# LMNS3d/SOFTX_2020_200

Hardware: AMD Instinct MI355X
Metric: nonlinear iters/sec (3D cavity Q2 128^3 BDF2) (higher is better)
Workload: dtype f64; 1 GPU; 3D lid-driven cavity Q2-Q2 128^3 transient BDF2 (BASELINE configs[2]); n_dofs=67898372, n_cells=2097152, parallelism=single

## Files before the change

softx_2020_200_amd/csrc/gls_api.cpp:

```cpp
#include <hip/hip_runtime.h>

#include <algorithm>
#include <array>
#include <chrono>
#include <cmath>
#include <cstdlib>
#include <cstdarg>
#include <cstdio>
#include <cstring>
#include <map>
#include <array>
#include <memory>
#include <string>
#include <vector>
#include <set>

#include "gls_ctx.hpp"

using namespace gls_impl;

namespace {

thread_local std::string g_err;

// ... 748 lines not shown
    v = c->hang.vbuf.p;
  }
  P.v = v;
  P.y = y;
  P.hmask = c->hang.on ? c->hang.hmask.p : nullptr;
  const bool brick = c->use_brick && mode != gls::MODE_DIAG;
  const bool col = brick && c->use_colors;
  if (col) set_colors(c, P, y);
  else P.slab = brick ? brick_slab(c) : nullptr;
  if (!brick) {
    GLS_TRY(ensure_element_maps(c));
    P.ev = c->ev.p;
    if (cq_on) {
      P.cq = c->cq.p;
      P.cq_mode = mode == gls::MODE_DIAG ? 1 : 2;
    }
  }
  const bool oct = c->oct.on && (mode == gls::MODE_JV || mode == gls::MODE_DIAG) && !brick;
  if (oct) {
    const size_t nq = gls::brick_qdata_size(c->k, 8 * c->oct.nb);
    if (c->qdata.n != nq) {
      GLS_TRY(c->qdata.alloc(nq));
      c->qd_valid = false;
      c->cq_valid = false;
    }
    if (mode == gls::MODE_JV && !c->qd_valid) GLS_TRY(oct_lin(c));
    if (mode == gls::MODE_JV && c->oct.f32_next && !c->qd32_valid) {
      if (c->qdata32.n != c->qdata.n) GLS_TRY(c->qdata32.alloc(c->qdata.n));
      HIP_TRY(gls::vec_to_f32(c->qdata.p, c->qdata32.p, (int64_t)c->qdata.n, c->stream));
      c->qd32_valid = true;
    }
    P.cell_list = c->oct.rest.p;
    P.cell_list_n = c->oct.n_rest;
  }
  if (!col && !P.slab && !P.ev) HIP_TRY(hipMemsetAsync(y, 0, sizeof(double) * c->n_dofs, c->stream));
  {
    TimedLaunch t(c, mode == gls::MODE_JVQ ? (int)gls::MODE_JV : (lin_diag ? (int)gls::MODE_DIAG : mode));
    if (brick && split_jv && mode == gls::MODE_JVQ) {
      auto &D = c->dist;
      double *vv = const_cast<double *>(v);
      const int64_t voff = 3 * (int64_t)c->n_vnodes;
      if (D.on && !D.comm) {
        GLS_TRY(dist_import(c, vv));
      } else if (D.on) {
        HIP_TRY(hipEventRecord(D.ev_ready, c->stream));
        HIP_TRY(hipStreamWaitEvent(D.xstream, D.ev_ready, 0));
        HIP_TRY(gls::vec_pack_nodes(vv, D.send_nodes.p, D.n_send, voff, D.send_buf, D.xstream));
        if (rccl_exchange_on(c, 0, D.xstream) != 0) return set_err(GLS_ECOMM, "ghost import exchange failed");
        HIP_TRY(gls::vec_unpack_nodes(vv, D.recv_nodes.p, D.n_recv, voff, D.recv_buf, 0, D.xstream));
        HIP_TRY(hipEventRecord(D.ev_done, D.xstream));
      }
      gls::OpParams Q = P;
      Q.subset = c->split.p + c->split_bnd;
      Q.subset_n = c->split_int;
      if (Q.subset_n > 0) HIP_TRY(gls::launch_brick_kernel(c->k, mode, Q, c->tables, c->stream));
      if (D.on && D.comm) HIP_TRY(hipStreamWaitEvent(c->stream, D.ev_done, 0));
      Q.subset = c->split.p;
      Q.subset_n = c->split_bnd;
      if (Q.subset_n > 0) HIP_TRY(gls::launch_brick_kernel(c->k, mode, Q, c->tables, c->stream));
    } else if (brick) {
      HIP_TRY(gls::launch_brick_kernel(c->k, mode, P, c->tables, c->stream));
    } else {
      HIP_TRY(gls::launch_cell_kernel(c->dim, c->k, c->kp, c->nq1d, mode, P, c->tables, c->stream));
      if (oct) {
        gls::OpParams Q = P;
        Q.cell_list = nullptr;
        Q.cell_list_n = 0;
        Q.y = nullptr;
        Q.qd = c->qdata.p;
        Q.subset = c->oct.list.p;
        Q.subset_n = c->oct.nb;
        Q.brick_cell0 = c->oct.cell0.p;
        const bool f32 = mode == gls::MODE_JV && c->oct.f32_next;
        if (f32) Q.qdf = c->qdata32.p;
        HIP_TRY(gls::launch_pencil_ev(mode == gls::MODE_JV ? gls::MODE_JVQ : gls::MODE_LIN, Q, c->tables, c->stream, f32));
        if (mode == gls::MODE_DIAG) {
          c->qd_valid = true;
          c->qd32_valid = false;
        }
      }
    }
  }
  if (P.ev)
    HIP_TRY(gls::gather_element_vectors(y, c->ev.p, c->ev_voff.p, c->ev_vslot.p, c->n_vnodes, c->ev_poff.p,
                                        c->ev_pslot.p, c->n_pnodes, c->dim, c->stream));
  if (brick && !col && P.slab) {
    TimedLaunch t(c, 5);
    HIP_TRY(slab_sum(c, y));
  }
  if (c->hang.on && (mode == gls::MODE_RESIDUAL || mode == gls::MODE_JV))
    HIP_TRY(gls::vec_csr_condense(y, c->hang.tm.p, c->hang.toff.p, c->hang.tdof.p, c->hang.tw.p,
                                  (int64_t)c->hang.tm.n, c->stream));
  if (!c->probe_local) GLS_TRY(dist_export_add(c, y));
  if (P.cq_mode == 1) c->cq_valid = true;
  if (lin_diag) {
    c->qd_valid = true;
    c->qd32_valid = P.qdf != nullptr;
    c->qd32_partial = P.qdf != nullptr && P.oseen;
  }
  return GLS_OK;
}

}
namespace gls_impl {
int ensure_diag(gls_ctx *c) {
  if (c->diag_valid) return GLS_OK;
  GLS_TRY(run_cell(c, gls::MODE_DIAG, nullptr, c->diag.p));
  if (c->dist.on) {
    const int64_t d = c->dim, nl = c->n_vnodes, no = c->dist.n_owned, npl = c->n_dofs - d * nl, nop = c->dist.n_owned_p;
    HIP_TRY(gls::vec_fill(c->diag.p + d * no, d * (nl - no), 1.0, c->stream));
    HIP_TRY(gls::vec_fill(c->diag.p + d * nl + nop, npl - nop, 1.0, c->stream));
  }
  c->diag_valid = true;
  return GLS_OK;
}
}
namespace {

int device_dot(gls_ctx *c, const double *a, const double *b, double *host_out) {
  return dist_multidot(c, a, 0, 1, b, host_out);
}

const double *reduce_dots_async(gls_ctx *c, const double *out, int nd, double *hp, int *err) {
  const double *res = out;
  *err = GLS_OK;
  if (c->dist.on) {
    if (hipMemcpyAsync(c->dist.red_buf, out, sizeof(double) * nd, hipMemcpyDeviceToDevice, c->stream) != hipSuccess) {
      *err = set_err(GLS_EHIP, "reduce_dots_async: D2D copy");
      return nullptr;
    }
    if (c->dist.allreduce(c->dist.user, c->dist.red_buf, nd) != 0) {
      *err = set_err(GLS_ECOMM, "allreduce failed");
      return nullptr;
    }
    res = c->dist.red_buf;
  }
  if (hipMemcpyAsync(hp, res, sizeof(double) * nd, hipMemcpyDeviceToHost, c->stream) != hipSuccess) {
    *err = set_err(GLS_EHIP, "reduce_dots_async: D2H copy");
    return nullptr;
  }
  return res;
}
int multidot_async(gls_ctx *c, const double *A, int64_t lda, int nk, const double *w, double *out, double *hp,
                   const double **dev_res) {
  const int64_t n1 = c->dist.on ? (int64_t)c->dim * c->dist.n_owned : c->n_dofs;
  const int64_t off2 = c->dist.on ? (int64_t)c->dim * c->n_vnodes : 0;
  const int64_t n2 = c->dist.on ? c->dist.n_owned_p : 0;
  HIP_TRY(gls::vec_multidot2(A, lda, nk, w, n1, off2, n2, out, c->work.p, c->stream));
  int err;
  *dev_res = reduce_dots_async(c, out, nk, hp, &err);
  return err;
}
int multiaxpy_dots_async(gls_ctx *c, double *w, const double *V, int64_t lda, int nk, const double *h, bool dots,
                         double *out, double *hp, const double **dev_res, double scale = 1.0) {
  const int64_t n1 = c->dist.on ? (int64_t)c->dim * c->dist.n_owned : c->n_dofs;
  const int64_t off2 = c->dist.on ? (int64_t)c->dim * c->n_vnodes : 0;
  const int64_t n2 = c->dist.on ? c->dist.n_owned_p : 0;
  HIP_TRY(gls::vec_multiaxpy_dots(w, V, lda, nk, h, 1.0, c->n_dofs, n1, off2, n2, dots, scale, out, c->work.p,
                                  c->stream));
  int err;
  *dev_res = reduce_dots_async(c, out, dots ? nk + 1 : 1, hp, &err);
  return err;
}

}

extern "C" {

int gls_create(const gls_mesh_desc *d, gls_ctx **out) {
  if (!d || !out) return set_err(GLS_EINVAL, "null argument");
  *out = nullptr;
  const int nq1d = d->nq1d > 0 ? d->nq1d : d->k + 1;
  if (d->dim != 2 && d->dim != 3) return set_err(GLS_EINVAL, "dim must be 2 or 3");
  if (!gls::cell_kernel_supported(d->dim, d->k, d->kp, nq1d))
    return set_err(GLS_EINVAL, "unsupported element Q%d-Q%d (dim %d, QGauss %d)", d->k, d->kp, d->dim, nq1d);
  const bool mapped = d->map_degree > 0;
  if (d->n_cells < 0 || d->n_vnodes <= 0 || d->n_pnodes <= 0 || !d->cell_vnodes || (!mapped && !d->cell_h))
    return set_err(GLS_EINVAL, "incomplete mesh description");
  if (mapped && (d->map_degree > 2 || !d->cell_support))
    return set_err(GLS_EINVAL, "mapped cells: map_degree 1 or 2 with cell_support");
  if (d->kp != d->k && !d->cell_pnodes) return set_err(GLS_EINVAL, "cell_pnodes required when kp != k");
  if (d->srf && !d->cell_x0 && !mapped) return set_err(GLS_EINVAL, "srf requires cell_x0");
  std::unique_ptr<gls_ctx> c(new gls_ctx);
  c->dim = d->dim;
  c->k = d->k;
  c->kp = d->kp;
  c->nq1d = nq1d;
  c->n_cells = d->n_cells;
  c->n_vnodes = d->n_vnodes;
  c->n_pnodes = d->n_pnodes;
  c->nq = gls::ipow(nq1d, d->dim);
  c->n_dofs = (int64_t)d->dim * d->n_vnodes + d->n_pnodes;
  c->viscosity = d->viscosity;
  c->srf = d->srf;
  for (int i = 0; i < 3; ++i) c->omega[i] = d->omega[i];
  c->tables = make_tables(d->k, d->kp, nq1d);
  const int nv = gls::ipow(d->k + 1, d->dim), np = gls::ipow(d->kp + 1, d->dim);
  for (int64_t i = 0; i < (int64_t)d->n_cells * nv; ++i)
    if (d->cell_vnodes[i] < 0 || d->cell_vnodes[i] >= d->n_vnodes) return set_err(GLS_EINVAL, "cell_vnodes out of range");
  if (d->cell_pnodes)
    for (int64_t i = 0; i < (int64_t)d->n_cells * np; ++i)
      if (d->cell_pnodes[i] < 0 || d->cell_pnodes[i] >= d->n_pnodes) return set_err(GLS_EINVAL, "cell_pnodes out of range");
  if (!d->cell_pnodes && d->n_pnodes != d->n_vnodes) return set_err(GLS_EINVAL, "n_pnodes != n_vnodes without cell_pnodes");

  GLS_TRY(c->cell_vnodes.upload(d->cell_vnodes, (size_t)d->n_cells * nv));
  c->use_brick = !mapped && detect_bricks(d, nq1d);
  if (c->use_brick) GLS_TRY(build_slab_map(c.get(), d));
  if (const char *e = std::getenv("GLS_JV_RECOMPUTE")) c->use_qdata = std::atoi(e) == 0;
  if (d->cell_pnodes) GLS_TRY(c->cell_pnodes.upload(d->cell_pnodes, (size_t)d->n_cells * np));
  std::vector<double> geo((size_t)d->n_cells * 4);
  const int nsup = mapped ? gls::ipow(d->map_degree + 1, d->dim) : 0;
  for (int cix = 0; cix < d->n_cells; ++cix) {
    double meas = 1.;
    if (mapped) {
      meas = corner_measure(d->dim, d->map_degree, d->cell_support + (size_t)cix * nsup * d->dim);
      if (!(meas > 0)) return set_err(GLS_EINVAL, "cell %d: non-positive measure (inverted cell)", cix);
      geo[cix * 4 + 0] = geo[cix * 4 + 1] = geo[cix * 4 + 2] = 1.0;
    } else {
      for (int e = 0; e < d->dim; ++e) {
        geo[cix * 4 + e] = d->cell_h[(size_t)cix * d->dim + e];
        meas *= geo[cix * 4 + e];
      }
      if (d->dim == 2) geo[cix * 4 + 2] = 1.0;
    }
    geo[cix * 4 + 3] = d->dim == 2 ? std::sqrt(4. * meas / M_PI) / d->k : std::pow(6 * meas / M_PI, 1. / 3.) / d->k;
  }
  GLS_TRY(c->geo.upload(geo.data(), geo.size()));
  if (mapped) {
    c->map_degree = d->map_degree;
    c->host_support.assign(d->cell_support, d->cell_support + (size_t)d->n_cells * nsup * d->dim);
    std::vector<double> gq((size_t)d->n_cells * c->nq * gls::kGeo);
    for (int cix = 0; cix < d->n_cells; ++cix) {
      mapped_geometry(d->dim, d->map_degree, nq1d, d->cell_support + (size_t)cix * nsup * d->dim,
                      gq.data() + (size_t)cix * c->nq * gls::kGeo);
      for (int q = 0; q < c->nq; ++q)
        if (!(gq[((size_t)cix * c->nq + q) * gls::kGeo + gls::kGeoJxW] > 0))
          return set_err(GLS_EINVAL, "cell %d: non-positive Jacobian at quadrature point %d", cix, q);
    }
    GLS_TRY(c->gq.upload(gq.data(), gq.size()));
  } else {
    c->host_h.assign(d->cell_h, d->cell_h + (size_t)d->n_cells * d->dim);
    if (d->cell_x0) c->host_x0.assign(d->cell_x0, d->cell_x0 + (size_t)d->n_cells * d->dim);
  }
  if (d->cell_x0) {
    std::vector<double> x0((size_t)d->n_cells * 3, 0.);
    for (int cix = 0; cix < d->n_cells; ++cix)
      for (int e = 0; e < d->dim; ++e) x0[cix * 3 + e] = d->cell_x0[(size_t)cix * d->dim + e];
    GLS_TRY(c->x0.upload(x0.data(), x0.size()));
  }
  if (d->force_q) GLS_TRY(c->force_q.upload(d->force_q, (size_t)d->n_cells * c->nq * d->dim));
  std::vector<int64_t> con;
  if (d->vnode_mask) {
    GLS_TRY(c->vmask.upload(d->vnode_mask, (size_t)d->n_vnodes));
    for (int64_t n = 0; n < d->n_vnodes; ++n)
      for (int e = 0; e < d->dim; ++e)
        if ((d->vnode_mask[n] >> e) & 1) con.push_back(n * d->dim + e);
  }
  GLS_TRY(c->con_dofs.upload(con.data(), con.size()));
  GLS_TRY(c->diag.alloc(c->n_dofs));
  GLS_TRY(c->work.alloc(gls::multidot_work_size()));
  GLS_TRY(c->scal.alloc(64));
  if (hipStreamCreateWithFlags(&c->stream, hipStreamNonBlocking) != hipSuccess)
    return set_err(GLS_EHIP, "stream create failed");
  c->own_stream = true;
  HIP_TRY(hipDeviceSynchronize());
  *out = c.release();
  return GLS_OK;
}

int gls_destroy(gls_ctx *c) {
  if (!c) return GLS_OK;
  (void)hipStreamSynchronize(c->stream);
  delete c;
  return GLS_OK;
}

int gls_set_stream(gls_ctx *c, void *s) {
  GLS_TRY(check_ctx(c));
  if (c->own_stream && c->stream) {
    (void)hipStreamSynchronize(c->stream);
    (void)hipStreamDestroy(c->stream);
  }
  c->own_stream = false;
  c->stream = (hipStream_t)s;
  if (c->mg.on) {
    for (size_t l = 1; l < c->mg.lev.size(); ++l) GLS_TRY(gls_set_stream(c->mg.lev[l], s));
    if (c->mg.replica) GLS_TRY(gls_set_stream(c->mg.replica, s));
    if (c->mg.rep2) GLS_TRY(gls_set_stream(c->mg.rep2, s));
  }
  return GLS_OK;
}

int gls_uses_brick_kernels(const gls_ctx *c) { return c && c->use_brick ? 1 : 0; }

int gls_quadrature_points(const gls_ctx *c, double *xq) {
  if (!c || !xq) return set_err(GLS_EINVAL, "null argument");
  const int dim = c->dim, nq = c->nq;
  if (c->map_degree > 0) {
    const int nsup = gls::ipow(c->map_degree + 1, dim);
    std::vector<double> g((size_t)nq * gls::kGeo);
    for (int cix = 0; cix < c->n_cells; ++cix) {
      mapped_geometry(dim, c->map_degree, c->nq1d, c->host_support.data() + (size_t)cix * nsup * dim, g.data());
      for (int q = 0; q < nq; ++q)
        for (int e = 0; e < dim; ++e) xq[((size_t)cix * nq + q) * dim + e] = g[(size_t)q * gls::kGeo + gls::kGeoX + e];
    }
    return GLS_OK;
  }
  if (c->host_x0.empty()) return set_err(GLS_EINVAL, "gls_quadrature_points: the mesh was created without cell_x0");
  for (int cix = 0; cix < c->n_cells; ++cix)
    for (int q = 0; q < nq; ++q) {
      const int qi[3] = {q % c->nq1d, (q / c->nq1d) % c->nq1d, q / (c->nq1d * c->nq1d)};
      for (int e = 0; e < dim; ++e)
        xq[((size_t)cix * nq + q) * dim + e] =
            c->host_x0[(size_t)cix * dim + e] + c->host_h[(size_t)cix * dim + e] * c->tables.xi[qi[e]];
    }
  return GLS_OK;
}

int gls_n_dofs(const gls_ctx *c, int64_t *n) {
  if (!c || !n) return set_err(GLS_EINVAL, "null argument");
  *n = c->n_dofs;
  return GLS_OK;
}

int gls_set_force(gls_ctx *c, const double *f) {
  GLS_TRY(check_ctx(c));
  HIP_TRY(hipStreamSynchronize(c->stream));
  if (!f) {
    c->force_q.release();
  } else {
    GLS_TRY(c->force_q.upload(f, (size_t)c->n_cells * c->nq * c->dim));
  }
  c->diag_valid = false;
  c->ilu.valid = false;
  c->qd_valid = false;
  c->cq_valid = false;
  return GLS_OK;
}

int gls_set_viscosity(gls_ctx *c, double nu) {
  GLS_TRY(check_ctx(c));
  c->viscosity = nu;
  c->diag_valid = false;
  c->ilu.valid = false;
  c->qd_valid = false;
  c->cq_valid = false;
  return GLS_OK;
}

int gls_set_time(gls_ctx *c, int scheme, const double ts[4]) {
  GLS_TRY(check_ctx(c));
  if (scheme < GLS_STEADY || scheme > GLS_SDIRK3_3) return set_err(GLS_EINVAL, "scheme %d", scheme);
  if (scheme != GLS_STEADY && (!ts || ts[0] == 0.)) return set_err(GLS_EINVAL, "time steps required");
  c->scheme = scheme;
  if (ts)
    for (int i = 0; i < 4; ++i) c->time_steps[i] = ts[i];
  if (!c->jf.on) c->mg.dirty = true;
  for (double &a : c->alpha) a = 0.;
  c->alpha_jac = 0.;
  c->sdt2 = 0.;
  c->n_hist = 0;
  if (scheme != GLS_STEADY) {
    const double sdt = 1. / ts[0];
    c->sdt2 = sdt * sdt;
  }
  if (scheme == GLS_BDF1 || scheme == GLS_BDF2 || scheme == GLS_BDF3) {
    const int order = scheme - GLS_BDF1 + 1;
    double a[6];
    GLS_TRY(gls_bdf_coefficients(order, ts, 4, a));
    for (int i = 0; i <= order; ++i) c->alpha[i] = a[i];
    c->alpha_jac = a[0];
    c->n_hist = order;
  } else if (is_sdirk(scheme)) {
    const bool three = scheme == GLS_SDIRK3 || scheme == GLS_SDIRK3_1 || scheme == GLS_SDIRK3_2 || scheme == GLS_SDIRK3_3;
    const int order = three ? 3 : 2;
    double t[12];
    GLS_TRY(gls_sdirk_coefficients(order, ts[0], t));
    int stage = 0;
    if (scheme == GLS_SDIRK2_1 || scheme == GLS_SDIRK3_1) stage = 1;
    if (scheme == GLS_SDIRK2_2 || scheme == GLS_SDIRK3_2) stage = 2;
    if (scheme == GLS_SDIRK3_3) stage = 3;
    c->alpha_jac = t[0];
    if (stage > 0) {
      for (int i = 0; i <= stage; ++i) c->alpha[i] = t[(stage - 1) * (order + 1) + i];
      c->n_hist = stage;
    }
  }
  if (!c->jf.on) {
    c->diag_valid = false;
    c->ilu.valid = false;
    c->qd_valid = false;
    c->cq_valid = false;
  }
  return GLS_OK;
}

int gls_set_state(gls_ctx *c, const double *u, const double *u1, const double *u2, const double *u3) {
  GLS_TRY(check_ctx(c));
  if (!u) return set_err(GLS_EINVAL, "u is null");
  c->u = u;
  c->u1 = u1;
  c->u2 = u2;
  c->u3 = u3;
  if (!c->jf.on) {
    c->diag_valid = false;
    c->ilu.valid = false;
    c->qd_valid = false;
    c->cq_valid = false;
    c->mg.dirty = true;
  }
  return dist_import(c, const_cast<double *>(u));
}

int gls_freeze_jacobian(gls_ctx *c, int freeze) {
  GLS_TRY(check_ctx(c));
  auto &j = c->jf;
  if (!freeze) {
    if (j.on) {
      j.on = false;
      c->diag_valid = false;
      c->ilu.valid = false;
      c->qd_valid = false;
      c->cq_valid = false;
      c->mg.dirty = true;
    }
    return GLS_OK;
  }
  if (!c->u) return set_err(GLS_EINVAL, "gls_freeze_jacobian: gls_set_state was not called");
  if (j.on) return GLS_OK;
  const size_t n = (size_t)c->n_dofs;
  if (j.u.n != n) GLS_TRY(j.u.alloc(n));
  HIP_TRY(hipMemcpyAsync(j.u.p, c->u, sizeof(double) * n, hipMemcpyDeviceToDevice, c->stream));
  const double *hs[3] = {c->u1, c->u2, c->u3};
  for (int h = 0; h < 3; ++h) {
    j.has[h] = hs[h] != nullptr && h < c->n_hist;
    if (!j.has[h]) continue;
    if (j.h[h].n != n) GLS_TRY(j.h[h].alloc(n));
    HIP_TRY(hipMemcpyAsync(j.h[h].p, hs[h], sizeof(double) * n, hipMemcpyDeviceToDevice, c->stream));
  }
  for (int i = 0; i < 4; ++i) {
    j.alpha[i] = c->alpha[i];
    j.ts[i] = c->time_steps[i];
  }
  j.alpha_jac = c->alpha_jac;
  j.sdt2 = c->sdt2;
  j.n_hist = c->n_hist;
  j.scheme = c->scheme;
  j.on = true;
  return GLS_OK;
}

int gls_dist_import(gls_ctx *c, double *x) {
  GLS_TRY(check_ctx(c));
  return dist_import(c, x);
}

int gls_dist_attach(gls_ctx *c, int64_t n_owned_nodes, int n_nbrs, const int64_t *send_offsets,
                    const int32_t *send_nodes, const int64_t *recv_offsets, const int32_t *recv_nodes, double *send_buf,
                    double *recv_buf, double *red_buf, gls_exchange_fn xchg, gls_allreduce_fn allreduce, void *user) {
  GLS_TRY(check_ctx(c));
  if (c->dim != 3 || c->k != c->kp || c->cell_pnodes.p) return set_err(GLS_EINVAL, "distributed path: 3D Qk-Qk only");
  if (n_owned_nodes < 0 || n_owned_nodes > c->n_vnodes || n_nbrs < 0 || !xchg || !allreduce || !red_buf)
    return set_err(GLS_EINVAL, "gls_dist_attach: bad arguments");
  const int64_t ns = n_nbrs ? send_offsets[n_nbrs] : 0, nr = n_nbrs ? recv_offsets[n_nbrs] : 0;
  for (int64_t i = 0; i < ns; ++i)
    if (send_nodes[i] < 0 || send_nodes[i] >= n_owned_nodes) return set_err(GLS_EINVAL, "send node not owned");
  for (int64_t i = 0; i < nr; ++i)
    if (recv_nodes[i] < n_owned_nodes || recv_nodes[i] >= c->n_vnodes) return set_err(GLS_EINVAL, "recv node not a ghost");
  if ((ns && !send_buf) || (nr && !recv_buf)) return set_err(GLS_EINVAL, "exchange buffers missing");
  GLS_TRY(upload_export_order(c->dist, send_nodes, ns));
  GLS_TRY(c->dist.send_nodes.upload(send_nodes, (size_t)ns));
  GLS_TRY(c->dist.recv_nodes.upload(recv_nodes, (size_t)nr));
  c->dist.n_owned = n_owned_nodes;
  c->dist.n_owned_p = n_owned_nodes;
  c->dist.dofs = false;
  c->dist.width = 4;
  c->dist.n_send = ns;
  c->dist.n_recv = nr;
  c->dist.send_buf = send_buf;
  c->dist.recv_buf = recv_buf;
  c->dist.red_buf = red_buf;
  c->dist.xchg = xchg;
  c->dist.allreduce = allreduce;
  c->dist.user = user;
  c->dist.on = true;
  c->diag_valid = false;
  c->ilu.valid = false;
  c->qd_valid = false;
  c->cq_valid = false;
  if (c->use_brick && gls::brick_subset_supported(c->k)) {
    std::vector<char> flag((size_t)c->n_vnodes, 0);
    for (int64_t i = 0; i < ns; ++i) flag[(size_t)send_nodes[i]] = 1;
    for (int64_t i = 0; i < nr; ++i) flag[(size_t)recv_nodes[i]] = 1;
    GLS_TRY(build_brick_split(c, flag));
  }
  return GLS_OK;
}

int gls_dist_attach_dofs(gls_ctx *c, int64_t n_owned_vnodes, int64_t n_owned_pnodes, int n_nbrs,
                         const int64_t *send_offsets, const int32_t *send_dofs, const int64_t *recv_offsets,
                         const int32_t *recv_dofs, double *send_buf, double *recv_buf, double *red_buf,
                         gls_exchange_fn xchg, gls_allreduce_fn allreduce, void *user) {
  GLS_TRY(check_ctx(c));
  const int64_t nvd = (int64_t)c->dim * c->n_vnodes, npn = c->n_dofs - nvd;
  if (n_owned_vnodes < 0 || n_owned_vnodes > c->n_vnodes || n_owned_pnodes < 0 || n_owned_pnodes > npn || n_nbrs < 0 ||
      !xchg || !allreduce || !red_buf)
    return set_err(GLS_EINVAL, "gls_dist_attach_dofs: bad arguments");
  if (c->mg.on) return set_err(GLS_EINVAL, "gls_dist_attach_dofs: no multigrid");
  const int64_t ns = n_nbrs ? send_offsets[n_nbrs] : 0, nr = n_nbrs ? recv_offsets[n_nbrs] : 0;
  auto owned = [&](int64_t d) { return d < nvd ? d / c->dim < n_owned_vnodes : d - nvd < n_owned_pnodes; };
  for (int64_t i = 0; i < ns; ++i)
    if (send_dofs[i] < 0 || send_dofs[i] >= c->n_dofs || !owned(send_dofs[i])) return set_err(GLS_EINVAL, "send DoF not owned");
  for (int64_t i = 0; i < nr; ++i)
    if (recv_dofs[i] < 0 || recv_dofs[i] >= c->n_dofs || owned(recv_dofs[i])) return set_err(GLS_EINVAL, "recv DoF not a ghost");
  if ((ns && !send_buf) || (nr && !recv_buf)) return set_err(GLS_EINVAL, "exchange buffers missing");
  auto &D = c->dist;
  GLS_TRY(upload_export_order(D, send_dofs, ns));
  GLS_TRY(D.send_nodes.upload(send_dofs, (size_t)ns));
  GLS_TRY(D.recv_nodes.upload(recv_dofs, (size_t)nr));
  D.h_send.assign(send_dofs, send_dofs + ns);
  D.h_recv.assign(recv_dofs, recv_dofs + nr);
  D.h_soff.assign(1, 0);
  D.h_roff.assign(1, 0);
  if (n_nbrs > 0) {
    D.h_soff.assign(send_offsets, send_offsets + n_nbrs + 1);
    D.h_roff.assign(recv_offsets, recv_offsets + n_nbrs + 1);
  }
  D.dofs = true;
  D.width = 1;
  D.n_owned = n_owned_vnodes;
  D.n_owned_p = n_owned_pnodes;
  D.n_send = ns;
  D.n_recv = nr;
  D.send_buf = send_buf;
  D.recv_buf = recv_buf;
  D.red_buf = red_buf;
  D.xchg = xchg;
  D.allreduce = allreduce;
  D.user = user;
  D.on = true;
  c->diag_valid = false;
  c->ilu.valid = false;
  c->qd_valid = false;
  c->cq_valid = false;
  return GLS_OK;
}

int gls_residual(gls_ctx *c, double *rhs) {
  GLS_TRY(check_ctx(c));
  if (!rhs) return set_err(GLS_EINVAL, "rhs is null");
  GLS_TRY(run_cell(c, gls::MODE_RESIDUAL, nullptr, rhs));
  HIP_TRY(gls::vec_set_indexed(rhs, c->con_dofs.p, nullptr, (int64_t)c->con_dofs.n, c->stream));
  return GLS_OK;
}

int gls_residual_and_diagonal(gls_ctx *c, double *rhs, double *d) {
  GLS_TRY(check_ctx(c));
  if (!rhs) return set_err(GLS_EINVAL, "rhs is null");
  if (!c->u) return set_err(GLS_EINVAL, "gls_set_state was not called");
  if (c->n_hist > 0 && !c->u1) return set_err(GLS_EINVAL, "scheme needs solution_m1");
  if (c->n_hist > 1 && !c->u2) return set_err(GLS_EINVAL, "scheme needs solution_m2");
  if (c->n_hist > 2 && !c->u3) return set_err(GLS_EINVAL, "scheme needs solution_m3");
  const bool fuse = !c->diag_valid && c->use_brick && c->use_qdata && c->use_slab && !c->use_colors && !c->hang.on &&
                    !c->dist.on && !c->jf.on && c->k == 2 && c->cube_nb1 > 0 && gls::pencil_enabled() &&
                    std::getenv("GLS_NO_RESLIN") == nullptr;
  if (fuse) {
    const size_t nq = gls::brick_qdata_size(c->k, c->n_cells);
    if (c->qdata.n != nq) GLS_TRY(c->qdata.alloc(nq));
    double *slab = brick_slab(c);
    if (!slab) return set_err(GLS_ENOMEM, "slab allocation failed");
    if (c->slab2.n != c->slab.n) GLS_TRY(c->slab2.alloc(c->slab.n));
    gls::OpParams P = make_params(c, true);
    P.qd = c->qdata.p;
    GLS_TRY(lin_f32_target(c, P));
    P.y = c->diag.p;
    P.slab = slab;
    P.res_y = rhs;
    P.res_slab = c->slab2.p;
    {
      TimedLaunch t(c, gls::MODE_DIAG);
      HIP_TRY(gls::launch_pencil_reslin(P, c->tables, c->stream));
    }
    {
      TimedLaunch t(c, 5);
      HIP_TRY(slab_sum_ex(c, c->slab2.p, nullptr, rhs, nullptr, nullptr, nullptr, 0.0, nullptr));
    }
    {
      TimedLaunch t(c, 5);
      HIP_TRY(slab_sum(c, c->diag.p));
    }
    HIP_TRY(gls::vec_set_indexed(rhs, c->con_dofs.p, nullptr, (int64_t)c->con_dofs.n, c->stream));
    c->qd_valid = true;
    c->qd32_valid = P.qdf != nullptr;
  c->qd32_partial = P.qdf != nullptr && P.oseen;
    c->diag_valid = true;
  } else {
    GLS_TRY(gls_residual(c, rhs));
    GLS_TRY(ensure_diag(c));
  }
  if (d && d != c->diag.p) HIP_TRY(gls::vec_copy(d, c->diag.p, c->n_dofs, c->stream));
  return GLS_OK;
}

int gls_jacobian_diagonal(gls_ctx *c, double *d) {
  GLS_TRY(check_ctx(c));
  GLS_TRY(ensure_diag(c));
  if (d && d != c->diag.p) HIP_TRY(gls::vec_copy(d, c->diag.p, c->n_dofs, c->stream));
  return GLS_OK;
}

int gls_jacobian_apply(gls_ctx *c, const double *v, double *y) {
  GLS_TRY(check_ctx(c));
  if (!v || !y || v == y) return set_err(GLS_EINVAL, "v/y null or aliased");
  if (c->con_dofs.n || c->dist.on) GLS_TRY(ensure_diag(c));
  GLS_TRY(run_cell(c, gls::MODE_JV, v, y));
  HIP_TRY(gls::vec_gather_scale_set(y, c->diag.p, v, c->con_dofs.p, (int64_t)c->con_dofs.n, c->stream));
  return GLS_OK;
}

}
namespace gls_impl {
int ensure_qdata32(gls_ctx *g, bool full) {
  GLS_TRY(ensure_qdata(g));
  if (!g->qd32_valid || (full && g->qd32_partial)) {
    if (g->qdata32.n != g->qdata.n) GLS_TRY(g->qdata32.alloc(g->qdata.n));
    HIP_TRY(gls::vec_to_f32(g->qdata.p, g->qdata32.p, (int64_t)g->qdata.n, g->stream));
    g->qd32_valid = true;
    g->qd32_partial = false;
  }
  return GLS_OK;
}
bool slab_f32() { return std::getenv("GLS_SLAB_F64") == nullptr; }
bool first_sweep_fusable(gls_ctx *g) {
  const char *e = std::getenv("GLS_MG_FIRST_FUSE");
  return e && std::atoi(e) != 0 && g->smooth_f32 && g->use_brick && g->use_qdata && !g->use_colors && !g->dist.on &&
         !g->hang.on && g->k == 2 && g->cube_nb1 > 0 && g->use_slab && gls::pencil_enabled() &&
         std::getenv("GLS_MG_NO_FUSE") == nullptr;
}
int jacobian_apply_f32(gls_ctx *g, const double *v, double *y, const double *rb, double first_omega, bool oseen) {
  if (!g->u) return set_err(GLS_EINVAL, "gls_set_state was not called");
  GLS_TRY(ensure_diag(g));
  GLS_TRY(ensure_qdata32(g, !oseen));
  GLS_TRY(dist_import(g, const_cast<double *>(v)));
  gls::OpParams P = make_params(g, true);
  P.qdf = g->qdata32.p;
  P.oseen = oseen ? 1 : 0;
  P.v = v;
  P.y = y;
  const bool col = g->use_colors;
  P.slab = col ? nullptr : brick_slab(g);
  const bool fuse_rb = rb && (P.slab || col) && !g->dist.on && gls::brick_fused_jacobi_supported(g->k) &&
                       std::getenv("GLS_MG_NO_FUSE") == nullptr;
  P.rb = fuse_rb ? rb : nullptr;
  P.slabf = P.slab && slab_f32() && gls::brick_fused_jacobi_supported(g->k) ? reinterpret_cast<float *>(P.slab)
                                                                             : nullptr;
  if (first_omega > 0.0) {
    if (!fuse_rb || !first_sweep_fusable(g)) return set_err(GLS_EINVAL, "fused first sweep not applicable");
    P.jx0 = const_cast<double *>(v);
    P.jd = g->diag.p;
    P.jomega = first_omega;
  }
  if (col) set_colors(g, P, y);
  if (!col && !P.slab) HIP_TRY(hipMemsetAsync(y, 0, sizeof(double) * g->n_dofs, g->stream));
  {
    TimedLaunch t(g, 4);
    HIP_TRY(gls::launch_brick_jv_f32(g->k, P, g->tables, g->stream));
  }
  if (P.slab) {
    TimedLaunch t(g, 5);
    HIP_TRY(slab_sum_ex(g, P.slab, P.slabf, y, nullptr, nullptr, P.jx0 ? g->diag.p : nullptr, P.jomega, P.rb, P.jx0));
  }
  GLS_TRY(dist_export_add(g, y));
  HIP_TRY(gls::vec_gather_scale_set(y, g->diag.p, v, g->con_dofs.p, (int64_t)g->con_dofs.n, g->stream, P.rb));
  if (rb && !fuse_rb) HIP_TRY(gls::vec_axpby(y, 1.0, rb, -1.0, g->n_dofs, g->stream));
  return GLS_OK;
}
int smoother_apply(gls_ctx *g, const double *v, double *y, const double *rb) {
  if (g->smooth_f32 && g->use_brick && g->use_qdata) return jacobian_apply_f32(g, v, y, rb, 0.0, g->smooth_oseen);
  g->oct.f32_next = g->smooth_f32 && g->oct.on;
  const int rc = gls_jacobian_apply(g, v, y);
  g->oct.f32_next = false;
  GLS_TRY(rc);
  if (rb) HIP_TRY(gls::vec_axpby(y, 1.0, rb, -1.0, g->n_dofs, g->stream));
  return GLS_OK;
}
static int ilu_sweep(gls_ctx *g, double *x, const double *b, double *y, double *z) {
  GLS_TRY(ensure_ilu(g));
  GLS_TRY(gls_jacobian_apply(g, x, y));
  HIP_TRY(gls::vec_axpby(y, 1.0, b, -1.0, g->n_dofs, g->stream));
  GLS_TRY(apply_ilu(g, y, z));
  HIP_TRY(gls::vec_axpy(x, 1.0, z, g->n_dofs, g->stream));
  return GLS_OK;
}
int smoother_sweep(gls_ctx *g, double *x, const double *b, double *y, double omega, double *z, const double *pxc) {
  const bool nofuse = std::getenv("GLS_MG_NO_FUSE") != nullptr;
  const bool brick = g->use_brick && g->use_qdata && (g->use_colors || brick_slab(g)) && !g->dist.on &&
                     !g->hang.on && gls::brick_fused_jacobi_supported(g->k);
  if (pxc && ((z && g->ilu.on && !g->ilu.probe_only) || nofuse || !brick || !g->smooth_f32 || g->use_colors || g->cube_nb1 <= 0))
    return set_err(GLS_EINVAL, "fused prolongation not applicable");
  if (z && g->ilu.on && !g->ilu.probe_only) return ilu_sweep(g, x, b, y, z);
  if (nofuse || !brick) {
    GLS_TRY(smoother_apply(g, x, y));
    HIP_TRY(gls::mg_jacobi_update(x, b, y, g->diag.p, omega, g->n_dofs, 0, g->stream));
    return GLS_OK;
  }
  if (!g->u) return set_err(GLS_EINVAL, "gls_set_state was not called");
  GLS_TRY(ensure_diag(g));
  const bool f32 = g->smooth_f32;
  GLS_TRY(f32 ? ensure_qdata32(g, !g->smooth_oseen) : ensure_qdata(g));
  gls::OpParams P = make_params(g, true);
  P.v = x;
// ... 73 lines not shown
}

}
static int detect_oct_bricks(gls_ctx *c) {
  auto &O = c->oct;
  O = gls_ctx::Oct();
  const char *e = std::getenv("GLS_OCT_BRICKS");
  if ((e && std::atoi(e) == 0) || c->dim != 3 || c->k != 2 || c->kp != 2 || c->map_degree > 0 || c->dist.on ||
      c->cell_pnodes.p || c->host_h.empty() || !gls::pencil_enabled() || c->n_cells < 8)
    return GLS_OK;
  const int64_t nc = c->n_cells;
  std::vector<int32_t> cv((size_t)nc * 27);
  HIP_TRY(hipMemcpy(cv.data(), c->cell_vnodes.p, cv.size() * sizeof(int32_t), hipMemcpyDeviceToHost));
  std::vector<int32_t> cell0;
  std::vector<char> in((size_t)nc, 0);
  int32_t lat[125];
  for (int64_t i = 0; i + 8 <= nc;) {
    bool ok = true;
    for (int ci = 1; ci < 8 && ok; ++ci)
      for (int d = 0; d < 3; ++d) ok = ok && c->host_h[(size_t)(i + ci) * 3 + d] == c->host_h[(size_t)i * 3 + d];
    for (int t = 0; t < 125 && ok; ++t) lat[t] = -1;
    for (int ci = 0; ci < 8 && ok; ++ci) {
      const int cx = ci & 1, cy = (ci >> 1) & 1, cz = ci >> 2;
      for (int a = 0; a < 27 && ok; ++a) {
        const int X = 2 * cx + a % 3, Y = 2 * cy + (a / 3) % 3, Z = 2 * cz + a / 9;
        int32_t &slot = lat[X + 5 * (Y + 5 * Z)];
        const int32_t nd = cv[(size_t)(i + ci) * 27 + a];
        if (slot < 0) slot = nd;
        else ok = slot == nd;
      }
    }
    if (ok) {
      std::vector<int32_t> u(lat, lat + 125);
      std::sort(u.begin(), u.end());
      ok = std::adjacent_find(u.begin(), u.end()) == u.end();
    }
    if (ok) {
      cell0.push_back((int32_t)i);
      for (int ci = 0; ci < 8; ++ci) in[(size_t)(i + ci)] = 1;
      i += 8;
    } else {
      ++i;
    }
  }
  if (cell0.empty()) return GLS_OK;
  std::vector<int32_t> rest;
  for (int64_t q = 0; q < nc; ++q)
    if (!in[(size_t)q]) rest.push_back((int32_t)q);
  std::vector<int32_t> list(cell0.size());
  for (size_t b = 0; b < list.size(); ++b) list[b] = (int32_t)b;
  GLS_TRY(O.cell0.upload(cell0.data(), cell0.size()));
  GLS_TRY(O.list.upload(list.data(), list.size()));
  O.n_rest = (int)rest.size();
  if (rest.empty()) rest.push_back(0);
  GLS_TRY(O.rest.upload(rest.data(), rest.size()));
  O.nb = (int)cell0.size();
  O.on = true;
  return GLS_OK;
}
extern "C" {
int gls_forest_bricks(const gls_ctx *c) { return c && c->oct.on ? c->oct.nb : 0; }

int gls_set_hanging(gls_ctx *c, int64_t n, const int64_t *dofs, const int64_t *off, const int64_t *masters,
                    const double *w) {
  GLS_TRY(check_ctx(c));
  if (n < 0 || (n > 0 && (!dofs || !off || !masters || !w))) return set_err(GLS_EINVAL, "gls_set_hanging: arrays");
  if (c->mg.on) return set_err(GLS_EINVAL, "hanging constraints: no multigrid");
  if (c->dist.on && !c->dist.dofs) return set_err(GLS_EINVAL, "hanging constraints across ranks: gls_dist_attach_dofs");
  HIP_TRY(hipStreamSynchronize(c->stream));
  const int dim = c->dim;
  const int64_t N = c->n_dofs, nvd = (int64_t)dim * c->n_vnodes;
  std::vector<uint8_t> vm((size_t)c->n_vnodes, 0);
  if (c->vmask.p) HIP_TRY(hipMemcpy(vm.data(), c->vmask.p, (size_t)c->n_vnodes, hipMemcpyDeviceToHost));
  auto dirichlet = [&](int64_t d) { return d < nvd && ((vm[(size_t)(d / dim)] >> (d % dim)) & 1); };
  std::vector<char> is_h((size_t)N, 0);
  if (n > 0 && off[0] != 0) return set_err(GLS_EINVAL, "gls_set_hanging: offsets[0] != 0");
  for (int64_t i = 0; i < n; ++i) {
    const int64_t d = dofs[i];
    if (d < 0 || d >= N || off[i + 1] < off[i]) return set_err(GLS_EINVAL, "gls_set_hanging: line %lld", (long long)i);
    if (dirichlet(d)) return set_err(GLS_EINVAL, "hanging DoF %lld carries a Dirichlet mask bit", (long long)d);
    if (is_h[(size_t)d]) return set_err(GLS_EINVAL, "hanging DoF %lld listed twice", (long long)d);
    is_h[(size_t)d] = 1;
  }
  const int64_t nm = n ? off[n] : 0;
  for (int64_t j = 0; j < nm; ++j)
    if (masters[j] < 0 || masters[j] >= N || is_h[(size_t)masters[j]])
      return set_err(GLS_EINVAL, "gls_set_hanging: master %lld out of range or hanging itself", (long long)masters[j]);
  std::vector<int64_t> ooff{0}, omas, cnt((size_t)N + 1, 0);
  std::vector<double> ow;
  for (int64_t i = 0; i < n; ++i) {
    for (int64_t j = off[i]; j < off[i + 1]; ++j)
      if (!dirichlet(masters[j])) {
        omas.push_back(masters[j]);
        ow.push_back(w[j]);
        ++cnt[(size_t)masters[j] + 1];
      }
    ooff.push_back((int64_t)omas.size());
  }
  std::vector<int64_t> tm, toff{0};
  std::vector<int64_t> start((size_t)N + 1, 0);
  for (int64_t m = 0; m < N; ++m) {
    start[(size_t)m + 1] = start[(size_t)m] + cnt[(size_t)m + 1];
    if (cnt[(size_t)m + 1]) {
      tm.push_back(m);
      toff.push_back(start[(size_t)m + 1]);
    }
  }
  std::vector<int64_t> tdof(omas.size()), fill(start.begin(), start.end() - 1);
  std::vector<double> tw(omas.size());
  for (int64_t i = 0; i < n; ++i)
    for (int64_t j = ooff[(size_t)i]; j < ooff[(size_t)i + 1]; ++j) {
      const int64_t slot = fill[(size_t)omas[(size_t)j]]++;
      tdof[(size_t)slot] = dofs[i];
      tw[(size_t)slot] = ow[(size_t)j];
    }
  c->hang.h_dof.assign(dofs, dofs + n);
  c->hang.h_off.assign(off, off + n + 1);
  c->hang.h_master.assign(masters, masters + nm);
  if (n == 0) c->hang.h_off.assign(1, 0);
  std::vector<uint8_t> hm((size_t)c->n_vnodes, 0), dm((size_t)N, 0);
  std::vector<int64_t> con;
  for (int64_t d = 0; d < N; ++d) {
    if (is_h[(size_t)d] && d < nvd) hm[(size_t)(d / dim)] |= (uint8_t)(1u << (d % dim));
    dm[(size_t)d] = is_h[(size_t)d] ? 1 : 0;
    if (is_h[(size_t)d] || dirichlet(d)) con.push_back(d);
  }
  auto &h = c->hang;
  GLS_TRY(h.dof.upload(dofs, (size_t)n));
  GLS_TRY(h.off.upload(off, (size_t)(n ? n + 1 : 0)));
  GLS_TRY(h.master.upload(masters, (size_t)nm));
  GLS_TRY(h.w.upload(w, (size_t)nm));
  GLS_TRY(h.ooff.upload(ooff.data(), n ? ooff.size() : 0));
  GLS_TRY(h.omaster.upload(omas.data(), omas.size()));
  GLS_TRY(h.ow.upload(ow.data(), ow.size()));
  GLS_TRY(h.tm.upload(tm.data(), tm.size()));
  GLS_TRY(h.toff.upload(toff.data(), tm.empty() ? 0 : toff.size()));
  GLS_TRY(h.tdof.upload(tdof.data(), tdof.size()));
  GLS_TRY(h.tw.upload(tw.data(), tw.size()));
  GLS_TRY(h.hmask.upload(hm.data(), hm.size()));
  GLS_TRY(h.dmask.upload(dm.data(), dm.size()));
  GLS_TRY(c->con_dofs.upload(con.data(), con.size()));
  h.on = n > 0;
  c->use_brick = false;
  c->use_slab = false;
  c->use_colors = false;
  c->diag_valid = false;
  c->ilu.valid = false;
  c->qd_valid = false;
  c->cq_valid = false;
  return detect_oct_bricks(c);
}

namespace {
int apply_prec(gls_ctx *c, const double *v, double *z) {
  if (c->mg.on && c->mg.rep_csr) return mg_vcycle_rep2(c, v, z);
  if (c->mg.on) return mg_vcycle(c, 0, v, z);
  if (c->ilu.on && !c->ilu.probe_only) return apply_ilu(c, v, z);
  HIP_TRY(gls::vec_div(z, v, c->diag.p, c->n_dofs, c->stream));
  return GLS_OK;
}
}

int gls_apply_preconditioner(gls_ctx *c, const double *v, double *z) {
  GLS_TRY(check_ctx(c));
  if (!v || !z || v == z) return set_err(GLS_EINVAL, "v/z null or aliased");
  GLS_TRY(ensure_diag(c));
  if (c->mg.on) GLS_TRY(mg_prepare(c));
  GLS_TRY(ensure_ilu(c));
  return apply_prec(c, v, z);
}


static int solve_bicgstab(gls_ctx *c, const double *b, double *x, gls_linear_params *prm) {
  const int64_t n = c->n_dofs;
  hipStream_t s = c->stream;
  double *w[7];
  if (c->krylov.p && c->krylov.n >= (size_t)7 * n) {
    for (int i = 0; i < 7; ++i) w[i] = c->krylov.p + (int64_t)i * n;
  } else {
    if (c->bicg.n != (size_t)7 * n) GLS_TRY(c->bicg.alloc((size_t)7 * n));
    for (int i = 0; i < 7; ++i) w[i] = c->bicg.p + (int64_t)i * n;
  }
  double *r = w[0], *rh = w[1], *p = w[2], *v = w[3], *ph = w[4], *sh = w[5], *t = w[6];
  double bn2;
  GLS_TRY(device_dot(c, b, b, &bn2));
  const double tol = std::max(prm->relative_residual * std::sqrt(bn2), prm->minimum_residual);
  HIP_TRY(gls::vec_fill(x, n, 0.0, s));
  HIP_TRY(gls::vec_copy(r, b, n, s));
  HIP_TRY(gls::vec_copy(rh, b, n, s));
  HIP_TRY(gls::vec_fill(p, n, 0.0, s));
  HIP_TRY(gls::vec_fill(v, n, 0.0, s));
  double res = std::sqrt(bn2), rho = 1.0, alpha = 1.0, omega = 1.0;
  int it = 0;
  bool converged = res <= tol;
  while (!converged && it < prm->max_iterations) {
    double rho1;
    GLS_TRY(device_dot(c, rh, r, &rho1));
    if (rho1 == 0.0 || omega == 0.0) break;
    const double beta = (rho1 / rho) * (alpha / omega);
    rho = rho1;
    HIP_TRY(gls::vec_axpy(p, -omega, v, n, s));
    HIP_TRY(gls::vec_axpby(p, 1.0, r, beta, n, s));
    GLS_TRY(apply_prec(c, p, ph));
    GLS_TRY(gls_jacobian_apply(c, ph, v));
    double rhv;
    GLS_TRY(device_dot(c, rh, v, &rhv));
    if (rhv == 0.0) break;
    alpha = rho / rhv;
    HIP_TRY(gls::vec_axpy(r, -alpha, v, n, s));
    HIP_TRY(gls::vec_axpy(x, alpha, ph, n, s));
    ++it;
    double sn2;
    GLS_TRY(device_dot(c, r, r, &sn2));
    res = std::sqrt(sn2);
    if (res <= tol) {
      converged = true;
      break;
    }
    GLS_TRY(apply_prec(c, r, sh));
    GLS_TRY(gls_jacobian_apply(c, sh, t));
    double tt, ts;
    GLS_TRY(device_dot(c, t, t, &tt));
    GLS_TRY(device_dot(c, t, r, &ts));
    if (tt == 0.0) break;
    omega = ts / tt;
    HIP_TRY(gls::vec_axpy(x, omega, sh, n, s));
    HIP_TRY(gls::vec_axpy(r, -omega, t, n, s));
    double rn2;
    GLS_TRY(device_dot(c, r, r, &rn2));
    res = std::sqrt(rn2);
    converged = res <= tol;
    if (getenv("GLS_GMRES_VERBOSE") && (it % 10 == 0 || it == 1))
      printf("  bicgstab it %d  res %.6e  (tol %.3e)\n", it, res, tol);
  }
  if (converged && prm->true_residual) {
    GLS_TRY(gls_jacobian_apply(c, x, t));
    HIP_TRY(gls::vec_axpby(t, 1.0, b, -1.0, n, s));
    double rn2;
    GLS_TRY(device_dot(c, t, t, &rn2));
    res = std::sqrt(rn2);
  }
  prm->iterations = it;
  prm->final_residual = res;
  if (!converged) return set_err(GLS_ENOCONV, "BiCGStab: %d iterations, residual %.3e > %.3e", it, res, tol);
  return GLS_OK;
}

int gls_solve_linear(gls_ctx *c, const double *b, double *x, gls_linear_params *prm) {
  GLS_TRY(check_ctx(c));
  if (!b || !x || !prm) return set_err(GLS_EINVAL, "null argument");
  const int m = prm->restart > 0 ? std::min(prm->restart, 200) : 30;
  const int64_t n = c->n_dofs;
  if (c->krylov_m != m || !c->krylov.p) {
    GLS_TRY(c->krylov.alloc((size_t)(m + 1) * n));
    GLS_TRY(c->coef.alloc((size_t)m + 8));
    if (c->scal.n < (size_t)m + 8) GLS_TRY(c->scal.alloc((size_t)m + 8));
    if (c->scal2.n < (size_t)m + 8) GLS_TRY(c->scal2.alloc((size_t)m + 8));
    if (c->hpin_n < 3 * ((size_t)m + 8)) {
      if (c->hpin) HIP_TRY(hipHostFree(c->hpin));
      c->hpin = nullptr;
      c->hpin_n = 0;
      HIP_TRY(hipHostMalloc(reinterpret_cast<void **>(&c->hpin), sizeof(double) * 3 * ((size_t)m + 8)));
      c->hpin_n = 3 * ((size_t)m + 8);
    }
    c->krylov_m = m;
  }
  if (!c->tmp1.p) {
    GLS_TRY(c->tmp1.alloc(n));
    GLS_TRY(c->tmp2.alloc(n));
  }
  GLS_TRY(ensure_diag(c));
  if (c->mg.on) GLS_TRY(mg_prepare(c));
  GLS_TRY(ensure_ilu(c));
  if (prm->method == GLS_LIN_BICGSTAB) return solve_bicgstab(c, b, x, prm);
  if (prm->method != GLS_LIN_GMRES) return set_err(GLS_EINVAL, "linear solver method %d unknown", prm->method);
  const bool keepz = c->mg.on;
  if (keepz && c->zbasis.n != (size_t)m * n) GLS_TRY(c->zbasis.alloc((size_t)m * n));
  double *V = c->krylov.p, *z = c->tmp1.p, *r = c->tmp2.p;
  hipStream_t s = c->stream;
  double bnorm2;
  GLS_TRY(device_dot(c, b, b, &bnorm2));
  const double tol = std::max(prm->relative_residual * std::sqrt(bnorm2), prm->minimum_residual);
  bool x_zero = keepz;
  if (!keepz) HIP_TRY(gls::vec_fill(x, n, 0.0, s));
  const double *rcur = b;
  double beta = std::sqrt(bnorm2);
  int it = 0;
  std::vector<double> H((size_t)(m + 1) * m), cs(m), sn(m), g(m + 1), hc2(m + 2), y(m);
  const bool gram = prm->orthogonalization != GLS_ORTHO_CGS2;
  int ortho_repairs = 0;
  const double repair_tol = std::getenv("GLS_GMRES_REPAIR_TOL") ? std::atof(std::getenv("GLS_GMRES_REPAIR_TOL")) : 1e-8;
  const bool repair_measured = std::getenv("GLS_GMRES_REPAIR_MEASURED") != nullptr;
  std::vector<double> Gm((size_t)(m + 1) * (m + 1), 0.0);
  bool converged = beta <= tol;
  const bool lverbose = std::getenv("GLS_ILU_VERBOSE") != nullptr;
  while (!converged && it < prm->max_iterations) {
    if (lverbose) std::printf("gmres: it %d residual %.6e (tol %.3e)\n", it, beta, tol);
    HIP_TRY(gls::vec_axpby(V, 1.0 / beta, rcur, 0.0, n, s));
    std::fill(Gm.begin(), Gm.end(), 0.);
    std::fill(g.begin(), g.end(), 0.);
    g[0] = beta;
    int j = 0;
    double res = beta;
    for (; j < m && it < prm->max_iterations; ++j) {
      double *vj = V + (int64_t)j * n, *w = V + (int64_t)(j + 1) * n;
      double *zj = keepz ? c->zbasis.p + (int64_t)j * n : z;
      GLS_TRY(apply_prec(c, vj, zj));
      GLS_TRY(gls_jacobian_apply(c, zj, w));
      double *hp1 = c->hpin, *hp2 = c->hpin + (m + 8), *hp3 = c->hpin + 2 * (m + 8);
      const double *hdev = nullptr, *h2dev = nullptr, *h3dev = nullptr;
      GLS_TRY(multidot_async(c, V, n, j + 2, w, c->scal.p, hp1, &hdev));
      double wn2, wnorm, wnorm0;
      bool normalized = false;
      bool done = false;
      if (gram) {
        HIP_TRY(hipStreamSynchronize(s));
        const double wn0sq = std::max(hp1[j + 1], 0.0);
        wnorm0 = std::sqrt(wn0sq);
        auto G = [&](int a, int b) { return Gm[(size_t)std::min(a, b) * (m + 1) + std::max(a, b)]; };
        double *hc = hp3;
        for (int i = 0; i <= j; ++i) {
          double t = hp1[i];
          for (int k = 0; k <= j; ++k)
            if (k != i) t -= G(i, k) * hp1[k];
          hc[i] = t;
        }
        double q = wn0sq;
        for (int i = 0; i <= j; ++i) q += hc[i] * hc[i] - 2.0 * hc[i] * hp1[i];
        for (int i = 0; i <= j; ++i)
          for (int k = i + 1; k <= j; ++k) q += 2.0 * hc[i] * hc[k] * G(i, k);
        if (q > 1e-20 * wn0sq && q > 0.) {
          const double est = std::sqrt(q);
          HIP_TRY(hipMemcpyAsync(c->coef.p, hc, sizeof(double) * (j + 1), hipMemcpyHostToDevice, s));
          if (j + 1 <= 8) {
            GLS_TRY(multiaxpy_dots_async(c, w, V, n, j + 1, c->coef.p, true, c->scal2.p, hp2, &h2dev, 1.0 / est));
          } else {
            HIP_TRY(gls::vec_multiaxpy(w, V, n, j + 1, c->coef.p, 1.0, n, s));
            HIP_TRY(gls::vec_scale(w, 1.0 / est, n, s));
            GLS_TRY(multidot_async(c, V, n, j + 2, w, c->scal2.p, hp2, &h2dev));
          }
          HIP_TRY(hipStreamSynchronize(s));
          for (int i = 0; i <= j; ++i) H[(size_t)i * m + j] = hc[i];
          H[(size_t)(j + 1) * m + j] = est;
          double gmax = 0., gg = 0.;
          for (int i = 0; i <= j; ++i) {
            gmax = std::max(gmax, std::fabs(hp2[i]));
            gg += hp2[i] * hp2[i];
          }
          const double nrm2 = hp2[j + 1];
          const double est2sq = nrm2 - gg;
          if (gmax > repair_tol || std::fabs(nrm2 - 1.0) > repair_tol) {
            const bool use_est = est2sq > 1e-4 && !repair_measured;
            const double est2 = use_est ? std::sqrt(est2sq) : 1.0;
            for (int i = 0; i <= j; ++i) H[(size_t)i * m + j] += est * hp2[i];
            if (j + 1 <= 8) {
              GLS_TRY(multiaxpy_dots_async(c, w, V, n, j + 1, h2dev, true, c->scal.p, hp1, &hdev, 1.0 / est2));
            } else {
              HIP_TRY(gls::vec_multiaxpy(w, V, n, j + 1, h2dev, 1.0, n, s));
              if (use_est) HIP_TRY(gls::vec_scale(w, 1.0 / est2, n, s));
              GLS_TRY(multidot_async(c, V, n, j + 2, w, c->scal.p, hp1, &hdev));
            }
            HIP_TRY(hipStreamSynchronize(s));
            const double nn = std::max(hp1[j + 1], 0.0);
            double sc = 1.0;
            if (nn <= 1e-28 * (use_est ? 1.0 : std::max(nrm2, 1e-300))) {
              sc = 0.0;
            } else if (!use_est || std::fabs(nn - 1.0) > 1e-8) {
              sc = std::sqrt(nn);
              HIP_TRY(gls::vec_scale(w, 1.0 / sc, n, s));
            }
            H[(size_t)(j + 1) * m + j] = est * est2 * sc;
            for (int i = 0; i <= j; ++i) Gm[(size_t)i * (m + 1) + j + 1] = sc > 0. ? hp1[i] / sc : 0.;
            ++ortho_repairs;
          } else {
            for (int i = 0; i <= j; ++i) Gm[(size_t)i * (m + 1) + j + 1] = hp2[i];
          }
          wnorm = H[(size_t)(j + 1) * m + j];
          normalized = done = true;
        }
      }
      if (done) {
      } else if (j + 1 <= 8) {
        GLS_TRY(multiaxpy_dots_async(c, w, V, n, j + 1, hdev, true, c->scal2.p, hp2, &h2dev));
        HIP_TRY(hipStreamSynchronize(s));
        wnorm0 = std::sqrt(std::max(hp1[j + 1], 0.0));
        for (int i = 0; i <= j; ++i) H[(size_t)i * m + j] = hp1[i];
        std::copy(hp2, hp2 + j + 2, hc2.begin());
        wnorm = std::sqrt(std::max(hc2[j + 1], 0.0));
        if (wnorm < 0.7071 * wnorm0) {
          for (int i = 0; i <= j; ++i) H[(size_t)i * m + j] += hc2[i];
          double h2 = 0.;
          for (int i = 0; i <= j; ++i) h2 += hc2[i] * hc2[i];
          const double est2 = wnorm * wnorm - h2;
          if (est2 > 0.25 * wnorm * wnorm && est2 > 0.) {
            const double est = std::sqrt(est2);
            GLS_TRY(multiaxpy_dots_async(c, w, V, n, j + 1, h2dev, false, c->scal.p, hp3, &h3dev, 1.0 / est));
            HIP_TRY(hipStreamSynchronize(s));
            wn2 = hp3[0];
            H[(size_t)(j + 1) * m + j] = est;
            normalized = true;
            wnorm = est * std::sqrt(std::max(wn2, 0.0));
          } else {
            GLS_TRY(multiaxpy_dots_async(c, w, V, n, j + 1, h2dev, false, c->scal.p, hp3, &h3dev));
            HIP_TRY(hipStreamSynchronize(s));
            wn2 = hp3[0];
            wnorm = std::sqrt(std::max(wn2, 0.0));
          }
        }
      } else {
        HIP_TRY(gls::vec_multiaxpy(w, V, n, j + 1, hdev, 1.0, n, s));
        GLS_TRY(multidot_async(c, w, 0, 1, w, c->scal2.p, hp2, &h2dev));
        HIP_TRY(hipStreamSynchronize(s));
        wnorm0 = std::sqrt(std::max(hp1[j + 1], 0.0));
        for (int i = 0; i <= j; ++i) H[(size_t)i * m + j] = hp1[i];
        wn2 = hp2[0];
        wnorm = std::sqrt(std::max(wn2, 0.0));
        if (wnorm < 0.7071 * wnorm0) {
          GLS_TRY(multidot_async(c, V, n, j + 1, w, c->scal.p, hp1, &hdev));
          HIP_TRY(gls::vec_multiaxpy(w, V, n, j + 1, hdev, 1.0, n, s));
          GLS_TRY(multidot_async(c, w, 0, 1, w, c->scal2.p, hp2, &h2dev));
          HIP_TRY(hipStreamSynchronize(s));
          for (int i = 0; i <= j; ++i) H[(size_t)i * m + j] += hp1[i];
          wn2 = hp2[0];
          wnorm = std::sqrt(std::max(wn2, 0.0));
        }
      }
      if (!normalized) {
        H[(size_t)(j + 1) * m + j] = wnorm;
        if (wnorm > 0) HIP_TRY(gls::vec_scale(w, 1.0 / wnorm, n, s));
      }
      for (int i = 0; i < j; ++i) {
        const double a = H[(size_t)i * m + j], bb = H[(size_t)(i + 1) * m + j];
        H[(size_t)i * m + j] = cs[i] * a + sn[i] * bb;
        H[(size_t)(i + 1) * m + j] = -sn[i] * a + cs[i] * bb;
      }
      const double a = H[(size_t)j * m + j], bb = H[(size_t)(j + 1) * m + j];
      const double rr = std::hypot(a, bb);
      cs[j] = rr > 0 ? a / rr : 1.0;
      sn[j] = rr > 0 ? bb / rr : 0.0;
      H[(size_t)j * m + j] = rr;
      H[(size_t)(j + 1) * m + j] = 0.;
      g[j + 1] = -sn[j] * g[j];
      g[j] = cs[j] * g[j];
      res = std::fabs(g[j + 1]);
      ++it;
      if (getenv("GLS_GMRES_VERBOSE") && (it % 10 == 0 || it == 1))
        printf("  gmres it %d  res %.6e  (tol %.3e)\n", it, res, tol);
      if (res <= tol || wnorm == 0.) { ++j; break; }
    }
    const int kdim = j;
    for (int i = kdim - 1; i >= 0; --i) {
      double s_ = g[i];
      for (int l = i + 1; l < kdim; ++l) s_ -= H[(size_t)i * m + l] * y[l];
      y[i] = H[(size_t)i * m + i] != 0. ? s_ / H[(size_t)i * m + i] : 0.;
    }
    HIP_TRY(hipMemcpyAsync(c->coef.p, y.data(), sizeof(double) * kdim, hipMemcpyHostToDevice, s));
    if (keepz) {
      HIP_TRY(gls::vec_multiaxpy(x, c->zbasis.p, n, kdim, c->coef.p, -1.0, n, s, x_zero));
      x_zero = false;
    } else {
      HIP_TRY(gls::vec_fill(r, n, 0.0, s));
      HIP_TRY(gls::vec_multiaxpy(r, V, n, kdim, c->coef.p, -1.0, n, s));
      GLS_TRY(apply_prec(c, r, z));
      HIP_TRY(gls::vec_axpy(x, 1.0, z, n, s));
    }
    if (res <= tol) {
      beta = res;
      converged = true;
      if (prm->true_residual) {
        GLS_TRY(gls_jacobian_apply(c, x, r));
        HIP_TRY(gls::vec_axpby(r, 1.0, b, -1.0, n, s));
        double rn2;
        GLS_TRY(device_dot(c, r, r, &rn2));
        beta = std::sqrt(rn2);
      }
      break;
    }
    GLS_TRY(gls_jacobian_apply(c, x, r));
    HIP_TRY(gls::vec_axpby(r, 1.0, b, -1.0, n, s));
    rcur = r;
    double rn2;
    GLS_TRY(device_dot(c, r, r, &rn2));
    beta = std::sqrt(rn2);
    converged = beta <= tol;
    if (beta == 0.) break;
  }
  if (x_zero) HIP_TRY(gls::vec_fill(x, n, 0.0, s));
  prm->iterations = it;
  prm->final_residual = beta;
  if (ortho_repairs && std::getenv("GLS_GMRES_VERBOSE")) printf("  gmres: %d orthogonality repair passes\n", ortho_repairs);
  if (!converged) return set_err(GLS_ENOCONV, "GMRES: %d iterations, residual %.3e > %.3e", it, beta, tol);
  return GLS_OK;
}

}

namespace {

struct NewtonStats {
  int outer = 0, linear = 0, residuals = 0;
  double final_res = 0.;
};

template <class Phys>
int skip_newton_template(Phys &ph, double tolerance, int max_iterations, int verbosity, int skip_iterations,
                         bool is_initial_step, bool force_matrix_renewal, int &consecutive, NewtonStats &st) {
  double current_res = 1.0, last_res = 1.0;
  int outer = 0;
  bool assembly_needed = consecutive == 0 || is_initial_step || force_matrix_renewal;
  while (current_res > tolerance && outer < max_iterations) {
    GLS_TRY(ph.evaluation_point_from_present());
    if (assembly_needed) {
      GLS_TRY(ph.assemble_matrix_and_rhs());
      ++st.residuals;
    } else if (outer == 0) {
      GLS_TRY(ph.assemble_rhs());
      ++st.residuals;
    }
    if (outer == 0) {
      GLS_TRY(ph.rhs_norm(current_res));
      last_res = current_res;
    }
    if (verbosity) printf("Newton iteration: %d  - Residual:  %g\n", outer, current_res);
    int lin_it = 0;
    GLS_TRY(ph.solve_linear_system(lin_it));
    st.linear += lin_it;
    for (double alpha = 1.0; alpha > 1e-3; alpha *= 0.5) {
      GLS_TRY(ph.line_point(alpha));
      GLS_TRY(ph.assemble_rhs());
      ++st.residuals;
      GLS_TRY(ph.rhs_norm(current_res));
      if (verbosity) printf("\t\talpha = %6g res = %g\n", alpha, current_res);
      if (current_res < 0.9 * last_res || last_res < tolerance) break;
    }
    GLS_TRY(ph.present_from_evaluation_point());
    last_res = current_res;
    ++outer;
    assembly_needed = false;
  }
  if (!force_matrix_renewal) consecutive = (consecutive + 1) % std::max(skip_iterations, 1);
  st.outer = outer;
  st.final_res = current_res;
  return GLS_OK;
}

template <class Phys>
int newton_template(Phys &ph, double tolerance, int max_iterations, int verbosity, NewtonStats &st) {
  double current_res = 1.0, last_res = 1.0;
  int outer = 0;
  while (current_res > tolerance && outer < max_iterations) {
    GLS_TRY(ph.evaluation_point_from_present());
    GLS_TRY(ph.assemble_matrix_and_rhs());
    ++st.residuals;
    if (outer == 0) {
      GLS_TRY(ph.rhs_norm(current_res));
      last_res = current_res;
    }
    if (verbosity) printf("Newton iteration: %d  - Residual:  %g\n", outer, current_res);
    int lin_it = 0;
    GLS_TRY(ph.solve_linear_system(lin_it));
    st.linear += lin_it;
    for (double alpha = 1.0; alpha > 1e-3; alpha *= 0.5) {
      GLS_TRY(ph.line_point(alpha));
      GLS_TRY(ph.assemble_rhs());
      ++st.residuals;
      GLS_TRY(ph.rhs_norm(current_res));
      if (verbosity) printf("\t\talpha = %6g res = %g\n", alpha, current_res);
      if (current_res < 0.9 * last_res || last_res < tolerance) break;
    }
    GLS_TRY(ph.present_from_evaluation_point());
    last_res = current_res;
    ++outer;
  }
  st.outer = outer;
  st.final_res = current_res;
  return GLS_OK;
}

struct SectionScope {
  gls_ctx *c;
  int s;
  std::chrono::steady_clock::time_point t0;
  SectionScope(gls_ctx *c_, int s_) : c(c_), s(s_) {
    if (c->sec_on) {
      (void)hipStreamSynchronize(c->stream);
      t0 = std::chrono::steady_clock::now();
    }
  }
  ~SectionScope() {
    if (!c->sec_on) return;
    (void)hipStreamSynchronize(c->stream);
    c->sec_t[s] += std::chrono::duration<double>(std::chrono::steady_clock::now() - t0).count();
    ++c->sec_n[s];
  }
};

struct DevicePhysics {
  gls_ctx *c;
  double *present, *eval, *update, *rhs;
  const double *u1, *u2, *u3;
  gls_linear_params lin;
  int verbosity;
  bool skip = false;
  int linear_failures = 0;
  int evaluation_point_from_present() {
    if (!skip) return gls_set_state(c, present, u1, u2, u3);
    HIP_TRY(gls::vec_copy(eval, present, c->n_dofs, c->stream));
    return gls_set_state(c, eval, u1, u2, u3);
  }
  int assemble_matrix_and_rhs() {
    SectionScope t(c, GLS_SEC_ASSEMBLE_SYSTEM);
    if (skip) {
      GLS_TRY(gls_freeze_jacobian(c, 0));
      GLS_TRY(gls_set_state(c, eval, u1, u2, u3));
    }
    GLS_TRY(gls_residual_and_diagonal(c, rhs, nullptr));
    return skip ? gls_freeze_jacobian(c, 1) : GLS_OK;
  }
  int assemble_rhs() {
    SectionScope t(c, GLS_SEC_ASSEMBLE_RHS);
    return gls_residual(c, rhs);
  }
  int rhs_norm(double &r) {
    double r2;
    GLS_TRY(device_dot(c, rhs, rhs, &r2));
    r = std::sqrt(r2);
    return GLS_OK;
  }
  int solve_linear_system(int &its) {
    gls_linear_params lp = lin;
    if (c->mg.on) {
      SectionScope t(c, GLS_SEC_SETUP_GMG);
      GLS_TRY(ensure_diag(c));
      GLS_TRY(mg_prepare(c));
    } else if (c->ilu.on && !c->ilu.probe_only) {
      SectionScope t(c, GLS_SEC_SETUP_ILU);
      GLS_TRY(ensure_diag(c));
      GLS_TRY(ensure_ilu(c));
    }
    SectionScope t(c, GLS_SEC_SOLVE_LINEAR);
    const int rc = gls_solve_linear(c, rhs, update, &lp);
    if (rc < 0 && rc != GLS_ENOCONV) return rc;
    if (rc == GLS_ENOCONV) {
      ++linear_failures;
      if (verbosity) printf("  -Iterative solver did not converge: %d steps, residual %g\n", lp.iterations, lp.final_residual);
    }
    its = lp.iterations;
    if (verbosity) printf("  -Iterative solver took : %d steps \n", lp.iterations);
    HIP_TRY(gls::vec_set_indexed(update, c->con_dofs.p, nullptr, (int64_t)c->con_dofs.n, c->stream));
    return GLS_OK;
  }
  int line_point(double alpha) {
    HIP_TRY(gls::vec_waxpy(eval, present, alpha, update, c->n_dofs, c->stream));
    GLS_TRY(gls_apply_dirichlet(c, eval));
    return gls_set_state(c, eval, u1, u2, u3);
  }
  int present_from_evaluation_point() {
    HIP_TRY(gls::vec_copy(present, eval, c->n_dofs, c->stream));
    return GLS_OK;
  }
};

struct KatPhysics {
  double present[2] = {1., 0.}, eval[2] = {0, 0}, update[2] = {0, 0}, rhs[2] = {0, 0};
  double J[2][2] = {{0, 0}, {0, 0}};
  int evaluation_point_from_present() { eval[0] = present[0]; eval[1] = present[1]; return GLS_OK; }
  int assemble_matrix_and_rhs() {
    J[0][0] = 2 * eval[0]; J[0][1] = 1; J[1][0] = 0; J[1][1] = 2;
    return assemble_rhs();
  }
  int assemble_rhs() {
    rhs[0] = -(eval[0] * eval[0] + eval[1]);
    rhs[1] = -(2 * eval[1] + 3);
    return GLS_OK;
  }
  int rhs_norm(double &r) { r = std::sqrt(rhs[0] * rhs[0] + rhs[1] * rhs[1]); return GLS_OK; }
  int solve_linear_system(int &its) {
    const double det = J[0][0] * J[1][1] - J[0][1] * J[1][0];
    if (det == 0.) return set_err(GLS_EINVAL, "singular KAT Jacobian");
    update[0] = (rhs[0] * J[1][1] - J[0][1] * rhs[1]) / det;
    update[1] = (J[0][0] * rhs[1] - J[1][0] * rhs[0]) / det;
    its = 1;
    return GLS_OK;
  }
  int line_point(double a) { eval[0] = present[0] + a * update[0]; eval[1] = present[1] + a * update[1]; return GLS_OK; }
  int present_from_evaluation_point() { present[0] = eval[0]; present[1] = eval[1]; return GLS_OK; }
};

}

extern "C" {

int gls_newton_solve(gls_ctx *c, double *present, const double *u1, const double *u2, const double *u3,
                     gls_newton_params *prm) {
  GLS_TRY(check_ctx(c));
  if (!present || !prm) return set_err(GLS_EINVAL, "null argument");
  const int64_t n = c->n_dofs;
  if (!c->tmp3.p) {
    GLS_TRY(c->tmp3.alloc(n));
    GLS_TRY(c->tmp4.alloc(n));
    GLS_TRY(c->tmp5.alloc(n));
  }
  DevicePhysics ph{c, present, c->tmp3.p, c->tmp4.p, c->tmp5.p, u1, u2, u3, prm->lin, prm->verbosity};
  NewtonStats st;
  if (prm->solver == GLS_SKIP_NEWTON) {
    ph.skip = true;
    GLS_TRY(skip_newton_template(ph, prm->tolerance, prm->max_iterations, prm->verbosity, prm->skip_iterations,
                                 prm->is_initial_step != 0, prm->force_matrix_renewal != 0, c->skip_consecutive, st));
  } else {
    GLS_TRY(gls_freeze_jacobian(c, 0));
    GLS_TRY(newton_template(ph, prm->tolerance, prm->max_iterations, prm->verbosity, st));
  }
  HIP_TRY(hipStreamSynchronize(c->stream));
  prm->newton_iterations = st.outer;
  prm->linear_iterations = st.linear;
  prm->residual_evaluations = st.residuals;
  prm->final_residual = st.final_res;
  prm->linear_failures = ph.linear_failures;
  return GLS_OK;
}

int gls_section_timing(gls_ctx *c, int enable) {
  GLS_TRY(check_ctx(c));
  c->sec_on = enable != 0;
  for (int i = 0; i < GLS_N_SECTIONS; ++i) {
    c->sec_t[i] = 0.;
    c->sec_n[i] = 0;
  }
  return GLS_OK;
}
int gls_section_get(const gls_ctx *c, int section, double *seconds, int *calls) {
  if (!c) return set_err(GLS_EINVAL, "null context");
  if (section < 0 || section >= GLS_N_SECTIONS) return set_err(GLS_EINVAL, "section %d", section);
  if (seconds) *seconds = c->sec_t[section];
  if (calls) *calls = c->sec_n[section];
  return GLS_OK;
}

int gls_newton_selftest(double xo[2]) {
  if (!xo) return set_err(GLS_EINVAL, "null");
  KatPhysics ph;
  NewtonStats st;
  GLS_TRY(newton_template(ph, 1e-8, 10, 0, st));
  xo[0] = ph.present[0];
  xo[1] = ph.present[1];
  return GLS_OK;
}

int gls_skip_newton_selftest(int skip_iterations, double xo[2]) {
  if (!xo || skip_iterations < 1) return set_err(GLS_EINVAL, "gls_skip_newton_selftest arguments");
  KatPhysics ph;
  NewtonStats st;
  int consecutive = 0;
  GLS_TRY(skip_newton_template(ph, 1e-8, 10, 0, skip_iterations, true, true, consecutive, st));
  xo[0] = ph.present[0];
  xo[1] = ph.present[1];
  return GLS_OK;
}

int gls_mesh_hyper_cube_sizes(int dim, int n, int k, int kp, int pmask, int64_t *nc, int64_t *nv, int64_t *np) {
  if ((dim != 2 && dim != 3) || n <= 0 || k <= 0 || kp <= 0) return set_err(GLS_EINVAL, "mesh args");
  int64_t c = 1, v = 1, p = 1;
  for (int d = 0; d < dim; ++d) {
    const bool per = (pmask >> d) & 1;
    c *= n;
    v *= (int64_t)k * n + (per ? 0 : 1);
    p *= (int64_t)kp * n + (per ? 0 : 1);
  }
  if (nc) *nc = c;
  if (nv) *nv = v;
  if (np) *np = p;
  return GLS_OK;
}

int gls_mesh_hyper_cube(int dim, int n, int k, int kp, double lo, double hi, int pmask, int32_t *cv, int32_t *cp,
                        double *x0, double *h) {
  int64_t nc, nv, np;
  GLS_TRY(gls_mesh_hyper_cube_sizes(dim, n, k, kp, pmask, &nc, &nv, &np));
  if (nv > INT32_MAX || np > INT32_MAX) return set_err(GLS_EINVAL, "mesh too large for int32 node ids");
  int L = 0;
  while ((1 << L) < n) ++L;
  const double hc = (hi - lo) / n;
  int vsh[3], psh[3];
  for (int d = 0; d < 3; ++d) {
    const bool per = (pmask >> d) & 1;
    vsh[d] = k * n + (per ? 0 : 1);
    psh[d] = kp * n + (per ? 0 : 1);
  }
  const int nvl = gls::ipow(k + 1, dim), npl = gls::ipow(kp + 1, dim);
  int64_t cell = 0;
  const int64_t total = (int64_t)1 << (dim * L);
  for (int64_t mcode = 0; mcode < total; ++mcode) {
    int ijk[3] = {0, 0, 0};
    for (int b = 0; b < L; ++b)
      for (int d = 0; d < dim; ++d) ijk[d] |= (int)((mcode >> (b * dim + d)) & 1) << b;
    bool inside = true;
    for (int d = 0; d < dim; ++d) inside = inside && ijk[d] < n;
    if (!inside) continue;
    for (int a = 0; a < nvl; ++a) {
      int loc[3] = {a % (k + 1), (a / (k + 1)) % (k + 1), a / ((k + 1) * (k + 1))};
      int64_t id = 0, stride = 1;
      for (int d = 0; d < dim; ++d) {
        id += (int64_t)((ijk[d] * k + loc[d]) % vsh[d]) * stride;
        stride *= vsh[d];
      }
      cv[cell * nvl + a] = (int32_t)id;
    }
    if (cp) {
      for (int a = 0; a < npl; ++a) {
        int loc[3] = {a % (kp + 1), (a / (kp + 1)) % (kp + 1), a / ((kp + 1) * (kp + 1))};
        int64_t id = 0, stride = 1;
        for (int d = 0; d < dim; ++d) {
          id += (int64_t)((ijk[d] * kp + loc[d]) % psh[d]) * stride;
          stride *= psh[d];
        }
        cp[cell * npl + a] = (int32_t)id;
      }
    }
    for (int d = 0; d < dim; ++d) {
      if (x0) x0[cell * dim + d] = lo + ijk[d] * hc;
      if (h) h[cell * dim + d] = hc;
    }
    ++cell;
  }
  return cell == nc ? GLS_OK : set_err(GLS_EINVAL, "morton enumeration mismatch");
}

int gls_timing_enable(gls_ctx *c, int en) {
  GLS_TRY(check_ctx(c));
  c->timing = en != 0;
  return GLS_OK;
}
int gls_timing_reset(gls_ctx *c) {
  GLS_TRY(check_ctx(c));
  HIP_TRY(hipStreamSynchronize(c->stream));
  for (auto &e : c->events) { (void)hipEventDestroy(e.a); (void)hipEventDestroy(e.b); }
  c->events.clear();
  for (int i = 0; i < 6; ++i) { c->t_ms[i] = 0; c->t_n[i] = 0; }
  return GLS_OK;
}
int gls_timing_get(gls_ctx *c, int which, double *ms, int64_t *cnt) {
  GLS_TRY(check_ctx(c));
  if (which < 0 || which > 5) return set_err(GLS_EINVAL, "which");
  HIP_TRY(hipStreamSynchronize(c->stream));
  for (auto &e : c->events) {
    float t = 0;
    HIP_TRY(hipEventElapsedTime(&t, e.a, e.b));
    c->t_ms[e.which] += t;
    c->t_n[e.which] += 1;
    (void)hipEventDestroy(e.a);
    (void)hipEventDestroy(e.b);
  }
  c->events.clear();
  if (ms) *ms = c->t_ms[which];
  if (cnt) *cnt = c->t_n[which];
  return GLS_OK;
}

}
```

softx_2020_200_amd/csrc/gls_brick_kernels.hip:

```cpp
#include "gls_brick_common.hpp"
#include "gls_common.hpp"
#include "gls_launch.hpp"

#include <algorithm>
#include <cstdlib>
#include <type_traits>

#ifndef GLS_ABL
#define GLS_ABL 0
#endif
#ifndef GLS_ROWS_REG
#define GLS_ROWS_REG 1
#endif
#ifndef GLS_BRICK_WAVES_PER_EU
#define GLS_BRICK_WAVES_PER_EU 4
#endif
#ifndef GLS_BRICK_WPE_F32
#define GLS_BRICK_WPE_F32 6
#endif

#ifndef GLS_QD_LITE
#define GLS_QD_LITE 0
#endif

// ... 1077 lines not shown
__device__ __forceinline__ uint32_t morton3(uint32_t x, uint32_t y, uint32_t z) {
  uint32_t m = 0;
  for (int b = 0; b < 10; ++b)
    m |= (((x >> b) & 1u) << (3 * b)) | (((y >> b) & 1u) << (3 * b + 1)) | (((z >> b) & 1u) << (3 * b + 2));
  return m;
}
template <typename S, bool J, int K, bool XS = false>
__global__ void __launch_bounds__(256) k_slab_sum_cube(const S *__restrict__ slab, int nb1, int64_t voff,
                                                       double *__restrict__ y, const uint8_t *__restrict__ vmask,
                                                       const double *__restrict__ jb, const double *__restrict__ jd,
                                                       double jomega, const double *__restrict__ rb,
                                                       double *__restrict__ x0, const double *__restrict__ xs) {
  static_assert(!XS || J, "start values: fused Jacobi sweep");
  constexpr int BN = 2 * K + 1, P2 = 2 * K, NBND = BN * BN * BN - (BN - 2) * (BN - 2) * (BN - 2);
  const int NX = P2 * nb1 + 1;
  int bx = blockIdx.x, Z = blockIdx.y;
  if (GLS_SLAB_XCD) {
    const int lin = xcd_swizzle((int)(blockIdx.x + gridDim.x * blockIdx.y), (int)(gridDim.x * gridDim.y));
    bx = lin % (int)gridDim.x;
    Z = lin / (int)gridDim.x;
  }
  const bool zs = Z % P2 == 0;
  const int64_t t = (int64_t)bx * blockDim.x + threadIdx.x;
  int X, Y;
  const int ns = nb1 + 1;
  if (zs) {
    if (t >= (int64_t)NX * NX) return;
    X = (int)(t % NX);
    Y = (int)(t / NX);
  } else {
    const int64_t full = (int64_t)ns * NX, sparse = (int64_t)(NX - ns) * ns;
    if (t >= full + sparse) return;
    if (t < full) {
      X = (int)(t % NX);
      Y = (int)(t / NX) * P2;
    } else {
      const int64_t u = t - full;
      const int r = (int)(u / ns);
      X = (int)(u % ns) * P2;
      Y = (r / (P2 - 1)) * P2 + 1 + r % (P2 - 1);
    }
  }
  int bc[3][2], lc[3][2], nc[3];
  const int co[3] = {X, Y, Z};
#pragma unroll
  for (int d = 0; d < 3; ++d) {
    const int x = co[d];
    if (x % P2 == 0 && x > 0 && x < NX - 1) {
      nc[d] = 2;
      bc[d][0] = x / P2 - 1;
      lc[d][0] = P2;
      bc[d][1] = x / P2;
      lc[d][1] = 0;
    } else {
      nc[d] = 1;
      bc[d][0] = min(x / P2, nb1 - 1);
      lc[d][0] = x - P2 * bc[d][0];
      bc[d][1] = bc[d][0];
      lc[d][1] = lc[d][0];
    }
  }
  int64_t sl[8];
  int cnt = 0;
#pragma unroll
  for (int k = 0; k < 2; ++k)
#pragma unroll
    for (int j = 0; j < 2; ++j)
#pragma unroll
      for (int i = 0; i < 2; ++i) {
        const bool on = i < nc[0] && j < nc[1] && k < nc[2];
        const int64_t s = (int64_t)morton3(bc[0][i], bc[1][j], bc[2][k]) * NBND + bnd_index<BN>(lc[0][i], lc[1][j], lc[2][k]);
        sl[i + 2 * j + 4 * k] = on ? s : INT64_MAX;
        cnt += on;
      }
  auto cs = [&](int a, int b) {
    const int64_t lo = min(sl[a], sl[b]), hi = max(sl[a], sl[b]);
    sl[a] = lo;
    sl[b] = hi;
  };
  cs(0, 1); cs(2, 3); cs(4, 5); cs(6, 7);
  cs(0, 2); cs(1, 3); cs(4, 6); cs(5, 7);
  cs(1, 2); cs(5, 6); cs(0, 4); cs(3, 7);
  cs(1, 5); cs(2, 6);
  cs(1, 4); cs(3, 6);
  cs(2, 4); cs(3, 5);
  cs(3, 4);
  double e[8][4];
#pragma unroll
  for (int q = 0; q < 8; ++q)
    if (q < cnt) SlabQuad<S>::load(slab + sl[q] * 4, e[q][0], e[q][1], e[q][2], e[q][3]);
  double s[4] = {0., 0., 0., 0.};
#pragma unroll
  for (int q = 0; q < 8; ++q)
    if (q < cnt) {
      s[0] += e[q][0];
      s[1] += e[q][1];
      s[2] += e[q][2];
      s[3] += e[q][3];
    }
  const int64_t node = X + (int64_t)NX * (Y + (int64_t)NX * Z);
  const int64_t gi[4] = {node * 3, node * 3 + 1, node * 3 + 2, voff + node};
  if constexpr (J) {
    const unsigned m = vmask ? vmask[node] : 0u;
#pragma unroll
    for (int f = 0; f < 4; ++f) {
      const double x = XS ? xs[gi[f]] : y[gi[f]], dd = jd[gi[f]];
      y[gi[f]] = x + jomega * (jb[gi[f]] - ((f < 3 && ((m >> f) & 1u)) ? dd * x : s[f])) / dd;
    }
  } else if (rb) {
#pragma unroll
    for (int f = 0; f < 4; ++f) y[gi[f]] = rb[gi[f]] - s[f];
    if (x0) {
#pragma unroll
      for (int f = 0; f < 4; ++f) x0[gi[f]] = 0.0 + jomega * rb[gi[f]] / jd[gi[f]];
    }
  } else {
#pragma unroll
    for (int f = 0; f < 4; ++f) y[gi[f]] = s[f];
  }
}
hipError_t brick_slab_sum_cube(int k, int nb1, const double *slab, const float *slabf, int64_t n_vnodes, double *y,
                               const uint8_t *vmask, const double *jb, const double *jd, double jomega, hipStream_t s,
                               const double *rb, double *x0, const double *xs) {
  if (nb1 <= 0 || (k != 1 && k != 2)) return hipErrorInvalidValue;
  if (x0 && (!rb || !jd || jb)) return hipErrorInvalidValue;
  if (xs && (k != 2 || !jb || !jd || xs == y)) return hipErrorInvalidValue;
  const int NX = 2 * k * nb1 + 1;
  const dim3 g((unsigned)(((int64_t)NX * NX + 255) / 256), (unsigned)NX), b(256);
  const int64_t voff = 3 * n_vnodes;
  if (xs) {
    if (slabf) hipLaunchKernelGGL((k_slab_sum_cube<float, true, 2, true>), g, b, 0, s, slabf, nb1, voff, y, vmask, jb, jd, jomega, rb, x0, xs);
    else hipLaunchKernelGGL((k_slab_sum_cube<double, true, 2, true>), g, b, 0, s, slab, nb1, voff, y, vmask, jb, jd, jomega, rb, x0, xs);
    return hipGetLastError();
  }
  const double *const no_xs = nullptr;
#define GLS_SLAB_CUBE(KK)                                                                                                  \
  if (slabf) {                                                                                                              \
    if (jb) hipLaunchKernelGGL((k_slab_sum_cube<float, true, KK>), g, b, 0, s, slabf, nb1, voff, y, vmask, jb, jd, jomega, rb, x0, no_xs);  \
    else hipLaunchKernelGGL((k_slab_sum_cube<float, false, KK>), g, b, 0, s, slabf, nb1, voff, y, vmask, jb, jd, jomega, rb, x0, no_xs);   \
  } else {                                                                                                                  \
    if (jb) hipLaunchKernelGGL((k_slab_sum_cube<double, true, KK>), g, b, 0, s, slab, nb1, voff, y, vmask, jb, jd, jomega, rb, x0, no_xs); \
    else hipLaunchKernelGGL((k_slab_sum_cube<double, false, KK>), g, b, 0, s, slab, nb1, voff, y, vmask, jb, jd, jomega, rb, x0, no_xs);  \
  }
  if (k == 1) {
    GLS_SLAB_CUBE(1)
  } else {
    GLS_SLAB_CUBE(2)
  }
#undef GLS_SLAB_CUBE
  return hipGetLastError();
}

__global__ void __launch_bounds__(256) k_restrict_sum_cube(const double *__restrict__ ev, int nb1, int64_t voff,
                                                           double *__restrict__ bc, const uint8_t *__restrict__ vmask) {
  const int NX = 2 * nb1 + 1;
  int bx = blockIdx.x, Z = blockIdx.y;
  if (GLS_SLAB_XCD) {
    const int lin = xcd_swizzle((int)(blockIdx.x + gridDim.x * blockIdx.y), (int)(gridDim.x * gridDim.y));
    bx = lin % (int)gridDim.x;
    Z = lin / (int)gridDim.x;
  }
  const int64_t t = (int64_t)bx * blockDim.x + threadIdx.x;
  if (t >= (int64_t)NX * NX) return;
  const int X = (int)(t % NX), Y = (int)(t / NX);
  int bcd[3][2], lc[3][2], nc[3];
  const int co[3] = {X, Y, Z};
#pragma unroll
  for (int d = 0; d < 3; ++d) {
    const int x = co[d];
    if (x % 2 == 0 && x > 0 && x < NX - 1) {
      nc[d] = 2;
      bcd[d][0] = x / 2 - 1;
      lc[d][0] = 2;
      bcd[d][1] = x / 2;
      lc[d][1] = 0;
    } else {
      nc[d] = 1;
      bcd[d][0] = min(x / 2, nb1 - 1);
      lc[d][0] = x - 2 * bcd[d][0];
      bcd[d][1] = bcd[d][0];
      lc[d][1] = lc[d][0];
    }
  }
  int64_t sl[8];
  int cnt = 0;
#pragma unroll
  for (int k = 0; k < 2; ++k)
#pragma unroll
    for (int j = 0; j < 2; ++j)
#pragma unroll
      for (int i = 0; i < 2; ++i) {
        const bool on = i < nc[0] && j < nc[1] && k < nc[2];
        const int64_t s = (int64_t)morton3(bcd[0][i], bcd[1][j], bcd[2][k]) * 27 + lc[0][i] + 3 * (lc[1][j] + 3 * lc[2][k]);
        sl[i + 2 * j + 4 * k] = on ? s : INT64_MAX;
        cnt += on;
      }
  auto cs = [&](int a, int b) {
    const int64_t lo = min(sl[a], sl[b]), hi = max(sl[a], sl[b]);
    sl[a] = lo;
    sl[b] = hi;
  };
  cs(0, 1); cs(2, 3); cs(4, 5); cs(6, 7);
  cs(0, 2); cs(1, 3); cs(4, 6); cs(5, 7);
  cs(1, 2); cs(5, 6); cs(0, 4); cs(3, 7);
  cs(1, 5); cs(2, 6);
  cs(1, 4); cs(3, 6);
  cs(2, 4); cs(3, 5);
  cs(3, 4);
  double e[8][4];
#pragma unroll
  for (int q = 0; q < 8; ++q)
    if (q < cnt) SlabQuad<double>::load(ev + sl[q] * 4, e[q][0], e[q][1], e[q][2], e[q][3]);
  double s[4] = {0., 0., 0., 0.};
#pragma unroll
  for (int q = 0; q < 8; ++q)
    if (q < cnt) {
      s[0] += e[q][0];
      s[1] += e[q][1];
      s[2] += e[q][2];
      s[3] += e[q][3];
    }
  const int64_t node = X + (int64_t)NX * (Y + (int64_t)NX * Z);
  const unsigned m = vmask ? vmask[node] : 0u;
  bc[node * 3] = (m & 1u) ? 0.0 : s[0];
  bc[node * 3 + 1] = (m & 2u) ? 0.0 : s[1];
  bc[node * 3 + 2] = (m & 4u) ? 0.0 : s[2];
  bc[voff + node] = s[3];
}
hipError_t brick_restrict_sum_cube(int nb1, const double *ev, int64_t n_vnodes, double *bc, const uint8_t *vmask,
                                   hipStream_t s) {
  const int64_t NX = 2 * (int64_t)nb1 + 1;
  if (nb1 <= 0 || nb1 > 1023 || !ev || !bc || NX * NX * NX != n_vnodes) return hipErrorInvalidValue;
  const dim3 g((unsigned)((NX * NX + 255) / 256), (unsigned)NX), b(256);
  hipLaunchKernelGGL(k_restrict_sum_cube, g, b, 0, s, ev, nb1, 3 * n_vnodes, bc, vmask);
  return hipGetLastError();
}

bool brick_fused_jacobi_supported(int k) { return brick_impl(k) == 0 && (k == 1 || k == 2); }
#ifdef GLS_BRICK_COLORS_BUILD
bool brick_colors_supported(int k) { return brick_impl(k) == 0 && (k == 1 || k == 2); }
#else
bool brick_colors_supported(int) { return false; }
#endif
bool brick_subset_supported(int k) { return brick_impl(k) == 0 && (k == 1 || k == 2); }

size_t brick_qdata_size(int k, int n_cells) {
  if (brick_impl(k) == 1) return brick_wave_qdata_size(k, n_cells);
  return k == 1 ? brick_qdata_doubles<1>(n_cells) : (k == 2 ? brick_qdata_doubles<2>(n_cells) : 0);
}

hipError_t launch_brick_kernel(int k, int mode, const OpParams &P, const Tables1D &T, hipStream_t s) {
  if (mode == MODE_DIAG) return hipErrorNotSupported;
  if (brick_impl(k) == 1) return launch_brick_wave(k, mode, P, T, s);
  if (k == 1) return launch_brick_t<1>(mode, P, T, s);
  if (k == 2) return launch_brick_t<2>(mode, P, T, s);
  return hipErrorNotSupported;
}

}
```

softx_2020_200_amd/csrc/gls_ctx.hpp:

```cpp
#pragma once
#include <hip/hip_runtime.h>

#include <array>
#include <cstdint>
#include <memory>
#include <string>
#include <vector>

#include <rocblas/rocblas.h>
#include <rocsparse/rocsparse.h>
#include <rccl/rccl.h>

#include "../../include/gls_native.h"
#include "gls_common.hpp"
#include "gls_devbuf.hpp"
#include "gls_error.hpp"
#include "gls_launch.hpp"
#include "gls_mg_coarse.hpp"

#define RS_TRY(x)                                                                        \
  do {                                                                                   \
    const rocsparse_status rs_ = (x);                                                    \
    if (rs_ != rocsparse_status_success) return ::gls_impl::set_err(GLS_EHIP, "%s: rocsparse status %d", #x, (int)rs_); \
  } while (0)

using gls_impl::DevBuf;

struct gls_ctx {
  int dim = 0, k = 0, kp = 0, nq1d = 0, n_cells = 0, n_vnodes = 0, n_pnodes = 0, nq = 0;
  int64_t n_dofs = 0;
  hipStream_t stream = nullptr;
  bool own_stream = false;
  gls::Tables1D tables;
  DevBuf<int32_t> cell_vnodes, cell_pnodes;
  DevBuf<int32_t> face_nbr;
  DevBuf<double> geo, x0, force_q;
  DevBuf<double> gq;
  DevBuf<double> fd_meas, fd_tab, fd_partial, fd_out;
  std::vector<double> host_x0, host_h, host_support;
  int map_degree = 0;
  DevBuf<uint8_t> vmask;
  DevBuf<int64_t> con_dofs;
  DevBuf<int64_t> dir_dofs;
  DevBuf<double> dir_vals;
  double viscosity = 1.0;
  int srf = 0;
  double omega[3] = {0, 0, 0};
  int scheme = GLS_STEADY;
  double alpha[4] = {0, 0, 0, 0}, alpha_jac = 0., sdt2 = 0.;
  int n_hist = 0;
  const double *u = nullptr, *u1 = nullptr, *u2 = nullptr, *u3 = nullptr;
  DevBuf<double> diag;
  bool diag_valid = false;
  DevBuf<double> qdata;
  bool qd_valid = false;
  DevBuf<double> cq;
  bool cq_valid = false;
  DevBuf<float> qdata32;
  bool qd32_valid = false;
  bool qd32_partial = false;
  DevBuf<double> ev;
  DevBuf<double> bev;
  DevBuf<uint8_t> bact;
  DevBuf<int64_t> ev_voff, ev_vslot, ev_poff, ev_pslot;
  bool smooth_f32 = false;
  bool smooth_oseen = false;
  bool use_qdata = true;
  DevBuf<double> work, scal, coef;
  DevBuf<double> scal2;
  double *hpin = nullptr;
  size_t hpin_n = 0;
  DevBuf<double> krylov;
  DevBuf<double> zbasis;
  DevBuf<double> bicg;
  int krylov_m = 0;
  DevBuf<double> tmp1, tmp2, tmp3, tmp4, tmp5;
  bool use_brick = false;
  bool use_slab = false;
  DevBuf<double> slab;
  DevBuf<double> slab2;
  DevBuf<int32_t> sum_nodes, sum_off, sum_slots;
  int cube_nb1 = 0;
  bool use_colors = false;
  int n_colors = 0;
  int color_off[17] = {0};
  DevBuf<int32_t> color_bricks;
  DevBuf<uint16_t> ncolor;
  DevBuf<double> acc;
  struct Dist {
    bool on = false;
    bool dofs = false;
    int width = 4;
    int64_t n_owned = 0, n_owned_p = 0, n_send = 0, n_recv = 0;
    DevBuf<int32_t> add_u, add_off, add_slot;
    DevBuf<int32_t> send_nodes, recv_nodes;
    double *send_buf = nullptr, *recv_buf = nullptr, *red_buf = nullptr;
    gls_exchange_fn xchg = nullptr;
    gls_allreduce_fn allreduce = nullptr;
    void *user = nullptr;
    ncclComm_t comm = nullptr;
    std::vector<int> nbrs;
    std::vector<int64_t> soff, roff;
    std::vector<int32_t> h_send, h_recv;
    std::vector<int64_t> h_soff, h_roff;
    DevBuf<double> own_send, own_recv, own_red;
    hipStream_t xstream = nullptr;
    hipEvent_t ev_ready = nullptr, ev_done = nullptr;
  } dist;
  DevBuf<int32_t> split;
  int split_bnd = 0, split_int = 0;
  struct ILU {
    bool on = false, valid = false;
    bool probe_only = false;
    double athresh = 0., rthresh = 1.;
    double boost_tol = 0., boost_val = 0.;
    int n_probes = 0, fill = 0;
    int64_t block_dofs = 0;
    int ordering = GLS_ILU_ORDER_CM, n_blocks = 1, n_order_colors = 0;
    bool mc_solve = false;
    bool mc_factor = false;
    bool mc_compact = false;
    DevBuf<double> rdiag;
    std::vector<uint8_t> mc_wl, mc_wu;
    DevBuf<int64_t> mc_desc;
    DevBuf<int64_t> mc_moff;
    DevBuf<uint16_t> mc_map;
    std::vector<int32_t> mc_cg;
    DevBuf<int32_t> mc_grow;
    DevBuf<int64_t> mc_lsp, mc_usp;
    DevBuf<int64_t> ghost_diag;
    bool complete = false;
    int n_rounds = 0;
    std::vector<int64_t> rr;
    DevBuf<int64_t> ru;
    DevBuf<int32_t> ruoff, rslot;
    std::vector<int64_t> pdoff, peoff;
    DevBuf<int32_t> pdofs, prow;
    DevBuf<int64_t> pent;
    DevBuf<int32_t> pdpid, pepid;
    DevBuf<double> bV, bC, bY;
    DevBuf<uint8_t> wact;
    DevBuf<int32_t> wlist;
    std::vector<int64_t> woff;
    int wB = 0;
    int64_t wnblk = 0;
    DevBuf<int64_t> rowp, didx;
    DevBuf<int32_t> col, rowp32;
    DevBuf<int32_t> perm;
    DevBuf<double> val, vbuf, ybuf, tbuf;
    DevBuf<char> work;
    rocsparse_handle h = nullptr;
    rocsparse_mat_descr dA = nullptr, dL = nullptr, dU = nullptr;
    rocsparse_mat_info info = nullptr;
    int64_t nnz = 0, nnz_a = 0;
    void release() {
      if (info) rocsparse_destroy_mat_info(info);
      if (dA) rocsparse_destroy_mat_descr(dA);
      if (dL) rocsparse_destroy_mat_descr(dL);
      if (dU) rocsparse_destroy_mat_descr(dU);
      if (h) rocsparse_destroy_handle(h);
      info = nullptr;
      dA = dL = dU = nullptr;
      h = nullptr;
    }
    ~ILU() { release(); }
  } ilu;
  struct Hang {
    bool on = false;
    DevBuf<int64_t> dof, off, master, ooff, omaster;
    DevBuf<double> w, ow;
    DevBuf<int64_t> tm, toff, tdof;
    DevBuf<double> tw;
    DevBuf<uint8_t> hmask;
    DevBuf<uint8_t> dmask;
    DevBuf<double> vbuf;
    std::vector<int64_t> h_dof, h_off, h_master;
  } hang;
  struct Oct {
    bool on = false;
    int nb = 0;
    DevBuf<int32_t> cell0, list;
    DevBuf<int32_t> rest;
    int n_rest = 0;
    bool f32_next = false;
  } oct;
  struct Lattice {
    bool set = false;
    int n1d = 0, box0[3] = {0, 0, 0}, bdim[3] = {0, 0, 0};
    DevBuf<int32_t> map;
  } lat;
  struct MG {
    bool on = false;
    bool boxed = false;
    std::vector<gls_ctx *> lev;
    std::vector<std::array<int, 3>> dims;
    int k = 2, pre = 2, post = 2, csweeps = 30;
    std::vector<int> lpre, lpost;
    double omega = 0.6, comega = 0.6;
    std::vector<std::unique_ptr<DevBuf<double>>> bufs;
    struct Taps {
      DevBuf<int32_t> pi[3], ri[3], pc[3], rc[3];
      DevBuf<double> pw[3], rw[3];
      bool two_pass = false;
      bool q2_brick = false;
    };
    std::vector<std::unique_ptr<Taps>> taps;
    bool csr = false;
    bool ilu_smooth = false;
    struct Csr {
      DevBuf<int64_t> poff, roff;
      DevBuf<int32_t> pcol, rcol, inj;
      DevBuf<double> pw, rw;
      int64_t nf = 0, nc = 0;
      int plane = 1, rlane = 1;
    };
    std::vector<std::unique_ptr<Csr>> xfer;
    std::vector<gls_ctx *> ilu_levels;
    DevBuf<double> xwork;
    bool direct = false;
    gls_ctx *probe_ilu = nullptr;
    gls_impl::CoarseSolve coarse;
    struct Graph {
      hipGraphExec_t h = nullptr;
      Graph() = default;
      Graph(const Graph &) = delete;
      Graph &operator=(const Graph &) = delete;
      Graph(Graph &&o) noexcept : h(o.h) { o.h = nullptr; }
      Graph &operator=(Graph &&o) noexcept {
        if (this != &o) {
          reset();
          h = o.h;
          o.h = nullptr;
        }
        return *this;
      }
      void reset() {
        if (h) (void)hipGraphExecDestroy(h);
        h = nullptr;
      }
      ~Graph() { reset(); }
    } cgraph;
    std::vector<unsigned char> cgraph_key;
    bool cgraph_failed = false;
    bool dirty = true;
    gls_ctx *replica = nullptr;
    bool rep_csr = false;
    gls_ctx *rep2 = nullptr;
    DevBuf<int64_t> r2p_off, r2r_off;
    DevBuf<int32_t> r2p_col, r2r_col;
    DevBuf<double> r2p_w, r2r_w;
    int r2p_lane = 1, r2r_lane = 1;
    DevBuf<int32_t> r2inj_c, r2inj_f;
    DevBuf<int32_t> rep_own_loc, rep_own_glob;
    DevBuf<int32_t> rep_map;
    DevBuf<double> rep_b, rep_x, rep_tmp, rep_u[4];
  } mg;
  double time_steps[4] = {1, 1, 1, 1};
  struct JacFreeze {
    bool on = false;
    DevBuf<double> u, h[3];
    bool has[3] = {false, false, false};
    double alpha[4] = {0, 0, 0, 0}, alpha_jac = 0., sdt2 = 0., ts[4] = {1, 1, 1, 1};
    int n_hist = 0, scheme = GLS_STEADY;
  } jf;
  int skip_consecutive = 0;
  bool probe_local = false;
  bool sec_on = false;
  double sec_t[GLS_N_SECTIONS] = {};
  int sec_n[GLS_N_SECTIONS] = {};
  bool timing = false;
  struct Ev { int which; hipEvent_t a, b; };
  std::vector<Ev> events;
  double t_ms[6] = {0, 0, 0, 0, 0, 0};
  int64_t t_n[6] = {0, 0, 0, 0, 0, 0};

  ~gls_ctx() {
    if (hpin) (void)hipHostFree(hpin);
    for (auto &e : events) { (void)hipEventDestroy(e.a); (void)hipEventDestroy(e.b); }
    if (dist.ev_ready) (void)hipEventDestroy(dist.ev_ready);
    if (dist.ev_done) (void)hipEventDestroy(dist.ev_done);
    if (dist.xstream) (void)hipStreamDestroy(dist.xstream);
    if (own_stream && stream) (void)hipStreamDestroy(stream);
  }
};

namespace gls_impl {

inline int check_ctx(gls_ctx *c) {
  if (!c) return set_err(GLS_EINVAL, "null context");
  return GLS_OK;
}

gls::OpParams make_params(gls_ctx *c, bool jac = false);

struct TimedLaunch {
  gls_ctx *c;
  int which;
  hipEvent_t a = nullptr, b = nullptr;
  TimedLaunch(gls_ctx *c_, int w) : c(c_), which(w) {
    if (c->timing) {
      (void)hipEventCreate(&a);
      (void)hipEventCreate(&b);
      (void)hipEventRecord(a, c->stream);
    }
  }
  ~TimedLaunch() {
    if (c->timing) {
      (void)hipEventRecord(b, c->stream);
      c->events.push_back({which, a, b});
    }
  }
};

void gauss_points(int n, double *x, double *w);
void lobatto_points(int k, double *x);
void lagrange_1d(int k, const double *xn, int i, double s, double &v, double &d, double &dd);
double corner_measure(int dim, int md, const double *S);
int ensure_element_maps(gls_ctx *c);
int ensure_diag(gls_ctx *c);
inline bool cell_cache_on(const gls_ctx *c) {
  return !c->use_brick && c->n_cells > 0;
}
inline size_t cell_cache_size(const gls_ctx *c) {
  const int dim = c->dim;
  return (size_t)c->n_cells * (size_t)gls::ipow(c->nq1d, dim) * (size_t)(dim + dim * dim + 1 + dim);
}

double *brick_slab(gls_ctx *c);
int dist_import(gls_ctx *c, double *x);
int dist_export_add(gls_ctx *c, double *y);
int dist_allreduce_vector(gls_ctx *c, double *v, int64_t n);
int ensure_qdata(gls_ctx *c);
int ensure_qdata32(gls_ctx *g, bool full = true);
bool slab_f32();
bool first_sweep_fusable(gls_ctx *g);
int jacobian_apply_f32(gls_ctx *g, const double *v, double *y, const double *rb = nullptr, double first_omega = 0.0,
                       bool oseen = false);
int smoother_apply(gls_ctx *g, const double *v, double *y, const double *rb = nullptr);
int smoother_sweep(gls_ctx *g, double *x, const double *b, double *y, double omega, double *z = nullptr,
                   const double *pxc = nullptr);

int mg_prepare(gls_ctx *c);
int mg_vcycle(gls_ctx *c, int l, const double *b, double *x);
int mg_vcycle_rep2(gls_ctx *c, const double *b, double *x);

int ilu_probe(gls_ctx *c);
int ensure_ilu(gls_ctx *c);
int apply_ilu(gls_ctx *c, const double *v, double *z);

int rccl_exchange_on(gls_ctx *c, int phase, hipStream_t stream);

}
```

softx_2020_200_amd/csrc/gls_launch.hpp:

```cpp
#pragma once
#include "gls_common.hpp"

namespace gls {

hipError_t gather_element_vectors(double *y, const double *ev, const int64_t *voff, const int64_t *vslot, int64_t nv,
                                  const int64_t *poff, const int64_t *pslot, int64_t np, int dim, hipStream_t s);
hipError_t launch_cell_kernel(int dim, int k, int kp, int nq1d, int mode, const OpParams &P, const Tables1D &T,
                              hipStream_t s);
bool cell_kernel_supported(int dim, int k, int kp, int nq1d);
hipError_t launch_cell_sf_jv(int dim, int k, int kp, int nq1d, const OpParams &P, const Tables1D &T, hipStream_t s);
bool cell_sf_enabled();
int cell_kernel_cells_per_block(int dim, int k, int nq1d, bool probe = false);
hipError_t launch_brick_kernel(int k, int mode, const OpParams &P, const Tables1D &T, hipStream_t s);
size_t brick_qdata_size(int k, int n_cells);
hipError_t launch_brick_jv_f32(int k, const OpParams &P, const Tables1D &T, hipStream_t s);
hipError_t vec_to_f32(const double *a, float *b, int64_t n, hipStream_t s);
hipError_t vec_from_f32(const float *a, double *b, int64_t n, hipStream_t s);
hipError_t launch_pencil_jv(const OpParams &P, const Tables1D &T, hipStream_t s, bool f32);
hipError_t launch_pencil_jv_restrict(const OpParams &P, const Tables1D &T, hipStream_t s);
hipError_t launch_pencil_jv_prolong(const OpParams &P, const Tables1D &T, hipStream_t s);
hipError_t launch_pencil_residual(const OpParams &P, const Tables1D &T, hipStream_t s);
hipError_t launch_pencil_lin(const OpParams &P, const Tables1D &T, hipStream_t s);
hipError_t launch_pencil_reslin(const OpParams &P, const Tables1D &T, hipStream_t s);
hipError_t launch_pencil_ev(int mode, const OpParams &P, const Tables1D &T, hipStream_t s, bool f32 = false);
bool pencil_enabled();
hipError_t launch_brick_wave(int k, int mode, const OpParams &P, const Tables1D &T, hipStream_t s);
hipError_t launch_brick_wave_jv_f32(int k, const OpParams &P, const Tables1D &T, hipStream_t s);
hipError_t launch_brick_wave_probe(int k, const OpParams &P, const Tables1D &T, int64_t j0, int nprobe, hipStream_t s);
size_t brick_wave_qdata_size(int k, int n_cells);

int brick_boundary_nodes(int k);
hipError_t brick_slab_sum(const double *slab, const int32_t *nodes, const int32_t *off, const int32_t *slots,
                          int64_t n_sum, int64_t n_vnodes, double *y, hipStream_t s);
hipError_t brick_slab_sum_ex(const double *slab, const float *slabf, const int32_t *nodes, const int32_t *off,
                             const int32_t *slots, int64_t n_sum, int64_t n_vnodes, double *y, const uint8_t *vmask,
                             const double *jb, const double *jd, double jomega, hipStream_t s,
                             const double *rb = nullptr);
hipError_t brick_slab_sum_cube(int k, int nb1, const double *slab, const float *slabf, int64_t n_vnodes, double *y,
                               const uint8_t *vmask, const double *jb, const double *jd, double jomega, hipStream_t s,
                               const double *rb = nullptr, double *x0 = nullptr,
                               const double *xs = nullptr);
hipError_t brick_restrict_sum_cube(int nb1, const double *ev, int64_t n_vnodes, double *bc, const uint8_t *vmask,
                                   hipStream_t s);
bool brick_fused_jacobi_supported(int k);
bool brick_colors_supported(int k);
bool brick_subset_supported(int k);
hipError_t launch_brick_probe(int k, const OpParams &P, const Tables1D &T, int64_t j0, int nprobe, hipStream_t s);

hipError_t vec_fill(double *x, int64_t n, double a, hipStream_t s);
hipError_t vec_copy(double *y, const double *x, int64_t n, hipStream_t s);
hipError_t vec_axpy(double *y, double a, const double *x, int64_t n, hipStream_t s);
hipError_t vec_axpby(double *y, double a, const double *x, double b, int64_t n, hipStream_t s);
hipError_t vec_scale(double *x, double a, int64_t n, hipStream_t s);
hipError_t vec_div(double *y, const double *x, const double *d, int64_t n, hipStream_t s);
hipError_t vec_multidot(const double *A, int64_t lda, int nk, const double *w, int64_t n, double *out,
                        double *work, hipStream_t s);
hipError_t vec_multidot2(const double *A, int64_t lda, int nk, const double *w, int64_t n1, int64_t off2, int64_t n2,
                         double *out, double *work, hipStream_t s);
hipError_t vec_pack_nodes(const double *x, const int32_t *nodes, int64_t m, int64_t voff, double *buf, hipStream_t s);
hipError_t vec_unpack_nodes(double *x, const int32_t *nodes, int64_t m, int64_t voff, const double *buf, int add,
                            hipStream_t s);
hipError_t vec_multiaxpy(double *w, const double *A, int64_t lda, int nk, const double *h, double sign, int64_t n,
                         hipStream_t s, bool zero_init = false);
hipError_t vec_waxpy(double *w, const double *y, double a, const double *x, int64_t n, hipStream_t s);
hipError_t vec_multiaxpy_dots(double *w, const double *A, int64_t lda, int nk, const double *h, double sign, int64_t n,
                              int64_t n1, int64_t off2, int64_t n2, bool dots, double scale, double *out,
                              double *work, hipStream_t s);
hipError_t vec_csr_gather_set(double *x, const double *src, const int64_t *dof, const int64_t *off,
                              const int64_t *master, const double *w, int64_t n, hipStream_t s);
hipError_t vec_copy_gather_set(double *x, const double *v, const uint8_t *dmask, int64_t n, const int64_t *dof,
                               const int64_t *off, const int64_t *master, const double *w, int64_t nl, hipStream_t s);
hipError_t vec_csr_condense(double *y, const int64_t *tm, const int64_t *toff, const int64_t *tdof, const double *tw,
                            int64_t n, hipStream_t s);
hipError_t vec_csr_spmv(double *y, const double *x, const int64_t *off, const int32_t *col, const double *w, int64_t n,
                        bool add, hipStream_t s, int lanes = 1);
hipError_t vec_gather_scale_set(double *y, const double *d, const double *v, const int64_t *idx, int64_t m,
                                hipStream_t s, const double *rb = nullptr);
hipError_t vec_set_const_indexed(double *x, const int32_t *idx, int64_t m, double a, hipStream_t s);
hipError_t csr_probe_extract(double *val, const int64_t *ent, const int32_t *row, int64_t m, const double *y,
                             hipStream_t s, bool add = false);
hipError_t csr_to_dense(double *A, const int64_t *rowp, const int32_t *col, const double *val, const int32_t *perm,
                        const int32_t *inv, int64_t n, hipStream_t s);
hipError_t vec_permute(double *out, const double *in, const int32_t *idx, int64_t n, int dir, hipStream_t s);
hipError_t probe_set_batched(double *V, int64_t n, const int32_t *dofs, const int32_t *pid, int p0, int64_t m,
                             hipStream_t s);
hipError_t probe_extract_batched(double *val, const int64_t *ent, const int32_t *row, const int32_t *pid, int p0,
                                 int64_t m, const double *Y, int64_t n, hipStream_t s);
hipError_t vec_csr_gather_set_b(double *x, const int64_t *dof, const int64_t *off, const int64_t *master,
                                const double *w, int64_t n, int nb, int64_t bs, hipStream_t s);
hipError_t vec_csr_condense_b(double *y, const int64_t *tm, const int64_t *toff, const int64_t *tdof, const double *tw,
                              int64_t n, int nb, int64_t bs, hipStream_t s);
hipError_t vec_gather_scale_set_b(double *y, const double *d, const double *v, const int64_t *idx, int64_t m, int nb,
                                  int64_t bs, hipStream_t s);
hipError_t gather_element_vectors_b(double *y, const double *ev, const int64_t *voff, const int64_t *vslot, int64_t nv,
                                    const int64_t *poff, const int64_t *pslot, int64_t np, int dim, int nb, int64_t ys,
                                    int64_t evs, const uint8_t *act, int64_t el, int cb, int nblk, hipStream_t s);
constexpr int kMaxGroupRows = 4;
constexpr int kIluMaxRow = 640;
constexpr int kIluCompactRow = 448;
hipError_t ilu_mc_factor(const int32_t *grow, const int32_t *color_groups, int n_colors, const int64_t *rowp,
                         const int32_t *col, double *val, const int64_t *lsp, const int64_t *didx, double boost_tol,
                         double boost_val, const int64_t *moff, const uint16_t *map, bool compact, double *rdiag,
                         hipStream_t s);
hipError_t ilu_mc_factor_map(int64_t n, const int64_t *rowp, const int32_t *col, const int64_t *lsp,
                             const int64_t *didx, const int64_t *moff, uint16_t *map, hipStream_t s);
constexpr int kGroupDesc = 24;
hipError_t ilu_mc_solve(const int64_t *gdesc, const int32_t *color_groups, int n_colors, const int32_t *col,
                        const double *val, const double *b, double *y, double *x, const uint8_t *waves_lower,
                        const uint8_t *waves_upper, hipStream_t s);
hipError_t vec_pack_dofs(const double *x, const int32_t *dofs, int64_t m, double *buf, hipStream_t s);
hipError_t vec_unpack_dofs(double *x, const int32_t *dofs, int64_t m, const double *buf, hipStream_t s);
hipError_t vec_add_dofs_ordered(double *x, const int32_t *u, const int32_t *off, const int32_t *slot, int64_t n,
                                const double *buf, hipStream_t s);
hipError_t vec_add_nodes_ordered(double *x, const int32_t *u, const int32_t *off, const int32_t *slot, int64_t n,
                                 int64_t voff, const double *buf, hipStream_t s);
hipError_t csr_diag_perturb(double *val, const int64_t *didx, int64_t n, double athresh, double rthresh, hipStream_t s);
hipError_t vec_set_const_indexed64(double *x, const int64_t *idx, int64_t m, double a, hipStream_t s);
hipError_t vec_add_pos_ordered(double *x, const int64_t *u, const int32_t *off, const int32_t *slot, int64_t n,
                               const double *buf, hipStream_t s);
hipError_t vec_set_indexed(double *y, const int64_t *idx, const double *vals, int64_t m, hipStream_t s);
int multidot_work_size();

struct KellyTables {
  int nq;
  double w[kMaxQ1D];
  double V[kMaxQ1D][kMaxNodes1D];
  double De[2][kMaxNodes1D];
  double xq[kMaxQ1D];
  double xn[kMaxNodes1D];
};
hipError_t launch_kelly_faces(int dim, int m, const int32_t *cell_nodes, const double *geo, const double *sol,
                              int64_t n_faces, const int32_t *fa, const int32_t *fb, const int32_t *fdir,
                              const double *rect_a, const double *rect_b, int ncomp, int64_t base, int stride,
                              const KellyTables &T, double *fint, hipStream_t s);
hipError_t launch_kelly_mapped(int dim, int m, const int32_t *cell_nodes, const double *sol, int64_t n_pieces, int nqf,
                               const int32_t *ca, const int32_t *cb, const double *xi, const double *g,
                               const double *jxw, int ncomp, int64_t base, int stride, const KellyTables &T,
                               double *fint, hipStream_t s);
hipError_t launch_kelly(int dim, int m, const int32_t *cell_nodes, const int32_t *nbr, const double *geo,
                        const double *sol, int n_cells, int ncomp, int64_t base, int stride, const KellyTables &T,
                        double *eta, hipStream_t s);

int64_t boundary_loads_blocks(int64_t n_pts);
bool boundary_loads_supported(int dim, int k, int kp);
hipError_t launch_boundary_loads(int dim, int k, int kp, const int32_t *cell_vnodes, const int32_t *cell_pnodes,
                                 const double *sol, int64_t pbase, int64_t n_pts, int nqf, const int32_t *fcell,
                                 const int32_t *fslot, const double *xi, const double *jinv, const double *normal,
                                 const double *jxw, const double *xq, double nu, const double *cor, int n_slots,
                                 double *partial, double *out, hipStream_t s);

int64_t flow_diagnostics_blocks(int64_t n_cells);
bool flow_diagnostics_supported(int dim, int k, int kp);
hipError_t launch_flow_diagnostics(int dim, int k, const int32_t *cell_vnodes, const double *geo, const double *gq,
                                   const double *meas, const double *tab, const double *sol, int64_t n_cells, double dt,
                                   double *partial, double *out, hipStream_t s);

bool output_fields_supported(int dim, int k, int kp, int map_degree, int subdivision);
hipError_t launch_output_fields(int dim, int k, int kp, int map_degree, int subdivision, const int32_t *cell_vnodes,
                                const int32_t *cell_pnodes, const double *sol, int64_t pbase, const double *x0h,
                                const double *support, const double *tab, int64_t n_cells, int srf, const double *omega,
                                double *pts, double *vel, double *pre, double *vort, double *qcr, double *eul,
                                hipStream_t s);

namespace expr {
struct DeviceProgram;
}
bool l2_error_supported(int dim, int k, int kp, int map_degree, int max_stack);
int64_t l2_error_blocks(int dim, int k, int kp, int map_degree, int max_stack, int64_t n_cells);
hipError_t launch_l2_error(int dim, int k, int kp, int map_degree, const int32_t *cell_vnodes, const int32_t *cell_pnodes,
                           const double *sol, int64_t pbase, const double *x0h, const double *support, const double *tab,
                           int64_t n_cells, const expr::DeviceProgram &exact, double time, double volume, double *partial,
                           double *out, hipStream_t s);

hipError_t mg_inject(const double *fine, double *coarse, const int nf[3], const int nc[3], hipStream_t s);
hipError_t mg_transfer3d(const double *in, double *out, const int nin[3], const int nout[3],
                         const int32_t *const taps[3], const double *const w[3], const int32_t *const cnt[3],
                         hipStream_t s);
hipError_t mg_transfer_2pass(const double *in, double *out, const int nin[3], const int nout[3], int restrict_,
                             const int32_t *const taps[3], const double *const w[3], const int32_t *const cnt[3],
                             double *work, hipStream_t s, int add = 0);
int mg_transfer_tile_fits(int restrict_, int axis, int n_out, const int32_t *taps, const int32_t *cnt);
hipError_t mg_box_gather(const double *loc, double *box, const int32_t *map, int64_t nbox, int64_t nvl,
                         int64_t n_owned, hipStream_t s);
hipError_t mg_box_scatter(const double *box, double *loc, const int32_t *map, int64_t nbox, int64_t nvl,
                          hipStream_t s);
hipError_t mg_dense_invert(const double *Y, double *aug, int n, int *status, hipStream_t s);
hipError_t mg_unit_step(double *e, int64_t j, hipStream_t s);
hipError_t mg_probe_fix(double *Y, int64_t n, int64_t j0, int nprobe, const int64_t *con, int64_t ncon, const double *d,
                        hipStream_t s);
hipError_t mg_dense_apply(const double *aug, int n, const double *b, double *x, hipStream_t s);
hipError_t mg_pin_dof(double *A, int64_t n, int64_t pin, hipStream_t s);
hipError_t mg_zero_row(double *A, int64_t n, int64_t row, hipStream_t s);
hipError_t dense_lu_solve_f32(const float *LU, int n, float *x, hipStream_t s, int bl = -1, int bu = -1);
hipError_t mg_jacobi_update(double *x, const double *b, const double *y, const double *d, double omega, int64_t n,
                            int zero_start, hipStream_t s);

}
```

softx_2020_200_amd/csrc/gls_mg.cpp:

```cpp
#include <algorithm>
#include <array>
#include <cmath>
#include <cstdio>
#include <cstdlib>
#include <cstring>
#include <memory>
#include <vector>

#include "gls_ctx.hpp"

using namespace gls_impl;

namespace {
enum { MB_U = 0, MB_U1, MB_U2, MB_U3, MB_B, MB_X, MB_Y, MB_BOX, MB_N };
double *mgbuf(gls_ctx *c, int l, int which) { return c->mg.bufs[(size_t)l * MB_N + which]->p; }
int64_t mg_nbox(const gls_ctx *c, int l) {
  const auto &d = c->mg.dims[(size_t)l];
  return (int64_t)d[0] * d[1] * d[2];
}
const double *mg_to_box(gls_ctx *c, int l, const double *loc, bool owned_only) {
  if (!c->mg.boxed) return loc;
  gls_ctx *g = c->mg.lev[(size_t)l];
  double *box = mgbuf(c, l, MB_BOX);
  if (gls::mg_box_gather(loc, box, g->lat.map.p, mg_nbox(c, l), g->n_vnodes, owned_only ? g->dist.n_owned : -1,
// ... 125 lines not shown
  const int batch = 4096;
  for (int64_t j0 = 0; j0 < n; j0 += batch) {
    const int nb = (int)std::min<int64_t>(batch, n - j0);
    P.y = A + j0 * n;
    HIP_TRY(gls::launch_brick_probe(g->k, P, g->tables, j0, nb, c->stream));
    HIP_TRY(gls::mg_probe_fix(A + j0 * n, n, j0, nb, g->con_dofs.p, (int64_t)g->con_dofs.n, g->diag.p, c->stream));
  }
  return GLS_OK;
}
int mg_probe_band(gls_ctx *c, gls_ctx *g) {
  auto &cs = c->mg.coarse;
  const auto &I = g->ilu;
  const int64_t n = g->n_dofs;
  std::vector<int64_t> rp((size_t)n + 1);
  std::vector<int32_t> cl((size_t)I.nnz), pm((size_t)n), id((size_t)n);
  HIP_TRY(hipMemcpy(rp.data(), I.rowp.p, sizeof(int64_t) * rp.size(), hipMemcpyDeviceToHost));
  HIP_TRY(hipMemcpy(cl.data(), I.col.p, sizeof(int32_t) * cl.size(), hipMemcpyDeviceToHost));
  HIP_TRY(hipMemcpy(pm.data(), I.perm.p, sizeof(int32_t) * pm.size(), hipMemcpyDeviceToHost));
  int64_t bl = 0, bu = 0;
  for (int64_t r = 0; r < n; ++r)
    for (int64_t e = rp[(size_t)r]; e < rp[(size_t)r + 1]; ++e) {
      bl = std::max<int64_t>(bl, r - cl[(size_t)e]);
      bu = std::max<int64_t>(bu, cl[(size_t)e] - r);
    }
  for (int64_t i = 0; i < n; ++i) id[(size_t)i] = (int32_t)i;
  GLS_TRY(cs.ident.upload(id.data(), id.size()));
  cs.band = {bl, bu, pm[(size_t)((int64_t)g->dim * g->n_vnodes)]};
  if (std::getenv("GLS_MG_VERBOSE"))
    std::printf("mg: coarse matrix n=%lld in Cuthill-McKee order: bandwidths %lld / %lld\n", (long long)n, (long long)bl,
                (long long)bu);
  return GLS_OK;
}
int mg_probe_ilu_csr(gls_ctx *c, gls_ctx *g, double *A, bool *banded) {
  auto &cs = c->mg.coarse;
  const int64_t n = g->n_dofs;
  GLS_TRY(ensure_diag(g));
  GLS_TRY(ilu_probe(g));
  HIP_TRY(hipMemsetAsync(A, 0, sizeof(double) * (size_t)(n * n), c->stream));
  const auto &I = g->ilu;
  *banded = n > kDirectSmall;
  if (*banded && cs.band.bl < 0) GLS_TRY(mg_probe_band(c, g));
  HIP_TRY(gls::csr_to_dense(A, I.rowp.p, I.col.p, I.val.p, *banded ? cs.ident.p : I.perm.p, cs.pinv.p, n, c->stream));
  return GLS_OK;
}
int mg_probe_columns(gls_ctx *c, gls_ctx *g, double *A) {
  const int64_t n = g->n_dofs;
  double *unit = c->mg.coarse.unit.p;
  HIP_TRY(gls::vec_fill(unit, n, 0.0, c->stream));
  for (int64_t j = 0; j < n; ++j) {
    HIP_TRY(gls::mg_unit_step(unit, j, c->stream));
    GLS_TRY(gls_jacobian_apply(g, unit, A + j * n));
  }
  return GLS_OK;
}
}

namespace gls_impl {
int mg_prepare(gls_ctx *c) {
  auto &mg = c->mg;
  if (!mg.dirty) return GLS_OK;
  GLS_TRY(mg.coarse.finish(c->stream));
  if (std::getenv("GLS_MG_VERBOSE")) (void)hipStreamSynchronize(c->stream);
  const auto t0 = CoarseSolve::Clock::now();
  GLS_TRY(mg_prepare_levels(c));
  mg.coarse.ok = false;
  if (mg.direct) {
    gls_ctx *g = mg.rep_csr ? mg.rep2 : mg.lev.back();
    double *A = mg.coarse.matrix();
    bool banded = false;
    if (g->use_brick && g->use_qdata) GLS_TRY(mg_probe_brick(c, g, A));
    else if (mg.probe_ilu == g && g->ilu.on) GLS_TRY(mg_probe_ilu_csr(c, g, A, &banded));
    else GLS_TRY(mg_probe_columns(c, g, A));
    GLS_TRY(mg.coarse.factor(c->stream, (int64_t)g->dim * g->n_vnodes, banded, t0));
  }
  mg.dirty = false;
  return GLS_OK;
}
}

namespace {
int mg_restrict(gls_ctx *c, int l, const double *y, double *bc) {
  auto &mg = c->mg;
  gls_ctx *h = mg.lev[(size_t)l + 1];
  hipStream_t s = c->stream;
  if (mg.csr) {
    const auto &X = *mg.xfer[(size_t)l];
    HIP_TRY(gls::vec_csr_spmv(bc, y, X.roff.p, X.rcol.p, X.rw.p, X.nc, false, s, X.rlane));
    (void)h;
    return GLS_OK;
  }
  const double *yb = mg_to_box(c, l, y, true);
  if (!yb) return set_err(GLS_EHIP, "mg box gather failed");
  {
    const auto &T = *mg.taps[(size_t)l];
    const int32_t *ti[3] = {T.ri[0].p, T.ri[1].p, T.ri[2].p}, *tc[3] = {T.rc[0].p, T.rc[1].p, T.rc[2].p};
    const double *tw[3] = {T.rw[0].p, T.rw[1].p, T.rw[2].p};
    if (T.two_pass)
      HIP_TRY(gls::mg_transfer_2pass(yb, mg_box_target(c, l + 1, bc), mg.dims[l].data(), mg.dims[l + 1].data(), 1, ti,
                                     tw, tc, mg.xwork.p, s));
    else
      HIP_TRY(gls::mg_transfer3d(yb, mg_box_target(c, l + 1, bc), mg.dims[l].data(), mg.dims[l + 1].data(), ti, tw,
                                 tc, s));
  }
  GLS_TRY(mg_from_box(c, l + 1, bc));
  GLS_TRY(dist_export_add(h, bc));
  return GLS_OK;
}

bool mg_prolong_add_ok(gls_ctx *c, int l) {
  if (c->mg.csr) return false;
  return !c->mg.boxed && c->mg.taps[(size_t)l]->two_pass && std::getenv("GLS_MG_NO_FUSE") == nullptr;
}
int mg_prolong(gls_ctx *c, int l, double *xc, double *y, bool add = false) {
  auto &mg = c->mg;
  gls_ctx *h = mg.lev[(size_t)l + 1];
  hipStream_t s = c->stream;
  if (mg.csr) {
    const auto &X = *mg.xfer[(size_t)l];
    HIP_TRY(gls::vec_csr_spmv(y, xc, X.poff.p, X.pcol.p, X.pw.p, X.nf, add, s, X.plane));
    return GLS_OK;
  }
  GLS_TRY(dist_import(h, xc));
  const double *xb = mg_to_box(c, l + 1, xc, false);
  if (!xb) return set_err(GLS_EHIP, "mg box gather failed");
  {
    const auto &T = *mg.taps[(size_t)l];
    const int32_t *ti[3] = {T.pi[0].p, T.pi[1].p, T.pi[2].p}, *tc[3] = {T.pc[0].p, T.pc[1].p, T.pc[2].p};
    const double *tw[3] = {T.pw[0].p, T.pw[1].p, T.pw[2].p};
    if (T.two_pass)
      HIP_TRY(gls::mg_transfer_2pass(xb, mg_box_target(c, l, y), mg.dims[l + 1].data(), mg.dims[l].data(), 0, ti, tw,
                                     tc, mg.xwork.p, s, add ? 1 : 0));
    else if (add)
      return set_err(GLS_EINVAL, "mg_prolong: accumulate needs the two-pass transfer");
    else
      HIP_TRY(gls::mg_transfer3d(xb, mg_box_target(c, l, y), mg.dims[l + 1].data(), mg.dims[l].data(), ti, tw, tc, s));
  }
  GLS_TRY(mg_from_box(c, l, y));
  return GLS_OK;
}

bool mg_fused_restrict_ok(gls_ctx *c, int l) {
  auto &mg = c->mg;
  if (l < 0 || l + 1 >= (int)mg.lev.size() || mg.csr || mg.boxed || (size_t)l >= mg.taps.size()) return false;
  const char *e = std::getenv("GLS_MG_FUSE_TRANSFER");
  if ((e && std::atoi(e) == 0) || std::getenv("GLS_MG_NO_FUSE") != nullptr) return false;
  gls_ctx *g = mg.lev[(size_t)l], *h = mg.lev[(size_t)l + 1];
  const auto &T = *mg.taps[(size_t)l];
  const int64_t nc1 = 2 * (int64_t)g->cube_nb1 + 1;
  return T.two_pass && T.q2_brick && g->smooth_f32 && g->use_brick && g->use_qdata && !g->use_colors && !g->dist.on &&
         !g->hang.on && !g->oct.on && g->k == 2 && g->cube_nb1 > 0 && g->cube_nb1 < 1024 && g->use_slab && !g->srf &&
         gls::pencil_enabled() && gls::brick_fused_jacobi_supported(g->k) && !h->dist.on && !h->hang.on &&
         h->n_vnodes == nc1 * nc1 * nc1 && g->stream == c->stream;
}
int mg_residual_restrict_fused(gls_ctx *c, int l, double *x, const double *b, double *bc, double first_omega = 0.0) {
  gls_ctx *g = c->mg.lev[(size_t)l], *h = c->mg.lev[(size_t)l + 1];
  if (!g->u) return set_err(GLS_EINVAL, "gls_set_state was not called");
  GLS_TRY(ensure_diag(g));
  GLS_TRY(ensure_qdata32(g, !g->smooth_oseen));
  gls::OpParams P = make_params(g, true);
  P.qdf = g->qdata32.p;
  P.oseen = g->smooth_oseen ? 1 : 0;
  P.v = x;
  P.rb = b;
  P.cube_nb1 = g->cube_nb1;
  if (first_omega > 0.0) {
    P.jx0 = x;
    P.jd = g->diag.p;
    P.jomega = first_omega;
  }
  P.slab = brick_slab(g);
  if (!P.slab) return set_err(GLS_EHIP, "brick slab allocation failed");
  {
    TimedLaunch t(g, 4);
    HIP_TRY(gls::launch_pencil_jv_restrict(P, g->tables, c->stream));
  }
  TimedLaunch t(g, 5);
  HIP_TRY(gls::brick_restrict_sum_cube(g->cube_nb1, P.slab, h->n_vnodes, bc, h->vmask.p, c->stream));
  return GLS_OK;
}

bool mg_fused_prolong_ok(gls_ctx *c, int l) {
  auto &mg = c->mg;
  if (l < 0 || l + 1 >= (int)mg.lev.size() || mg.csr || mg.boxed || (size_t)l >= mg.taps.size() || !mg_prolong_add_ok(c, l))
    return false;
  const char *e = std::getenv("GLS_MG_FUSE_PROLONG");
  if (e && std::atoi(e) == 0) return false;
  gls_ctx *g = mg.lev[(size_t)l], *h = mg.lev[(size_t)l + 1];
  const auto &T = *mg.taps[(size_t)l];
  const int64_t nc1 = 2 * (int64_t)g->cube_nb1 + 1;
  const bool ilu_smooth = mg.ilu_smooth && g->ilu.on && !g->ilu.probe_only;
  return T.two_pass && T.q2_brick && mg.lpost[(size_t)l] >= 1 && !ilu_smooth && g->smooth_f32 && g->use_brick &&
         g->use_qdata && !g->use_colors && !g->dist.on && !g->hang.on && !g->oct.on && g->k == 2 && g->cube_nb1 > 0 &&
         g->cube_nb1 < 1024 && g->use_slab && brick_slab(g) && !g->srf && gls::pencil_enabled() &&
         gls::brick_fused_jacobi_supported(g->k) && !h->dist.on && !h->hang.on && h->cube_nb1 > 0 &&
         g->cube_nb1 == 2 * h->cube_nb1 && h->n_vnodes == nc1 * nc1 * nc1 && g->stream == c->stream;
}

bool coarse_graph_eligible(gls_ctx *c, gls_ctx *g, const double *b, const double *x) {
  const int l = (int)c->mg.lev.size() - 1;
  return !c->mg.cgraph_failed && !c->mg.boxed && !g->dist.on && !g->hang.on && g->use_brick && g->use_qdata &&
         brick_slab(g) && gls::brick_fused_jacobi_supported(g->k) && g->stream == c->stream &&
         b == mgbuf(c, l, MB_B) && x == mgbuf(c, l, MB_X) && std::getenv("GLS_MG_NO_FUSE") == nullptr &&
         std::getenv("GLS_MG_GRAPH") != nullptr;
}
std::vector<unsigned char> coarse_graph_key(gls_ctx *g, const double *b, const double *x, const double *y,
                                                   int pre, double om) {
  const gls::OpParams P = make_params(g);
  const void *ptrs[7] = {b, x, y, g->diag.p, g->qdata.p, g->qdata32.p, brick_slab(g)};
  const int64_t ints[4] = {pre, g->n_dofs, (int64_t)g->smooth_f32, (int64_t)slab_f32()};
  std::vector<unsigned char> k(sizeof(P) + sizeof(ptrs) + sizeof(ints) + sizeof(om));
  unsigned char *o = k.data();
  std::memcpy(o, &P, sizeof(P));
  std::memcpy(o += sizeof(P), ptrs, sizeof(ptrs));
  std::memcpy(o += sizeof(ptrs), ints, sizeof(ints));
  std::memcpy(o + sizeof(ints), &om, sizeof(om));
  return k;
}
int coarse_graph_capture(gls_ctx *c, gls_ctx *g, const double *b, double *x, double *y, int pre, double om) {
  auto &mg = c->mg;
  hipStream_t s = c->stream;
  GLS_TRY(ensure_diag(g));
  GLS_TRY(g->smooth_f32 ? ensure_qdata32(g, !g->smooth_oseen) : ensure_qdata(g));
  if (g->use_colors && g->acc.n != (size_t)g->n_dofs) GLS_TRY(g->acc.alloc((size_t)g->n_dofs));
  const bool tim = g->timing;
  g->timing = false;
  hipGraph_t gr = nullptr;
  int rc = GLS_OK;
  hipError_t e = hipStreamBeginCapture(s, hipStreamCaptureModeThreadLocal);
  if (e == hipSuccess) {
    if (hipError_t e1 = gls::mg_jacobi_update(x, b, nullptr, g->diag.p, om, g->n_dofs, 1, s); e1 != hipSuccess)
      e = e1;
    for (int it = 1; it < pre && rc == GLS_OK && e == hipSuccess; ++it) rc = smoother_sweep(g, x, b, y, om);
    const hipError_t e2 = hipStreamEndCapture(s, &gr);
    if (e == hipSuccess) e = e2;
  }
  g->timing = tim;
  hipGraphExec_t ex = nullptr;
  if (rc == GLS_OK && e == hipSuccess && gr) e = hipGraphInstantiate(&ex, gr, nullptr, nullptr, 0);
  if (gr) (void)hipGraphDestroy(gr);
  if (rc != GLS_OK || e != hipSuccess || !ex) {
    (void)hipGetLastError();
    if (ex) (void)hipGraphExecDestroy(ex);
    mg.cgraph_failed = true;
    if (std::getenv("GLS_MG_VERBOSE")) std::printf("mg: coarse graph capture refused (%s)\n", hipGetErrorString(e));
    return GLS_OK;
  }
  mg.cgraph.h = ex;
  mg.cgraph_key = coarse_graph_key(g, b, x, y, pre, om);
  return GLS_OK;
}

int mg_presmooth(gls_ctx *g, hipStream_t s, int pre, double om, double *zs, const double *b, double *x, double *y,
                 bool residual) {
  const int64_t n = g->n_dofs;
  if (pre > 0 && zs) {
    GLS_TRY(ensure_ilu(g));
    GLS_TRY(apply_ilu(g, b, x));
    for (int it = 1; it < pre; ++it) GLS_TRY(smoother_sweep(g, x, b, y, om, zs));
  } else if (pre > 0) {
    HIP_TRY(gls::mg_jacobi_update(x, b, nullptr, g->diag.p, om, n, 1, s));
    for (int it = 1; it < pre; ++it) GLS_TRY(smoother_sweep(g, x, b, y, om));
  } else {
    HIP_TRY(gls::vec_fill(x, n, 0.0, s));
  }
  if (!residual) return GLS_OK;
  if (pre > 0) return smoother_apply(g, x, y, b);
  HIP_TRY(gls::vec_copy(y, b, n, s));
  return GLS_OK;
}
int mg_coarse_solve(gls_ctx *c, gls_ctx *g, const double *b, double *x) {
  auto &mg = c->mg;
  if (const int rc = mg.coarse.finish(c->stream); rc < 0) {
    mg.dirty = true;
    return rc;
  }
  return mg.coarse.solve(c->stream, b, x, g->ilu.perm.p);
}
}

namespace gls_impl {
int mg_vcycle_rep2(gls_ctx *c, const double *b, double *x) {
  auto &mg = c->mg;
  gls_ctx *r = mg.rep2;
  const int64_t n = c->n_dofs, ng = r->n_dofs;
  hipStream_t s = c->stream;
  GLS_TRY(ensure_diag(c));
  double *y = mgbuf(c, 0, MB_Y);
  double *zs = mg.ilu_smooth && c->ilu.on && !c->ilu.probe_only ? mgbuf(c, 0, MB_BOX) : nullptr;
  const int pre = mg.lpre[0], post = mg.lpost[0];
  GLS_TRY(mg_presmooth(c, s, pre, mg.omega, zs, b, x, y, true));
  HIP_TRY(gls::vec_csr_spmv(mg.rep_b.p, y, mg.r2r_off.p, mg.r2r_col.p, mg.r2r_w.p, ng, false, s, mg.r2r_lane));
  GLS_TRY(dist_allreduce_vector(c, mg.rep_b.p, ng));
  HIP_TRY(gls::vec_set_indexed(mg.rep_b.p, r->con_dofs.p, nullptr, (int64_t)r->con_dofs.n, s));
  if (mg.coarse.ok) {
    GLS_TRY(mg_coarse_solve(c, r, mg.rep_b.p, mg.rep_x.p));
  } else {
    GLS_TRY(gls_apply_preconditioner(r, mg.rep_b.p, mg.rep_x.p));
  }
  HIP_TRY(gls::vec_csr_spmv(y, mg.rep_x.p, mg.r2p_off.p, mg.r2p_col.p, mg.r2p_w.p, n, false, s, mg.r2p_lane));
  HIP_TRY(gls::vec_set_indexed(y, c->con_dofs.p, nullptr, (int64_t)c->con_dofs.n, s));
  HIP_TRY(gls::vec_axpy(x, 1.0, y, n, s));
  for (int it = 0; it < post; ++it) GLS_TRY(smoother_sweep(c, x, b, y, mg.omega, zs));
  return GLS_OK;
}

int mg_vcycle(gls_ctx *c, int l, const double *b, double *x) {
  auto &mg = c->mg;
  const int L = (int)mg.lev.size();
  gls_ctx *g = mg.lev[l];
  GLS_TRY(ensure_diag(g));
  const int64_t n = g->n_dofs;
  double *y = mgbuf(c, l, MB_Y);
  hipStream_t s = c->stream;
  if (l == L - 1 && mg.replica) {
    GLS_TRY(replica_gather(c, b, mg.rep_b.p));
    GLS_TRY(gls_apply_preconditioner(mg.replica, mg.rep_b.p, mg.rep_x.p));
    HIP_TRY(gls::vec_pack_dofs(mg.rep_x.p, mg.rep_map.p, n, x, c->stream));
    return GLS_OK;
  }
  if (l == L - 1 && mg.coarse.ok) return mg_coarse_solve(c, g, b, x);
  const int pre = l == L - 1 ? mg.csweeps : mg.lpre[(size_t)l];
  const double om = l == L - 1 ? mg.comega : mg.omega;
  if (l == L - 1 && l > 0 && pre > 1 && coarse_graph_eligible(c, g, b, x)) {
    GLS_TRY(ensure_diag(g));
    GLS_TRY(g->smooth_f32 ? ensure_qdata32(g, !g->smooth_oseen) : ensure_qdata(g));
    if (mg.cgraph.h && mg.cgraph_key != coarse_graph_key(g, b, x, y, pre, om)) mg.cgraph.reset();
    if (!mg.cgraph.h) GLS_TRY(coarse_graph_capture(c, g, b, x, y, pre, om));
    if (mg.cgraph.h) {
      HIP_TRY(hipGraphLaunch(mg.cgraph.h, s));
      return GLS_OK;
    }
  }
  const bool first_fused = pre == 1 && l < L - 1 && first_sweep_fusable(g);
  double *zs = mg.ilu_smooth && g->ilu.on && !g->ilu.probe_only ? mgbuf(c, l, MB_BOX) : nullptr;
  const bool fused_restrict = l < L - 1 && pre > 0 && mg_fused_restrict_ok(c, l);
  if (!first_fused) GLS_TRY(mg_presmooth(g, s, pre, om, zs, b, x, y, l < L - 1 && !fused_restrict));
  if (l == L - 1) return GLS_OK;
  gls_ctx *h = mg.lev[l + 1];
  double *bc = mgbuf(c, l + 1, MB_B), *xc = mgbuf(c, l + 1, MB_X);
  if (fused_restrict) {
    GLS_TRY(mg_residual_restrict_fused(c, l, x, b, bc, first_fused ? om : 0.0));
  } else {
    if (first_fused) GLS_TRY(jacobian_apply_f32(g, x, y, b, om, g->smooth_oseen));
    GLS_TRY(mg_restrict(c, l, y, bc));
    HIP_TRY(gls::vec_set_indexed(bc, h->con_dofs.p, nullptr, (int64_t)h->con_dofs.n, s));
  }
  GLS_TRY(mg_vcycle(c, l + 1, bc, xc));
  const bool pro = mg_fused_prolong_ok(c, l);
  if (pro) {
  } else if (mg_prolong_add_ok(c, l)) {
    GLS_TRY(mg_prolong(c, l, xc, x, true));
  } else {
    GLS_TRY(mg_prolong(c, l, xc, y));
    HIP_TRY(gls::vec_set_indexed(y, g->con_dofs.p, nullptr, (int64_t)g->con_dofs.n, s));
    HIP_TRY(gls::vec_axpy(x, 1.0, y, n, s));
  }
  for (int it = 0; it < mg.lpost[(size_t)l]; ++it)
    GLS_TRY(smoother_sweep(g, x, b, y, mg.omega, zs, pro && it == 0 ? xc : nullptr));
  return GLS_OK;
}
}

extern "C" {

int gls_mg_transfer(gls_ctx *c, int level, int direction, const double *in, double *out) {
  GLS_TRY(check_ctx(c));
  auto &mg = c->mg;
  if (!mg.on) return set_err(GLS_EINVAL, "gls_mg_transfer: no multigrid attached");
  if (level < 0 || level + 1 >= (int)mg.lev.size() || (direction != 0 && direction != 1) || !in || !out || in == out)
    return set_err(GLS_EINVAL, "gls_mg_transfer: bad level / direction / pointers");
  if (direction == 0) return mg_restrict(c, level, in, out);
  double *xc = mgbuf(c, level + 1, MB_X);
  HIP_TRY(gls::vec_copy(xc, in, mg.lev[(size_t)level + 1]->n_dofs, c->stream));
  return mg_prolong(c, level, xc, out);
}

int gls_mg_residual_restrict(gls_ctx *c, int level, const double *x, const double *b, double *bc, int *fused) {
  GLS_TRY(check_ctx(c));
  auto &mg = c->mg;
  if (!mg.on) return set_err(GLS_EINVAL, "gls_mg_residual_restrict: no multigrid attached");
  if (level < 0 || level + 1 >= (int)mg.lev.size() || !x || !b || !bc)
    return set_err(GLS_EINVAL, "gls_mg_residual_restrict: bad level / pointers");
  GLS_TRY(mg_prepare(c));
  const bool f = mg_fused_restrict_ok(c, level);
  if (fused) *fused = f ? 1 : 0;
  if (f) return mg_residual_restrict_fused(c, level, const_cast<double *>(x), b, bc);
  gls_ctx *g = mg.lev[(size_t)level], *h = mg.lev[(size_t)level + 1];
  double *y = mgbuf(c, level, MB_Y);
  GLS_TRY(smoother_apply(g, x, y, b));
  GLS_TRY(mg_restrict(c, level, y, bc));
  HIP_TRY(gls::vec_set_indexed(bc, h->con_dofs.p, nullptr, (int64_t)h->con_dofs.n, c->stream));
  return GLS_OK;
}

int gls_mg_prolong_smooth(gls_ctx *c, int level, const double *xc, double *x, const double *b, double omega, int *fused) {
  GLS_TRY(check_ctx(c));
  auto &mg = c->mg;
  if (!mg.on) return set_err(GLS_EINVAL, "gls_mg_prolong_smooth: no multigrid attached");
  if (level < 0 || level + 1 >= (int)mg.lev.size() || !xc || !x || !b || x == b || omega < 0.0)
    return set_err(GLS_EINVAL, "gls_mg_prolong_smooth: bad level / pointers / omega");
  GLS_TRY(mg_prepare(c));
  gls_ctx *g = mg.lev[(size_t)level];
  const bool f = mg_fused_prolong_ok(c, level);
  if (fused) *fused = f ? 1 : 0;
  double *y = mgbuf(c, level, MB_Y);
  double *zs = mg.ilu_smooth && g->ilu.on && !g->ilu.probe_only ? mgbuf(c, level, MB_BOX) : nullptr;
  double *xcw = mgbuf(c, level + 1, MB_X);
  if (xcw != xc) HIP_TRY(gls::vec_copy(xcw, xc, mg.lev[(size_t)level + 1]->n_dofs, c->stream));
  if (f) return smoother_sweep(g, x, b, y, omega, zs, xcw);
  if (mg_prolong_add_ok(c, level)) {
    GLS_TRY(mg_prolong(c, level, xcw, x, true));
  } else {
    GLS_TRY(mg_prolong(c, level, xcw, y));
    HIP_TRY(gls::vec_set_indexed(y, g->con_dofs.p, nullptr, (int64_t)g->con_dofs.n, c->stream));
    HIP_TRY(gls::vec_axpy(x, 1.0, y, g->n_dofs, c->stream));
  }
  return smoother_sweep(g, x, b, y, omega, zs);
}


int gls_set_lattice(gls_ctx *c, int n1d, const int64_t *l2g) {
  GLS_TRY(check_ctx(c));
  if (c->dim != 3 || n1d < 2 || !l2g) return set_err(GLS_EINVAL, "gls_set_lattice: 3D, n1d >= 2, map required");
  int lo[3] = {n1d, n1d, n1d}, hi[3] = {-1, -1, -1};
  for (int i = 0; i < c->n_vnodes; ++i) {
    const int64_t g = l2g[i];
    if (g < 0 || g >= (int64_t)n1d * n1d * n1d) return set_err(GLS_EINVAL, "lattice node out of range");
    const int x[3] = {(int)(g % n1d), (int)((g / n1d) % n1d), (int)(g / ((int64_t)n1d * n1d))};
    for (int a = 0; a < 3; ++a) { lo[a] = std::min(lo[a], x[a]); hi[a] = std::max(hi[a], x[a]); }
  }
  int bd[3];
  for (int a = 0; a < 3; ++a) bd[a] = hi[a] - lo[a] + 1;
  const int64_t nbox = (int64_t)bd[0] * bd[1] * bd[2];
  if (nbox != c->n_vnodes) return set_err(GLS_EINVAL, "local nodes do not fill a box (%lld != %d)", (long long)nbox, c->n_vnodes);
  std::vector<int32_t> map((size_t)nbox, -1);
  for (int i = 0; i < c->n_vnodes; ++i) {
    const int64_t g = l2g[i];
    const int64_t x = g % n1d - lo[0], y = (g / n1d) % n1d - lo[1], z = g / ((int64_t)n1d * n1d) - lo[2];
    int32_t &m = map[(size_t)((z * bd[1] + y) * bd[0] + x)];
    if (m >= 0) return set_err(GLS_EINVAL, "duplicate lattice node");
    m = i;
  }
  GLS_TRY(c->lat.map.upload(map.data(), map.size()));
  c->lat.n1d = n1d;
  for (int a = 0; a < 3; ++a) { c->lat.box0[a] = lo[a]; c->lat.bdim[a] = bd[a]; }
  c->lat.set = true;
  return GLS_OK;
}

static int mg_attach_common(gls_ctx *c, const gls_mg_params *p) {
  auto &mg = c->mg;
  mg.k = c->k;
  mg.pre = p->pre_smooth > 0 ? p->pre_smooth : (p->pre_smooth < 0 ? 0 : 2);
  mg.post = p->post_smooth >= 0 ? p->post_smooth : 2;
  mg.csweeps = p->coarse_sweeps > 0 ? p->coarse_sweeps : 30;
  mg.omega = p->omega > 0 ? p->omega : 0.6;
  mg.comega = p->coarse_omega > 0 ? p->coarse_omega : mg.omega;
  mg.lpre.assign((size_t)p->n_levels, mg.pre);
  mg.lpost.assign((size_t)p->n_levels, mg.post);
  if (p->level_sweeps)
    for (int l = 0; l < p->n_levels; ++l) {
      if (p->level_sweeps[2 * l] < 0 || p->level_sweeps[2 * l + 1] < 0) return set_err(GLS_EINVAL, "mg: negative level sweeps");
      mg.lpre[(size_t)l] = p->level_sweeps[2 * l];
      mg.lpost[(size_t)l] = p->level_sweeps[2 * l + 1];
    }
  for (auto *g : mg.lev) g->smooth_f32 = p->mixed_precision != 0;
  {
    const bool os = p->smoother_operator == 1;
    if (p->smoother_operator < 0 || p->smoother_operator > 1) return set_err(GLS_EINVAL, "mg: smoother_operator 0 or 1");
    for (auto *g : mg.lev) g->smooth_oseen = os && g->smooth_f32;
  }
  mg.ilu_smooth = p->smoother == 1 || p->smoother == 2;
  if (p->smoother < 0 || p->smoother > 2 || (mg.ilu_smooth && !mg.csr))
    return set_err(GLS_EINVAL, "mg: smoother 0 (Jacobi), 1 (ILU) or 2 (ILU below the finest level; gls_mg_attach_transfers hierarchies)");
  for (int l = 0; l < p->n_levels; ++l)
    for (int b = 0; b < MB_N; ++b) {
      mg.bufs.emplace_back(new DevBuf<double>());
      const bool need = b == MB_BOX ? (mg.boxed || mg.ilu_smooth) : (l > 0 || b == MB_Y);
      if (need)
        GLS_TRY(mg.bufs.back()->alloc(b == MB_BOX && mg.boxed ? (size_t)(4 * mg_nbox(c, l)) : (size_t)mg.lev[l]->n_dofs));
    }
  if (mg.ilu_smooth)
    for (int l = p->smoother == 2 ? 1 : 0; l + 1 < p->n_levels; ++l) {
      gls_ctx *g = mg.lev[(size_t)l];
      GLS_TRY(gls_ilu_set_options(g, GLS_ILU_ORDER_MULTICOLOR, 0));
      GLS_TRY(gls_ilu_attach(g, 0, 1e-12, 1.0));
      mg.ilu_levels.push_back(g);
    }
  {
    const int64_t nco = mg.lev.back()->n_dofs;
    const int want = p->coarse_direct;
    if (want > 0 && (mg.boxed || nco > kDirectMax))
      return set_err(GLS_EINVAL, "mg: direct coarse solve needs one GPU, <= %lld DoFs", (long long)kDirectMax);
    mg.direct = want > 0 || (want == 0 && !mg.boxed && nco <= 2048);
    if (mg.direct) {
      GLS_TRY(mg.coarse.init(nco));
      GLS_TRY(mg_probe_setup(c, mg.lev.back()));
    }
  }
  mg.on = true;
// ... 308 lines not shown
```

softx_2020_200_amd/csrc/gls_vector_kernels.hip:

```cpp
#include <algorithm>
#include <cstdint>
#include <cstdlib>
#include "gls_launch.hpp"

namespace gls {

namespace {
constexpr int kBlock = 256;
constexpr int kMaxBlocks = 2048;
constexpr int kDotChunk = 8;

inline int grid_for(int64_t n) {
  int64_t b = (n + kBlock - 1) / kBlock;
  return (int)(b < kMaxBlocks ? (b > 0 ? b : 1) : kMaxBlocks);
}

__global__ void k_fill(double *x, int64_t n, double a) {
  for (int64_t i = blockIdx.x * (int64_t)blockDim.x + threadIdx.x; i < n; i += (int64_t)gridDim.x * blockDim.x) x[i] = a;
}
__global__ void k_copy(double *__restrict__ y, const double *__restrict__ x, int64_t n) {
  for (int64_t i = blockIdx.x * (int64_t)blockDim.x + threadIdx.x; i < n; i += (int64_t)gridDim.x * blockDim.x) y[i] = x[i];
}
__global__ void k_axpy(double *__restrict__ y, double a, const double *__restrict__ x, int64_t n) {
  for (int64_t i = blockIdx.x * (int64_t)blockDim.x + threadIdx.x; i < n; i += (int64_t)gridDim.x * blockDim.x)
// ... 39 lines not shown
    const int64_t i = ii < n1 ? ii : off2 + (ii - n1);
    const double wi = w[i];
#pragma unroll
    for (int k = 0; k < NK; ++k) acc[k] += A[k * lda + i] * wi;
  }
  __shared__ double red[NK][kBlock / 64];
  const int lane = threadIdx.x & 63, wv = threadIdx.x >> 6;
#pragma unroll
  for (int k = 0; k < NK; ++k) {
    const double s = wave_sum(acc[k]);
    if (lane == 0) red[k][wv] = s;
  }
  __syncthreads();
  if (threadIdx.x < NK) {
    double s = 0.;
#pragma unroll
    for (int j = 0; j < kBlock / 64; ++j) s += red[threadIdx.x][j];
    work[threadIdx.x * gridDim.x + blockIdx.x] = s;
  }
}

__global__ void __launch_bounds__(kBlock) k_reduce_rows(const double *work, int nb, double *out) {
  double s = 0.;
  for (int b = threadIdx.x; b < nb; b += blockDim.x) s += work[blockIdx.x * nb + b];
  __shared__ double red[kBlock / 64];
  s = wave_sum(s);
  if ((threadIdx.x & 63) == 0) red[threadIdx.x >> 6] = s;
  __syncthreads();
  if (threadIdx.x == 0) {
    double t = 0.;
    for (int j = 0; j < kBlock / 64; ++j) t += red[j];
    out[blockIdx.x] = t;
  }
}

template <int NK>
__global__ void __launch_bounds__(kBlock) k_multiaxpy(double *__restrict__ w, const double *__restrict__ A, int64_t lda,
                                                      const double *__restrict__ h, double sign, int64_t n) {
  double hk[NK];
#pragma unroll
  for (int k = 0; k < NK; ++k) hk[k] = sign * h[k];
  for (int64_t i = blockIdx.x * (int64_t)blockDim.x + threadIdx.x; i < n; i += (int64_t)gridDim.x * blockDim.x) {
    double s = w[i];
#pragma unroll
    for (int k = 0; k < NK; ++k) s -= hk[k] * A[k * lda + i];
    w[i] = s;
  }
}

template <int NK, bool DOTS>
__global__ void __launch_bounds__(kBlock) k_multiaxpy_dot(double *__restrict__ w, const double *__restrict__ A,
                                                          int64_t lda, const double *__restrict__ h, double sign,
                                                          int64_t n, int64_t n1, int64_t off2, int64_t n2,
                                                          double scale, double *work) {
  constexpr int ND = (DOTS ? NK : 0) + 1;
  double hk[NK], acc[ND];
#pragma unroll
  for (int k = 0; k < NK; ++k) hk[k] = sign * h[k];
#pragma unroll
  for (int d = 0; d < ND; ++d) acc[d] = 0.;
  for (int64_t i = blockIdx.x * (int64_t)blockDim.x + threadIdx.x; i < n; i += (int64_t)gridDim.x * blockDim.x) {
    double a[NK];
#pragma unroll
    for (int k = 0; k < NK; ++k) a[k] = A[k * lda + i];
    double s = w[i];
#pragma unroll
    for (int k = 0; k < NK; ++k) s -= hk[k] * a[k];
    s *= scale;
    w[i] = s;
    if (i < n1 || (i >= off2 && i < off2 + n2)) {
      if constexpr (DOTS) {
#pragma unroll
        for (int k = 0; k < NK; ++k) acc[k] += a[k] * s;
      }
      acc[ND - 1] += s * s;
    }
  }
  __shared__ double red[ND][kBlock / 64];
  const int lane = threadIdx.x & 63, wv = threadIdx.x >> 6;
#pragma unroll
  for (int d = 0; d < ND; ++d) {
    const double t = wave_sum(acc[d]);
    if (lane == 0) red[d][wv] = t;
  }
  __syncthreads();
  if (threadIdx.x < ND) {
    double t = 0.;
#pragma unroll
    for (int j = 0; j < kBlock / 64; ++j) t += red[threadIdx.x][j];
    work[threadIdx.x * gridDim.x + blockIdx.x] = t;
  }
}

typedef double dbl2 __attribute__((ext_vector_type(2)));
template <int NK, bool ZERO>
__global__ void __launch_bounds__(kBlock) k_multiaxpy16(double *__restrict__ w, const double *__restrict__ A, int64_t lda,
                                                        const double *__restrict__ h, double sign, int64_t n) {
  double hk[NK];
#pragma unroll
  for (int k = 0; k < NK; ++k) hk[k] = sign * h[k];
  const int64_t np = n / 2;
  for (int64_t p = blockIdx.x * (int64_t)blockDim.x + threadIdx.x; p < np; p += (int64_t)gridDim.x * blockDim.x) {
    dbl2 s = ZERO ? dbl2{0.0, 0.0} : reinterpret_cast<const dbl2 *>(w)[p];
#pragma unroll
    for (int k = 0; k < NK; ++k) {
      const dbl2 a = __builtin_nontemporal_load(reinterpret_cast<const dbl2 *>(A + k * lda) + p);
      s.x -= hk[k] * a.x;
      s.y -= hk[k] * a.y;
    }
    reinterpret_cast<dbl2 *>(w)[p] = s;
  }
  if ((n & 1) && blockIdx.x == 0 && threadIdx.x == 0) {
    double s = ZERO ? 0.0 : w[n - 1];
#pragma unroll
    for (int k = 0; k < NK; ++k) s -= hk[k] * A[k * lda + n - 1];
    w[n - 1] = s;
  }
}

template <int NK>
__global__ void __launch_bounds__(kBlock) k_multidot16(const double *__restrict__ A, int64_t lda,
                                                       const double *__restrict__ w, int64_t n, double *work) {
  double acc[NK];
#pragma unroll
  for (int k = 0; k < NK; ++k) acc[k] = 0.;
  const int64_t np = n / 2;
  for (int64_t p = blockIdx.x * (int64_t)blockDim.x + threadIdx.x; p < np; p += (int64_t)gridDim.x * blockDim.x) {
    const dbl2 wi = __builtin_nontemporal_load(reinterpret_cast<const dbl2 *>(w) + p);
#pragma unroll
    for (int k = 0; k < NK; ++k) {
      const dbl2 a = __builtin_nontemporal_load(reinterpret_cast<const dbl2 *>(A + k * lda) + p);
      acc[k] += a.x * wi.x;
      acc[k] += a.y * wi.y;
    }
  }
  if ((n & 1) && blockIdx.x == 0 && threadIdx.x == 0)
#pragma unroll
    for (int k = 0; k < NK; ++k) acc[k] += A[k * lda + n - 1] * w[n - 1];
  __shared__ double red[NK][kBlock / 64];
  const int lane = threadIdx.x & 63, wv = threadIdx.x >> 6;
#pragma unroll
  for (int k = 0; k < NK; ++k) {
    const double t = wave_sum(acc[k]);
    if (lane == 0) red[k][wv] = t;
  }
  __syncthreads();
  if (threadIdx.x < NK) {
    double t = 0.;
#pragma unroll
    for (int j = 0; j < kBlock / 64; ++j) t += red[threadIdx.x][j];
    work[threadIdx.x * gridDim.x + blockIdx.x] = t;
  }
}
template <int NK, bool DOTS>
__global__ void __launch_bounds__(kBlock) k_multiaxpy_dot16(double *__restrict__ w, const double *__restrict__ A,
                                                            int64_t lda, const double *__restrict__ h, double sign,
                                                            int64_t n, double scale, double *work) {
  constexpr int ND = (DOTS ? NK : 0) + 1;
  double hk[NK], acc[ND];
#pragma unroll
  for (int k = 0; k < NK; ++k) hk[k] = sign * h[k];
#pragma unroll
  for (int d = 0; d < ND; ++d) acc[d] = 0.;
  auto row = [&](double wi, const double *a) {
    double s = wi;
#pragma unroll
    for (int k = 0; k < NK; ++k) s -= hk[k] * a[k];
    s *= scale;
    if constexpr (DOTS) {
#pragma unroll
      for (int k = 0; k < NK; ++k) acc[k] += a[k] * s;
    }
    acc[ND - 1] += s * s;
    return s;
  };
  const int64_t np = n / 2;
  for (int64_t p = blockIdx.x * (int64_t)blockDim.x + threadIdx.x; p < np; p += (int64_t)gridDim.x * blockDim.x) {
    double a0[NK], a1[NK];
#pragma unroll
    for (int k = 0; k < NK; ++k) {
      const dbl2 a = __builtin_nontemporal_load(reinterpret_cast<const dbl2 *>(A + k * lda) + p);
      a0[k] = a.x;
      a1[k] = a.y;
    }
    const dbl2 wi = reinterpret_cast<const dbl2 *>(w)[p];
    const double o0 = row(wi.x, a0), o1 = row(wi.y, a1);
    reinterpret_cast<dbl2 *>(w)[p] = dbl2{o0, o1};
  }
  if ((n & 1) && blockIdx.x == 0 && threadIdx.x == 0) {
    double a[NK];
#pragma unroll
    for (int k = 0; k < NK; ++k) a[k] = A[k * lda + n - 1];
    w[n - 1] = row(w[n - 1], a);
  }
  __shared__ double red[ND][kBlock / 64];
  const int lane = threadIdx.x & 63, wv = threadIdx.x >> 6;
#pragma unroll
  for (int d = 0; d < ND; ++d) {
    const double t = wave_sum(acc[d]);
    if (lane == 0) red[d][wv] = t;
  }
  __syncthreads();
  if (threadIdx.x < ND) {
    double t = 0.;
#pragma unroll
    for (int j = 0; j < kBlock / 64; ++j) t += red[threadIdx.x][j];
    work[threadIdx.x * gridDim.x + blockIdx.x] = t;
  }
}
bool vec16(const double *A, int64_t lda, const double *w, int64_t n, int64_t n1, int64_t n2) {
  return n2 == 0 && n1 == n && (lda % 2) == 0 && ((uintptr_t)A % 16) == 0 && ((uintptr_t)w % 16) == 0;
}

__global__ void k_csr_gather_set(double *x, const double *src, const int64_t *__restrict__ dof,
                                 const int64_t *__restrict__ off, const int64_t *__restrict__ master,
                                 const double *__restrict__ w, int64_t n, int64_t bs = 0) {
  x += blockIdx.y * bs;
  src += blockIdx.y * bs;
  for (int64_t i = blockIdx.x * (int64_t)blockDim.x + threadIdx.x; i < n; i += (int64_t)gridDim.x * blockDim.x) {
    double s = 0.;
    for (int64_t j = off[i]; j < off[i + 1]; ++j) s += w[j] * src[master[j]];
    x[dof[i]] = s;
  }
}
__global__ void k_csr_spmv(double *__restrict__ y, const double *__restrict__ x, const int64_t *__restrict__ off,
                           const int32_t *__restrict__ col, const double *__restrict__ w, int64_t n, int add) {
  for (int64_t i = blockIdx.x * (int64_t)blockDim.x + threadIdx.x; i < n; i += (int64_t)gridDim.x * blockDim.x) {
    double s = 0.;
    for (int64_t j = off[i]; j < off[i + 1]; ++j) s += w[j] * x[col[j]];
    y[i] = add ? y[i] + s : s;
  }
}
__global__ void k_csr_condense(double *y, const int64_t *__restrict__ tm, const int64_t *__restrict__ toff,
                               const int64_t *__restrict__ tdof, const double *__restrict__ tw, int64_t n, int64_t bs = 0) {
  y += blockIdx.y * bs;
  constexpr int kIn = 8;
  for (int64_t i = blockIdx.x * (int64_t)blockDim.x + threadIdx.x; i < n; i += (int64_t)gridDim.x * blockDim.x) {
    const int64_t j0 = toff[i], nj = toff[i + 1] - j0;
    double s = 0.;
    if (nj <= kIn) {
      int64_t r[kIn];
      double w[kIn], v[kIn];
#pragma unroll
      for (int t = 0; t < kIn; ++t) {
        r[t] = t < nj ? tdof[j0 + t] : -1;
        w[t] = t < nj ? tw[j0 + t] : 0.;
      }
#pragma unroll
      for (int t = 0; t < kIn; ++t) v[t] = r[t] >= 0 ? y[r[t]] : 0.;
#pragma unroll
      for (int t = 0; t < kIn; ++t)
        if (t < nj) s += w[t] * v[t];
    } else {
      for (int64_t j = j0; j < j0 + nj; ++j) s += tw[j] * y[tdof[j]];
    }
    y[tm[i]] += s;
  }
}

__global__ void k_gather_scale_set(double *y, const double *d, const double *v, const int64_t *idx, int64_t m,
                                   const double *rb, int64_t bs = 0) {
  y += blockIdx.y * bs;
  v += blockIdx.y * bs;
  for (int64_t j = blockIdx.x * (int64_t)blockDim.x + threadIdx.x; j < m; j += (int64_t)gridDim.x * blockDim.x) {
    const int64_t i = idx[j];
    y[i] = rb ? rb[i] - d[i] * v[i] : d[i] * v[i];
  }
}
__global__ void k_pack_nodes(const double *__restrict__ x, const int32_t *__restrict__ nodes, int64_t m, int64_t voff,
                             double *__restrict__ buf) {
  for (int64_t j = blockIdx.x * (int64_t)blockDim.x + threadIdx.x; j < m; j += (int64_t)gridDim.x * blockDim.x) {
    const int64_t n = nodes[j];
    buf[j * 4 + 0] = x[n * 3 + 0];
    buf[j * 4 + 1] = x[n * 3 + 1];
    buf[j * 4 + 2] = x[n * 3 + 2];
    buf[j * 4 + 3] = x[voff + n];
  }
}
__global__ void k_unpack_nodes(double *__restrict__ x, const int32_t *__restrict__ nodes, int64_t m, int64_t voff,
                               const double *__restrict__ buf, int add) {
  for (int64_t j = blockIdx.x * (int64_t)blockDim.x + threadIdx.x; j < m; j += (int64_t)gridDim.x * blockDim.x) {
    const int64_t n = nodes[j];
    if (add) {
      atomicAdd(&x[n * 3 + 0], buf[j * 4 + 0]);
      atomicAdd(&x[n * 3 + 1], buf[j * 4 + 1]);
      atomicAdd(&x[n * 3 + 2], buf[j * 4 + 2]);
      atomicAdd(&x[voff + n], buf[j * 4 + 3]);
    } else {
      x[n * 3 + 0] = buf[j * 4 + 0];
      x[n * 3 + 1] = buf[j * 4 + 1];
      x[n * 3 + 2] = buf[j * 4 + 2];
      x[voff + n] = buf[j * 4 + 3];
    }
  }
}
__global__ void k_set_indexed(double *y, const int64_t *idx, const double *vals, int64_t m) {
  for (int64_t j = blockIdx.x * (int64_t)blockDim.x + threadIdx.x; j < m; j += (int64_t)gridDim.x * blockDim.x)
    y[idx[j]] = vals ? vals[j] : 0.0;
}
}

int multidot_work_size() { return (kDotChunk + 1) * kMaxBlocks; }

__global__ void k_gather_ev(double *__restrict__ y, const double *__restrict__ ev, const int64_t *__restrict__ voff,
                            const int64_t *__restrict__ vslot, int64_t nv, const int64_t *__restrict__ poff,
                            const int64_t *__restrict__ pslot, int64_t np, int dim, int64_t ys = 0, int64_t evs = 0,
                            const uint8_t *__restrict__ act = nullptr, int64_t el = 1, int cb = 1, int nblk = 0) {
  y += blockIdx.y * ys;
  ev += blockIdx.y * evs;
  if (act) act += (int64_t)blockIdx.y * nblk;
  auto live = [&](int64_t slot) { return !act || act[slot / el / cb]; };
  const int64_t i = (int64_t)blockIdx.x * blockDim.x + threadIdx.x;
  constexpr int kIn = 8;
  if (i < nv && voff[i + 1] - voff[i] <= kIn) {
    const int64_t j0 = voff[i], nj = voff[i + 1] - j0;
    int64_t sl[kIn];
#pragma unroll
    for (int t = 0; t < kIn; ++t) sl[t] = t < nj ? vslot[j0 + t] : -1;
    if (act) {
#pragma unroll
      for (int t = 0; t < kIn; ++t) sl[t] = sl[t] >= 0 && live(sl[t]) ? sl[t] : -1;
    }
    double e[kIn][3];
#pragma unroll
    for (int t = 0; t < kIn; ++t)
#pragma unroll
      for (int c = 0; c < 3; ++c) e[t][c] = (sl[t] >= 0 && c < dim) ? ev[sl[t] + c] : 0.;
    double acc[3] = {0., 0., 0.};
#pragma unroll
    for (int t = 0; t < kIn; ++t)
      if (sl[t] >= 0)
#pragma unroll
        for (int c = 0; c < 3; ++c) acc[c] += e[t][c];
    for (int c = 0; c < dim; ++c) y[i * dim + c] = acc[c];
  } else if (i < nv) {
    double acc[3] = {0., 0., 0.};
    for (int64_t j = voff[i]; j < voff[i + 1]; ++j) {
      if (!live(vslot[j])) continue;
      const double *e = ev + vslot[j];
      for (int c = 0; c < dim; ++c) acc[c] += e[c];
    }
    for (int c = 0; c < dim; ++c) y[i * dim + c] = acc[c];
  } else if (i < nv + np && poff[i - nv + 1] - poff[i - nv] <= kIn) {
    const int64_t q = i - nv, j0 = poff[q], nj = poff[q + 1] - j0;
    int64_t sl[kIn];
#pragma unroll
    for (int t = 0; t < kIn; ++t) sl[t] = t < nj ? pslot[j0 + t] : -1;
    if (act) {
#pragma unroll
      for (int t = 0; t < kIn; ++t) sl[t] = sl[t] >= 0 && live(sl[t]) ? sl[t] : -1;
    }
    double e[kIn];
#pragma unroll
    for (int t = 0; t < kIn; ++t) e[t] = sl[t] >= 0 ? ev[sl[t]] : 0.;
    double acc = 0.;
#pragma unroll
    for (int t = 0; t < kIn; ++t)
      if (sl[t] >= 0) acc += e[t];
    y[dim * nv + q] = acc;
  } else if (i < nv + np) {
    const int64_t q = i - nv;
    double acc = 0.;
    for (int64_t j = poff[q]; j < poff[q + 1]; ++j)
      if (live(pslot[j])) acc += ev[pslot[j]];
    y[dim * nv + q] = acc;
  }
}

hipError_t gather_element_vectors(double *y, const double *ev, const int64_t *voff, const int64_t *vslot, int64_t nv,
                                  const int64_t *poff, const int64_t *pslot, int64_t np, int dim, hipStream_t s) {
  const int64_t n = nv + np;
  if (n <= 0) return hipSuccess;
  hipLaunchKernelGGL(k_gather_ev, dim3((unsigned)((n + 255) / 256)), dim3(256), 0, s, y, ev, voff, vslot, nv, poff,
                     pslot, np, dim);
  return hipGetLastError();
}

hipError_t vec_fill(double *x, int64_t n, double a, hipStream_t s) {
  hipLaunchKernelGGL(k_fill, dim3(grid_for(n)), dim3(kBlock), 0, s, x, n, a);
  return hipGetLastError();
}
hipError_t vec_copy(double *y, const double *x, int64_t n, hipStream_t s) {
  hipLaunchKernelGGL(k_copy, dim3(grid_for(n)), dim3(kBlock), 0, s, y, x, n);
  return hipGetLastError();
}
hipError_t vec_axpy(double *y, double a, const double *x, int64_t n, hipStream_t s) {
  hipLaunchKernelGGL(k_axpy, dim3(grid_for(n)), dim3(kBlock), 0, s, y, a, x, n);
  return hipGetLastError();
}
hipError_t vec_axpby(double *y, double a, const double *x, double b, int64_t n, hipStream_t s) {
  hipLaunchKernelGGL(k_axpby, dim3(grid_for(n)), dim3(kBlock), 0, s, y, a, x, b, n);
  return hipGetLastError();
}
hipError_t vec_scale(double *x, double a, int64_t n, hipStream_t s) {
  hipLaunchKernelGGL(k_scale, dim3(grid_for(n)), dim3(kBlock), 0, s, x, a, n);
  return hipGetLastError();
}
hipError_t vec_div(double *y, const double *x, const double *d, int64_t n, hipStream_t s) {
  hipLaunchKernelGGL(k_div, dim3(grid_for(n)), dim3(kBlock), 0, s, y, x, d, n);
  return hipGetLastError();
}

hipError_t vec_multidot(const double *A, int64_t lda, int nk, const double *w, int64_t n, double *out, double *work,
                        hipStream_t s) {
  return vec_multidot2(A, lda, nk, w, n, 0, 0, out, work, s);
}

hipError_t vec_multidot2(const double *A, int64_t lda, int nk, const double *w, int64_t n1, int64_t off2, int64_t n2,
                         double *out, double *work, hipStream_t s) {
  const int nb = grid_for(n1 + n2);
  const bool v16 = vec16(A, lda, w, n1 + n2, n1, n2);
  for (int k0 = 0; k0 < nk; k0 += kDotChunk) {
    const int m = nk - k0 < kDotChunk ? nk - k0 : kDotChunk;
    const double *Ak = A + (int64_t)k0 * lda;
    switch (m) {
#define MD(M)                                                                                                  \
  case M:                                                                                                      \
    if (v16) hipLaunchKernelGGL(k_multidot16<M>, dim3(nb), dim3(kBlock), 0, s, Ak, lda, w, n1, work);          \
    else hipLaunchKernelGGL(k_multidot<M>, dim3(nb), dim3(kBlock), 0, s, Ak, lda, w, n1, off2, n2, work);      \
    break;
      MD(1) MD(2) MD(3) MD(4) MD(5) MD(6) MD(7) MD(8)
#undef MD
    }
    hipLaunchKernelGGL(k_reduce_rows, dim3(m), dim3(kBlock), 0, s, work, nb, out + k0);
  }
  return hipGetLastError();
}

hipError_t vec_multiaxpy(double *w, const double *A, int64_t lda, int nk, const double *h, double sign, int64_t n,
                         hipStream_t s, bool zero_init) {
  const int nb = grid_for(n);
  const bool v16 = vec16(A, lda, w, n, n, 0);
  if (zero_init && (!v16 || nk <= 0)) {
    const hipError_t e = vec_fill(w, n, 0.0, s);
    if (e != hipSuccess || nk <= 0) return e;
  }
  for (int k0 = 0; k0 < nk; k0 += kDotChunk) {
    const int m = nk - k0 < kDotChunk ? nk - k0 : kDotChunk;
    const double *Ak = A + (int64_t)k0 * lda;
    const bool z = zero_init && v16 && k0 == 0;
    switch (m) {
#define MA(M)                                                                                                    \
  case M:                                                                                                        \
    if (z)                                                                                                       \
      hipLaunchKernelGGL((k_multiaxpy16<M, true>), dim3(nb), dim3(kBlock), 0, s, w, Ak, lda, h + k0, sign, n);   \
    else if (v16)                                                                                                \
      hipLaunchKernelGGL((k_multiaxpy16<M, false>), dim3(nb), dim3(kBlock), 0, s, w, Ak, lda, h + k0, sign, n);  \
    else                                                                                                         \
      hipLaunchKernelGGL(k_multiaxpy<M>, dim3(nb), dim3(kBlock), 0, s, w, Ak, lda, h + k0, sign, n);             \
    break;
      MA(1) MA(2) MA(3) MA(4) MA(5) MA(6) MA(7) MA(8)
#undef MA
    }
  }
  return hipGetLastError();
}

hipError_t vec_waxpy(double *w, const double *y, double a, const double *x, int64_t n, hipStream_t s) {
  hipLaunchKernelGGL(k_waxpy, dim3(grid_for(n)), dim3(kBlock), 0, s, w, y, a, x, n);
  return hipGetLastError();
}

hipError_t vec_multiaxpy_dots(double *w, const double *A, int64_t lda, int nk, const double *h, double sign, int64_t n,
                              int64_t n1, int64_t off2, int64_t n2, bool dots, double scale, double *out, double *work,
                              hipStream_t s) {
  if (nk < 1 || nk > kDotChunk) return hipErrorInvalidValue;
  const int nb = grid_for(n);
  const bool v16 = vec16(A, lda, w, n, n1, n2);
  switch (nk * 2 + (dots ? 1 : 0)) {
#define MX(M)                                                                                                         \
  case 2 * M:                                                                                                         \
    if (v16)                                                                                                          \
      hipLaunchKernelGGL((k_multiaxpy_dot16<M, false>), dim3(nb), dim3(kBlock), 0, s, w, A, lda, h, sign, n, scale, work); \
    else                                                                                                              \
      hipLaunchKernelGGL((k_multiaxpy_dot<M, false>), dim3(nb), dim3(kBlock), 0, s, w, A, lda, h, sign, n, n1, off2, n2, \
                         scale, work);                                                                                \
    break;                                                                                                            \
  case 2 * M + 1:                                                                                                     \
    if (v16)                                                                                                          \
      hipLaunchKernelGGL((k_multiaxpy_dot16<M, true>), dim3(nb), dim3(kBlock), 0, s, w, A, lda, h, sign, n, scale, work); \
    else                                                                                                              \
      hipLaunchKernelGGL((k_multiaxpy_dot<M, true>), dim3(nb), dim3(kBlock), 0, s, w, A, lda, h, sign, n, n1, off2, n2, \
                         scale, work);                                                                                \
    break;
    MX(1) MX(2) MX(3) MX(4) MX(5) MX(6) MX(7) MX(8)
#undef MX
  }
  hipLaunchKernelGGL(k_reduce_rows, dim3(dots ? nk + 1 : 1), dim3(kBlock), 0, s, work, nb, out);
  return hipGetLastError();
}

__global__ void k_copy_gather_set(double *__restrict__ x, const double *__restrict__ v, const uint8_t *__restrict__ dmask,
                                  int64_t n, const int64_t *__restrict__ dof, const int64_t *__restrict__ off,
                                  const int64_t *__restrict__ master, const double *__restrict__ w, int64_t nl) {
  for (int64_t i = blockIdx.x * (int64_t)blockDim.x + threadIdx.x; i < n + nl; i += (int64_t)gridDim.x * blockDim.x) {
    if (i < n) {
      if (!dmask[i]) x[i] = v[i];
    } else {
      const int64_t l = i - n, j0 = off[l], nj = off[l + 1] - j0;
      constexpr int kIn = 9;
      double s = 0.;
      if (nj <= kIn) {
        int64_t m[kIn];
        double wt[kIn], vv[kIn];
#pragma unroll
        for (int t = 0; t < kIn; ++t) {
          m[t] = t < nj ? master[j0 + t] : -1;
          wt[t] = t < nj ? w[j0 + t] : 0.;
        }
#pragma unroll
        for (int t = 0; t < kIn; ++t) vv[t] = m[t] >= 0 ? v[m[t]] : 0.;
#pragma unroll
        for (int t = 0; t < kIn; ++t)
          if (t < nj) s += wt[t] * vv[t];
      } else {
        for (int64_t j = j0; j < j0 + nj; ++j) s += w[j] * v[master[j]];
      }
      x[dof[l]] = s;
    }
  }
}
hipError_t vec_copy_gather_set(double *x, const double *v, const uint8_t *dmask, int64_t n, const int64_t *dof,
                               const int64_t *off, const int64_t *master, const double *w, int64_t nl, hipStream_t s) {
  if (n + nl <= 0) return hipSuccess;
  hipLaunchKernelGGL(k_copy_gather_set, dim3(grid_for(n + nl)), dim3(kBlock), 0, s, x, v, dmask, n, dof, off, master, w,
                     nl);
  return hipGetLastError();
}

hipError_t vec_csr_gather_set(double *x, const double *src, const int64_t *dof, const int64_t *off,
                              const int64_t *master, const double *w, int64_t n, hipStream_t s) {
  if (n <= 0) return hipSuccess;
  hipLaunchKernelGGL(k_csr_gather_set, dim3(grid_for(n)), dim3(kBlock), 0, s, x, src, dof, off, master, w, n);
  return hipGetLastError();
}
template <int L>
__global__ void __launch_bounds__(256) k_csr_spmv_v(double *__restrict__ y, const double *__restrict__ x,
                                                    const int64_t *__restrict__ off, const int32_t *__restrict__ col,
                                                    const double *__restrict__ w, int64_t n, int add) {
  const int r = threadIdx.x % L;
  for (int64_t i = (blockIdx.x * (int64_t)blockDim.x + threadIdx.x) / L; i < n;
       i += (int64_t)gridDim.x * blockDim.x / L) {
    double s = 0.;
    const int64_t e = off[i + 1];
    for (int64_t j = off[i] + r; j < e; j += L) s += w[j] * x[col[j]];
#pragma unroll
    for (int m = L / 2; m > 0; m >>= 1) s += __shfl_xor(s, m, L);
    if (r == 0) y[i] = add ? y[i] + s : s;
  }
}
hipError_t vec_csr_spmv(double *y, const double *x, const int64_t *off, const int32_t *col, const double *w, int64_t n,
                        bool add, hipStream_t s, int lanes) {
  if (n <= 0) return hipSuccess;
  const int a = add ? 1 : 0;
  const int64_t th = n * (lanes < 1 ? 1 : lanes);
  const dim3 g((unsigned)std::min<int64_t>((th + 255) / 256, 65535 * 8)), b(256);
  switch (lanes) {
    case 2: hipLaunchKernelGGL(k_csr_spmv_v<2>, g, b, 0, s, y, x, off, col, w, n, a); break;
    case 4: hipLaunchKernelGGL(k_csr_spmv_v<4>, g, b, 0, s, y, x, off, col, w, n, a); break;
    case 8: hipLaunchKernelGGL(k_csr_spmv_v<8>, g, b, 0, s, y, x, off, col, w, n, a); break;
    case 16: hipLaunchKernelGGL(k_csr_spmv_v<16>, g, b, 0, s, y, x, off, col, w, n, a); break;
    default: hipLaunchKernelGGL(k_csr_spmv, dim3(grid_for(n)), dim3(kBlock), 0, s, y, x, off, col, w, n, a);
  }
  return hipGetLastError();
}
hipError_t vec_csr_condense(double *y, const int64_t *tm, const int64_t *toff, const int64_t *tdof, const double *tw,
                            int64_t n, hipStream_t s) {
  if (n <= 0) return hipSuccess;
  hipLaunchKernelGGL(k_csr_condense, dim3(grid_for(n)), dim3(kBlock), 0, s, y, tm, toff, tdof, tw, n);
  return hipGetLastError();
}

hipError_t vec_gather_scale_set(double *y, const double *d, const double *v, const int64_t *idx, int64_t m,
                                hipStream_t s, const double *rb) {
  if (m <= 0) return hipSuccess;
  hipLaunchKernelGGL(k_gather_scale_set, dim3(grid_for(m)), dim3(kBlock), 0, s, y, d, v, idx, m, rb);
  return hipGetLastError();
}
hipError_t vec_pack_nodes(const double *x, const int32_t *nodes, int64_t m, int64_t voff, double *buf, hipStream_t s) {
  if (m <= 0) return hipSuccess;
  hipLaunchKernelGGL(k_pack_nodes, dim3(grid_for(m)), dim3(kBlock), 0, s, x, nodes, m, voff, buf);
  return hipGetLastError();
}
hipError_t vec_unpack_nodes(double *x, const int32_t *nodes, int64_t m, int64_t voff, const double *buf, int add,
                            hipStream_t s) {
  if (m <= 0) return hipSuccess;
  hipLaunchKernelGGL(k_unpack_nodes, dim3(grid_for(m)), dim3(kBlock), 0, s, x, nodes, m, voff, buf, add);
  return hipGetLastError();
}
__global__ void k_pack_dofs(const double *__restrict__ x, const int32_t *__restrict__ dofs, int64_t m,
                            double *__restrict__ buf) {
  for (int64_t j = blockIdx.x * (int64_t)blockDim.x + threadIdx.x; j < m; j += (int64_t)gridDim.x * blockDim.x)
    buf[j] = x[dofs[j]];
}
__global__ void k_unpack_dofs(double *__restrict__ x, const int32_t *__restrict__ dofs, int64_t m,
                              const double *__restrict__ buf) {
  for (int64_t j = blockIdx.x * (int64_t)blockDim.x + threadIdx.x; j < m; j += (int64_t)gridDim.x * blockDim.x)
    x[dofs[j]] = buf[j];
}
__global__ void k_add_dofs_ordered(double *__restrict__ x, const int32_t *__restrict__ u, const int32_t *__restrict__ off,
                                   const int32_t *__restrict__ slot, int64_t n, const double *__restrict__ buf) {
  for (int64_t i = blockIdx.x * (int64_t)blockDim.x + threadIdx.x; i < n; i += (int64_t)gridDim.x * blockDim.x) {
    double s = x[u[i]];
    for (int j = off[i]; j < off[i + 1]; ++j) s += buf[slot[j]];
    x[u[i]] = s;
  }
}
hipError_t vec_pack_dofs(const double *x, const int32_t *dofs, int64_t m, double *buf, hipStream_t s) {
  if (m <= 0) return hipSuccess;
  hipLaunchKernelGGL(k_pack_dofs, dim3(grid_for(m)), dim3(kBlock), 0, s, x, dofs, m, buf);
  return hipGetLastError();
}
hipError_t vec_unpack_dofs(double *x, const int32_t *dofs, int64_t m, const double *buf, hipStream_t s) {
  if (m <= 0) return hipSuccess;
  hipLaunchKernelGGL(k_unpack_dofs, dim3(grid_for(m)), dim3(kBlock), 0, s, x, dofs, m, buf);
  return hipGetLastError();
}
hipError_t vec_add_dofs_ordered(double *x, const int32_t *u, const int32_t *off, const int32_t *slot, int64_t n,
                                const double *buf, hipStream_t s) {
  if (n <= 0) return hipSuccess;
  hipLaunchKernelGGL(k_add_dofs_ordered, dim3(grid_for(n)), dim3(kBlock), 0, s, x, u, off, slot, n, buf);
  return hipGetLastError();
}
__global__ void k_add_nodes_ordered(double *__restrict__ x, const int32_t *__restrict__ u, const int32_t *__restrict__ off,
                                    const int32_t *__restrict__ slot, int64_t n, int64_t voff,
                                    const double *__restrict__ buf) {
  for (int64_t i = blockIdx.x * (int64_t)blockDim.x + threadIdx.x; i < n; i += (int64_t)gridDim.x * blockDim.x) {
    const int64_t nd = u[i];
    double s0 = x[nd * 3 + 0], s1 = x[nd * 3 + 1], s2 = x[nd * 3 + 2], s3 = x[voff + nd];
    for (int j = off[i]; j < off[i + 1]; ++j) {
      const double *b = buf + (int64_t)slot[j] * 4;
      s0 += b[0];
      s1 += b[1];
      s2 += b[2];
      s3 += b[3];
    }
    x[nd * 3 + 0] = s0;
    x[nd * 3 + 1] = s1;
    x[nd * 3 + 2] = s2;
    x[voff + nd] = s3;
  }
// ... 150 lines not shown
```

Measured before the change: 12.55 nonlinear_iters/s.

## Fuse first Jacobi sweep into GMRES orthogonalization and MG restriction; reuse rhs norm

Result: faster. 13.12 nonlinear_iters/s (median of 6 runs) (+4.5%).

```diff
diff --git a/softx_2020_200_amd/csrc/gls_api.cpp b/softx_2020_200_amd/csrc/gls_api.cpp
--- a/softx_2020_200_amd/csrc/gls_api.cpp
+++ b/softx_2020_200_amd/csrc/gls_api.cpp
@@ -924,12 +924,13 @@
   return err;
 }
 int multiaxpy_dots_async(gls_ctx *c, double *w, const double *V, int64_t lda, int nk, const double *h, bool dots,
-                         double *out, double *hp, const double **dev_res, double scale = 1.0) {
+                         double *out, double *hp, const double **dev_res, double scale = 1.0, double *x0 = nullptr,
+                         const double *x0d = nullptr, double x0omega = 0.0) {
   const int64_t n1 = c->dist.on ? (int64_t)c->dim * c->dist.n_owned : c->n_dofs;
   const int64_t off2 = c->dist.on ? (int64_t)c->dim * c->n_vnodes : 0;
   const int64_t n2 = c->dist.on ? c->dist.n_owned_p : 0;
   HIP_TRY(gls::vec_multiaxpy_dots(w, V, lda, nk, h, 1.0, c->n_dofs, n1, off2, n2, dots, scale, out, c->work.p,
-                                  c->stream));
+                                  c->stream, x0, x0d, x0omega));
   int err;
   *dev_res = reduce_dots_async(c, out, dots ? nk + 1 : 1, hp, &err);
   return err;
@@ -1170,6 +1171,7 @@
 int gls_set_state(gls_ctx *c, const double *u, const double *u1, const double *u2, const double *u3) {
   GLS_TRY(check_ctx(c));
   if (!u) return set_err(GLS_EINVAL, "u is null");
+  c->bnorm2_of = nullptr;
   c->u = u;
   c->u1 = u1;
   c->u2 = u2;
@@ -1321,6 +1323,7 @@
 int gls_residual(gls_ctx *c, double *rhs) {
   GLS_TRY(check_ctx(c));
   if (!rhs) return set_err(GLS_EINVAL, "rhs is null");
+  c->bnorm2_of = nullptr;
   GLS_TRY(run_cell(c, gls::MODE_RESIDUAL, nullptr, rhs));
   HIP_TRY(gls::vec_set_indexed(rhs, c->con_dofs.p, nullptr, (int64_t)c->con_dofs.n, c->stream));
   return GLS_OK;
@@ -1329,6 +1332,7 @@
 int gls_residual_and_diagonal(gls_ctx *c, double *rhs, double *d) {
   GLS_TRY(check_ctx(c));
   if (!rhs) return set_err(GLS_EINVAL, "rhs is null");
+  c->bnorm2_of = nullptr;
   if (!c->u) return set_err(GLS_EINVAL, "gls_set_state was not called");
   if (c->n_hist > 0 && !c->u1) return set_err(GLS_EINVAL, "scheme needs solution_m1");
   if (c->n_hist > 1 && !c->u2) return set_err(GLS_EINVAL, "scheme needs solution_m2");
@@ -1708,9 +1712,9 @@
 }
 
 namespace {
-int apply_prec(gls_ctx *c, const double *v, double *z) {
+int apply_prec(gls_ctx *c, const double *v, double *z, bool x0_ready = false) {
   if (c->mg.on && c->mg.rep_csr) return mg_vcycle_rep2(c, v, z);
-  if (c->mg.on) return mg_vcycle(c, 0, v, z);
+  if (c->mg.on) return mg_vcycle(c, 0, v, z, x0_ready);
   if (c->ilu.on && !c->ilu.probe_only) return apply_ilu(c, v, z);
   HIP_TRY(gls::vec_div(z, v, c->diag.p, c->n_dofs, c->stream));
   return GLS_OK;
@@ -1805,6 +1809,8 @@
 int gls_solve_linear(gls_ctx *c, const double *b, double *x, gls_linear_params *prm) {
   GLS_TRY(check_ctx(c));
   if (!b || !x || !prm) return set_err(GLS_EINVAL, "null argument");
+  const double *const bnorm2_of = c->bnorm2_of;
+  c->bnorm2_of = nullptr;
   const int m = prm->restart > 0 ? std::min(prm->restart, 200) : 30;
   const int64_t n = c->n_dofs;
   if (c->krylov_m != m || !c->krylov.p) {
@@ -1834,8 +1840,8 @@
   if (keepz && c->zbasis.n != (size_t)m * n) GLS_TRY(c->zbasis.alloc((size_t)m * n));
   double *V = c->krylov.p, *z = c->tmp1.p, *r = c->tmp2.p;
   hipStream_t s = c->stream;
-  double bnorm2;
-  GLS_TRY(device_dot(c, b, b, &bnorm2));
+  double bnorm2 = c->bnorm2_val;
+  if (bnorm2_of != b || std::getenv("GLS_GMRES_NO_NORM_REUSE") != nullptr) GLS_TRY(device_dot(c, b, b, &bnorm2));
   const double tol = std::max(prm->relative_residual * std::sqrt(bnorm2), prm->minimum_residual);
   bool x_zero = keepz;
   if (!keepz) HIP_TRY(gls::vec_fill(x, n, 0.0, s));
@@ -1847,6 +1853,13 @@
   int ortho_repairs = 0;
   const double repair_tol = std::getenv("GLS_GMRES_REPAIR_TOL") ? std::atof(std::getenv("GLS_GMRES_REPAIR_TOL")) : 1e-8;
   const bool repair_measured = std::getenv("GLS_GMRES_REPAIR_MEASURED") != nullptr;
+  const char *fle = std::getenv("GLS_GMRES_FULL_LAST_COLUMN");
+  const bool full_last = fle && std::atoi(fle) != 0;
+  std::vector<double> hcol((size_t)m + 2);
+  const double *x0d = nullptr;
+  double x0omega = 0.;
+  if (keepz) GLS_TRY(mg_fine_first_producer(c, &x0d, &x0omega));
+  bool x0_ready = false;
   std::vector<double> Gm((size_t)(m + 1) * (m + 1), 0.0);
   bool converged = beta <= tol;
   const bool lverbose = std::getenv("GLS_ILU_VERBOSE") != nullptr;
@@ -1858,10 +1871,13 @@
     g[0] = beta;
     int j = 0;
     double res = beta;
+    x0_ready = false;
     for (; j < m && it < prm->max_iterations; ++j) {
       double *vj = V + (int64_t)j * n, *w = V + (int64_t)(j + 1) * n;
       double *zj = keepz ? c->zbasis.p + (int64_t)j * n : z;
-      GLS_TRY(apply_prec(c, vj, zj));
+      GLS_TRY(apply_prec(c, vj, zj, x0_ready));
+      x0_ready = false;
+      double *x0 = x0d && j + 1 < m && j + 1 <= 8 ? c->zbasis.p + (int64_t)(j + 1) * n : nullptr;
       GLS_TRY(gls_jacobian_apply(c, zj, w));
       double *hp1 = c->hpin, *hp2 = c->hpin + (m + 8), *hp3 = c->hpin + 2 * (m + 8);
       const double *hdev = nullptr, *h2dev = nullptr, *h3dev = nullptr;
@@ -1869,6 +1885,7 @@
       double wn2, wnorm, wnorm0;
       bool normalized = false;
       bool done = false;
+      bool rotated = false;
       if (gram) {
         HIP_TRY(hipStreamSynchronize(s));
         const double wn0sq = std::max(hp1[j + 1], 0.0);
@@ -1885,11 +1902,39 @@
         for (int i = 0; i <= j; ++i) q += hc[i] * hc[i] - 2.0 * hc[i] * hp1[i];
         for (int i = 0; i <= j; ++i)
           for (int k = i + 1; k <= j; ++k) q += 2.0 * hc[i] * hc[k] * G(i, k);
-        if (q > 1e-20 * wn0sq && q > 0.) {
-          const double est = std::sqrt(q);
+        const bool qok = q > 1e-20 * wn0sq && q > 0.;
+        const double est = qok ? std::sqrt(q) : 0.;
+        if (qok && !full_last) {
+          for (int i = 0; i <= j; ++i) hcol[i] = hc[i];
+          hcol[j + 1] = est;
+          for (int i = 0; i < j; ++i) {
+            const double a = hcol[i], bb = hcol[i + 1];
+            hcol[i] = cs[i] * a + sn[i] * bb;
+            hcol[i + 1] = -sn[i] * a + cs[i] * bb;
+          }
+          const double a = hcol[j], bb = hcol[j + 1];
+          const double rr = std::hypot(a, bb);
+          const double csj = rr > 0 ? a / rr : 1.0, snj = rr > 0 ? bb / rr : 0.0;
+          if (std::fabs(-snj * g[j]) <= tol) {
+            for (int i = 0; i < j; ++i) H[(size_t)i * m + j] = hcol[i];
+            H[(size_t)j * m + j] = rr;
+            H[(size_t)(j + 1) * m + j] = 0.;
+            cs[j] = csj;
+            sn[j] = snj;
+            g[j + 1] = -snj * g[j];
+            g[j] = csj * g[j];
+            wnorm = est;
+            normalized = done = rotated = true;
+            if (std::getenv("GLS_GMRES_VERBOSE")) printf("  gmres: column %d converges, its projection is skipped\n", j);
+          }
+        }
+        if (rotated) {
+        } else if (qok) {
           HIP_TRY(hipMemcpyAsync(c->coef.p, hc, sizeof(double) * (j + 1), hipMemcpyHostToDevice, s));
           if (j + 1 <= 8) {
-            GLS_TRY(multiaxpy_dots_async(c, w, V, n, j + 1, c->coef.p, true, c->scal2.p, hp2, &h2dev, 1.0 / est));
+            GLS_TRY(multiaxpy_dots_async(c, w, V, n, j + 1, c->coef.p, true, c->scal2.p, hp2, &h2dev, 1.0 / est, x0, x0d,
+                                         x0omega));
+            x0_ready = x0 != nullptr;
           } else {
             HIP_TRY(gls::vec_multiaxpy(w, V, n, j + 1, c->coef.p, 1.0, n, s));
             HIP_TRY(gls::vec_scale(w, 1.0 / est, n, s));
@@ -1910,7 +1955,8 @@
             const double est2 = use_est ? std::sqrt(est2sq) : 1.0;
             for (int i = 0; i <= j; ++i) H[(size_t)i * m + j] += est * hp2[i];
             if (j + 1 <= 8) {
-              GLS_TRY(multiaxpy_dots_async(c, w, V, n, j + 1, h2dev, true, c->scal.p, hp1, &hdev, 1.0 / est2));
+              GLS_TRY(multiaxpy_dots_async(c, w, V, n, j + 1, h2dev, true, c->scal.p, hp1, &hdev, 1.0 / est2, x0, x0d,
+                                           x0omega));
             } else {
               HIP_TRY(gls::vec_multiaxpy(w, V, n, j + 1, h2dev, 1.0, n, s));
               if (use_est) HIP_TRY(gls::vec_scale(w, 1.0 / est2, n, s));
@@ -1921,9 +1967,11 @@
             double sc = 1.0;
             if (nn <= 1e-28 * (use_est ? 1.0 : std::max(nrm2, 1e-300))) {
               sc = 0.0;
+              x0_ready = false;
             } else if (!use_est || std::fabs(nn - 1.0) > 1e-8) {
               sc = std::sqrt(nn);
               HIP_TRY(gls::vec_scale(w, 1.0 / sc, n, s));
+              x0_ready = false;
             }
             H[(size_t)(j + 1) * m + j] = est * est2 * sc;
             for (int i = 0; i <= j; ++i) Gm[(size_t)i * (m + 1) + j + 1] = sc > 0. ? hp1[i] / sc : 0.;
@@ -1985,19 +2033,21 @@
         H[(size_t)(j + 1) * m + j] = wnorm;
         if (wnorm > 0) HIP_TRY(gls::vec_scale(w, 1.0 / wnorm, n, s));
       }
-      for (int i = 0; i < j; ++i) {
-        const double a = H[(size_t)i * m + j], bb = H[(size_t)(i + 1) * m + j];
-        H[(size_t)i * m + j] = cs[i] * a + sn[i] * bb;
-        H[(size_t)(i + 1) * m + j] = -sn[i] * a + cs[i] * bb;
+      if (!rotated) {
+        for (int i = 0; i < j; ++i) {
+          const double a = H[(size_t)i * m + j], bb = H[(size_t)(i + 1) * m + j];
+          H[(size_t)i * m + j] = cs[i] * a + sn[i] * bb;
+          H[(size_t)(i + 1) * m + j] = -sn[i] * a + cs[i] * bb;
+        }
+        const double a = H[(size_t)j * m + j], bb = H[(size_t)(j + 1) * m + j];
+        const double rr = std::hypot(a, bb);
+        cs[j] = rr > 0 ? a / rr : 1.0;
+        sn[j] = rr > 0 ? bb / rr : 0.0;
+        H[(size_t)j * m + j] = rr;
+        H[(size_t)(j + 1) * m + j] = 0.;
+        g[j + 1] = -sn[j] * g[j];
+        g[j] = cs[j] * g[j];
       }
-      const double a = H[(size_t)j * m + j], bb = H[(size_t)(j + 1) * m + j];
-      const double rr = std::hypot(a, bb);
-      cs[j] = rr > 0 ? a / rr : 1.0;
-      sn[j] = rr > 0 ? bb / rr : 0.0;
-      H[(size_t)j * m + j] = rr;
-      H[(size_t)(j + 1) * m + j] = 0.;
-      g[j + 1] = -sn[j] * g[j];
-      g[j] = cs[j] * g[j];
       res = std::fabs(g[j + 1]);
       ++it;
       if (getenv("GLS_GMRES_VERBOSE") && (it % 10 == 0 || it == 1))
@@ -2180,6 +2230,8 @@
   int rhs_norm(double &r) {
     double r2;
     GLS_TRY(device_dot(c, rhs, rhs, &r2));
+    c->bnorm2_of = rhs;
+    c->bnorm2_val = r2;
     r = std::sqrt(r2);
     return GLS_OK;
   }
@@ -2268,6 +2320,7 @@
     GLS_TRY(newton_template(ph, prm->tolerance, prm->max_iterations, prm->verbosity, st));
   }
   HIP_TRY(hipStreamSynchronize(c->stream));
+  c->bnorm2_of = nullptr;
   prm->newton_iterations = st.outer;
   prm->linear_iterations = st.linear;
   prm->residual_evaluations = st.residuals;
diff --git a/softx_2020_200_amd/csrc/gls_brick_kernels.hip b/softx_2020_200_amd/csrc/gls_brick_kernels.hip
--- a/softx_2020_200_amd/csrc/gls_brick_kernels.hip
+++ b/softx_2020_200_amd/csrc/gls_brick_kernels.hip
@@ -1253,7 +1253,9 @@
 }
 
 __global__ void __launch_bounds__(256) k_restrict_sum_cube(const double *__restrict__ ev, int nb1, int64_t voff,
-                                                           double *__restrict__ bc, const uint8_t *__restrict__ vmask) {
+                                                           double *__restrict__ bc, const uint8_t *__restrict__ vmask,
+                                                           double *__restrict__ x0, const double *__restrict__ d,
+                                                           double omega) {
   const int NX = 2 * nb1 + 1;
   int bx = blockIdx.x, Z = blockIdx.y;
   if (GLS_SLAB_XCD) {
@@ -1323,17 +1325,22 @@
     }
   const int64_t node = X + (int64_t)NX * (Y + (int64_t)NX * Z);
   const unsigned m = vmask ? vmask[node] : 0u;
-  bc[node * 3] = (m & 1u) ? 0.0 : s[0];
-  bc[node * 3 + 1] = (m & 2u) ? 0.0 : s[1];
-  bc[node * 3 + 2] = (m & 4u) ? 0.0 : s[2];
-  bc[voff + node] = s[3];
+  const double r[4] = {(m & 1u) ? 0.0 : s[0], (m & 2u) ? 0.0 : s[1], (m & 4u) ? 0.0 : s[2], s[3]};
+  const int64_t row[4] = {node * 3, node * 3 + 1, node * 3 + 2, voff + node};
+#pragma unroll
+  for (int q = 0; q < 4; ++q) bc[row[q]] = r[q];
+  if (x0) {
+#pragma unroll
+    for (int q = 0; q < 4; ++q) x0[row[q]] = 0.0 + omega * r[q] / d[row[q]];
+  }
 }
 hipError_t brick_restrict_sum_cube(int nb1, const double *ev, int64_t n_vnodes, double *bc, const uint8_t *vmask,
-                                   hipStream_t s) {
+                                   hipStream_t s, double *x0, const double *d, double omega) {
   const int64_t NX = 2 * (int64_t)nb1 + 1;
-  if (nb1 <= 0 || nb1 > 1023 || !ev || !bc || NX * NX * NX != n_vnodes) return hipErrorInvalidValue;
+  if (nb1 <= 0 || nb1 > 1023 || !ev || !bc || NX * NX * NX != n_vnodes || (x0 && (!d || x0 == bc)))
+    return hipErrorInvalidValue;
   const dim3 g((unsigned)((NX * NX + 255) / 256), (unsigned)NX), b(256);
-  hipLaunchKernelGGL(k_restrict_sum_cube, g, b, 0, s, ev, nb1, 3 * n_vnodes, bc, vmask);
+  hipLaunchKernelGGL(k_restrict_sum_cube, g, b, 0, s, ev, nb1, 3 * n_vnodes, bc, vmask, x0, d, omega);
   return hipGetLastError();
 }
 
diff --git a/softx_2020_200_amd/csrc/gls_ctx.hpp b/softx_2020_200_amd/csrc/gls_ctx.hpp
--- a/softx_2020_200_amd/csrc/gls_ctx.hpp
+++ b/softx_2020_200_amd/csrc/gls_ctx.hpp
@@ -74,6 +74,8 @@
   DevBuf<double> zbasis;
   DevBuf<double> bicg;
   int krylov_m = 0;
+  const double *bnorm2_of = nullptr;
+  double bnorm2_val = 0.;
   DevBuf<double> tmp1, tmp2, tmp3, tmp4, tmp5;
   bool use_brick = false;
   bool use_slab = false;
@@ -341,8 +343,9 @@
                    const double *pxc = nullptr);
 
 int mg_prepare(gls_ctx *c);
-int mg_vcycle(gls_ctx *c, int l, const double *b, double *x);
+int mg_vcycle(gls_ctx *c, int l, const double *b, double *x, bool x0_ready = false);
 int mg_vcycle_rep2(gls_ctx *c, const double *b, double *x);
+int mg_fine_first_producer(gls_ctx *c, const double **d, double *omega);
 
 int ilu_probe(gls_ctx *c);
 int ensure_ilu(gls_ctx *c);
diff --git a/softx_2020_200_amd/csrc/gls_launch.hpp b/softx_2020_200_amd/csrc/gls_launch.hpp
--- a/softx_2020_200_amd/csrc/gls_launch.hpp
+++ b/softx_2020_200_amd/csrc/gls_launch.hpp
@@ -41,7 +41,7 @@
                                const double *rb = nullptr, double *x0 = nullptr,
                                const double *xs = nullptr);
 hipError_t brick_restrict_sum_cube(int nb1, const double *ev, int64_t n_vnodes, double *bc, const uint8_t *vmask,
-                                   hipStream_t s);
+                                   hipStream_t s, double *x0 = nullptr, const double *d = nullptr, double omega = 0.0);
 bool brick_fused_jacobi_supported(int k);
 bool brick_colors_supported(int k);
 bool brick_subset_supported(int k);
@@ -65,7 +65,8 @@
 hipError_t vec_waxpy(double *w, const double *y, double a, const double *x, int64_t n, hipStream_t s);
 hipError_t vec_multiaxpy_dots(double *w, const double *A, int64_t lda, int nk, const double *h, double sign, int64_t n,
                               int64_t n1, int64_t off2, int64_t n2, bool dots, double scale, double *out,
-                              double *work, hipStream_t s);
+                              double *work, hipStream_t s, double *x0 = nullptr, const double *d = nullptr,
+                              double omega = 0.0);
 hipError_t vec_csr_gather_set(double *x, const double *src, const int64_t *dof, const int64_t *off,
                               const int64_t *master, const double *w, int64_t n, hipStream_t s);
 hipError_t vec_copy_gather_set(double *x, const double *v, const uint8_t *dmask, int64_t n, const int64_t *dof,
diff --git a/softx_2020_200_amd/csrc/gls_mg.cpp b/softx_2020_200_amd/csrc/gls_mg.cpp
--- a/softx_2020_200_amd/csrc/gls_mg.cpp
+++ b/softx_2020_200_amd/csrc/gls_mg.cpp
@@ -301,11 +301,13 @@
          gls::pencil_enabled() && gls::brick_fused_jacobi_supported(g->k) && !h->dist.on && !h->hang.on &&
          h->n_vnodes == nc1 * nc1 * nc1 && g->stream == c->stream;
 }
-int mg_residual_restrict_fused(gls_ctx *c, int l, double *x, const double *b, double *bc, double first_omega = 0.0) {
+int mg_residual_restrict_fused(gls_ctx *c, int l, double *x, const double *b, double *bc, double first_omega = 0.0,
+                               double *xc0 = nullptr, double omega_c = 0.0) {
   gls_ctx *g = c->mg.lev[(size_t)l], *h = c->mg.lev[(size_t)l + 1];
   if (!g->u) return set_err(GLS_EINVAL, "gls_set_state was not called");
   GLS_TRY(ensure_diag(g));
   GLS_TRY(ensure_qdata32(g, !g->smooth_oseen));
+  if (xc0) GLS_TRY(ensure_diag(h));
   gls::OpParams P = make_params(g, true);
   P.qdf = g->qdata32.p;
   P.oseen = g->smooth_oseen ? 1 : 0;
@@ -324,7 +326,8 @@
     HIP_TRY(gls::launch_pencil_jv_restrict(P, g->tables, c->stream));
   }
   TimedLaunch t(g, 5);
-  HIP_TRY(gls::brick_restrict_sum_cube(g->cube_nb1, P.slab, h->n_vnodes, bc, h->vmask.p, c->stream));
+  HIP_TRY(gls::brick_restrict_sum_cube(g->cube_nb1, P.slab, h->n_vnodes, bc, h->vmask.p, c->stream, xc0,
+                                       xc0 ? h->diag.p : nullptr, omega_c));
   return GLS_OK;
 }
 
@@ -400,14 +403,14 @@
 }
 
 int mg_presmooth(gls_ctx *g, hipStream_t s, int pre, double om, double *zs, const double *b, double *x, double *y,
-                 bool residual) {
+                 bool residual, bool x0_ready = false) {
   const int64_t n = g->n_dofs;
   if (pre > 0 && zs) {
     GLS_TRY(ensure_ilu(g));
     GLS_TRY(apply_ilu(g, b, x));
     for (int it = 1; it < pre; ++it) GLS_TRY(smoother_sweep(g, x, b, y, om, zs));
   } else if (pre > 0) {
-    HIP_TRY(gls::mg_jacobi_update(x, b, nullptr, g->diag.p, om, n, 1, s));
+    if (!x0_ready) HIP_TRY(gls::mg_jacobi_update(x, b, nullptr, g->diag.p, om, n, 1, s));
     for (int it = 1; it < pre; ++it) GLS_TRY(smoother_sweep(g, x, b, y, om));
   } else {
     HIP_TRY(gls::vec_fill(x, n, 0.0, s));
@@ -416,6 +419,20 @@
   if (pre > 0) return smoother_apply(g, x, y, b);
   HIP_TRY(gls::vec_copy(y, b, n, s));
   return GLS_OK;
+}
+bool mg_first_producer_ok(gls_ctx *c, int l) {
+  auto &mg = c->mg;
+  const int L = (int)mg.lev.size();
+  if (l < 0 || l >= L) return false;
+  const char *e = std::getenv("GLS_MG_FIRST_PRODUCER");
+  if ((e && std::atoi(e) == 0) || std::getenv("GLS_MG_NO_FUSE") != nullptr) return false;
+  gls_ctx *g = mg.lev[(size_t)l];
+  if (l == L - 1 && (mg.replica || mg.coarse.ok)) return false;
+  const int pre = l == L - 1 ? mg.csweeps : mg.lpre[(size_t)l];
+  if (pre < 1 || g->dist.on || g->stream != c->stream) return false;
+  if (l == L - 1 && l > 0 && pre > 1 && coarse_graph_eligible(c, g, mgbuf(c, l, MB_B), mgbuf(c, l, MB_X))) return false;
+  if (pre == 1 && l < L - 1 && first_sweep_fusable(g)) return false;
+  return !(mg.ilu_smooth && g->ilu.on && !g->ilu.probe_only);
 }
 int mg_coarse_solve(gls_ctx *c, gls_ctx *g, const double *b, double *x) {
   auto &mg = c->mg;
@@ -453,7 +470,18 @@
   return GLS_OK;
 }
 
-int mg_vcycle(gls_ctx *c, int l, const double *b, double *x) {
+int mg_fine_first_producer(gls_ctx *c, const double **d, double *omega) {
+  *d = nullptr;
+  auto &mg = c->mg;
+  if (!mg.on || mg.rep_csr || mg.lev.empty() || c->dist.on || !mg_first_producer_ok(c, 0)) return GLS_OK;
+  gls_ctx *g = mg.lev[0];
+  GLS_TRY(ensure_diag(g));
+  *d = g->diag.p;
+  *omega = mg.lev.size() == 1 ? mg.comega : mg.omega;
+  return GLS_OK;
+}
+
+int mg_vcycle(gls_ctx *c, int l, const double *b, double *x, bool x0_ready) {
   auto &mg = c->mg;
   const int L = (int)mg.lev.size();
   gls_ctx *g = mg.lev[l];
@@ -483,18 +511,20 @@
   const bool first_fused = pre == 1 && l < L - 1 && first_sweep_fusable(g);
   double *zs = mg.ilu_smooth && g->ilu.on && !g->ilu.probe_only ? mgbuf(c, l, MB_BOX) : nullptr;
   const bool fused_restrict = l < L - 1 && pre > 0 && mg_fused_restrict_ok(c, l);
-  if (!first_fused) GLS_TRY(mg_presmooth(g, s, pre, om, zs, b, x, y, l < L - 1 && !fused_restrict));
+  if (!first_fused) GLS_TRY(mg_presmooth(g, s, pre, om, zs, b, x, y, l < L - 1 && !fused_restrict, x0_ready));
   if (l == L - 1) return GLS_OK;
   gls_ctx *h = mg.lev[l + 1];
   double *bc = mgbuf(c, l + 1, MB_B), *xc = mgbuf(c, l + 1, MB_X);
+  const bool xc_ready = fused_restrict && mg_first_producer_ok(c, l + 1);
   if (fused_restrict) {
-    GLS_TRY(mg_residual_restrict_fused(c, l, x, b, bc, first_fused ? om : 0.0));
+    GLS_TRY(mg_residual_restrict_fused(c, l, x, b, bc, first_fused ? om : 0.0, xc_ready ? xc : nullptr,
+                                       l + 1 == L - 1 ? mg.comega : mg.omega));
   } else {
     if (first_fused) GLS_TRY(jacobian_apply_f32(g, x, y, b, om, g->smooth_oseen));
     GLS_TRY(mg_restrict(c, l, y, bc));
     HIP_TRY(gls::vec_set_indexed(bc, h->con_dofs.p, nullptr, (int64_t)h->con_dofs.n, s));
   }
-  GLS_TRY(mg_vcycle(c, l + 1, bc, xc));
+  GLS_TRY(mg_vcycle(c, l + 1, bc, xc, xc_ready));
   const bool pro = mg_fused_prolong_ok(c, l);
   if (pro) {
   } else if (mg_prolong_add_ok(c, l)) {
diff --git a/softx_2020_200_amd/csrc/gls_vector_kernels.hip b/softx_2020_200_amd/csrc/gls_vector_kernels.hip
--- a/softx_2020_200_amd/csrc/gls_vector_kernels.hip
+++ b/softx_2020_200_amd/csrc/gls_vector_kernels.hip
@@ -215,10 +215,12 @@
     work[threadIdx.x * gridDim.x + blockIdx.x] = t;
   }
 }
-template <int NK, bool DOTS>
+template <int NK, bool DOTS, bool X0 = false>
 __global__ void __launch_bounds__(kBlock) k_multiaxpy_dot16(double *__restrict__ w, const double *__restrict__ A,
                                                             int64_t lda, const double *__restrict__ h, double sign,
-                                                            int64_t n, double scale, double *work) {
+                                                            int64_t n, double scale, double *work,
+                                                            double *__restrict__ x0 = nullptr,
+                                                            const double *__restrict__ d = nullptr, double omega = 0.0) {
   constexpr int ND = (DOTS ? NK : 0) + 1;
   double hk[NK], acc[ND];
 #pragma unroll
@@ -246,15 +248,21 @@
       a0[k] = a.x;
       a1[k] = a.y;
     }
+    dbl2 di = {1.0, 1.0};
+    if constexpr (X0) di = __builtin_nontemporal_load(reinterpret_cast<const dbl2 *>(d) + p);
     const dbl2 wi = reinterpret_cast<const dbl2 *>(w)[p];
     const double o0 = row(wi.x, a0), o1 = row(wi.y, a1);
     reinterpret_cast<dbl2 *>(w)[p] = dbl2{o0, o1};
+    if constexpr (X0)
+      __builtin_nontemporal_store(dbl2{0.0 + omega * o0 / di.x, 0.0 + omega * o1 / di.y}, reinterpret_cast<dbl2 *>(x0) + p);
   }
   if ((n & 1) && blockIdx.x == 0 && threadIdx.x == 0) {
     double a[NK];
 #pragma unroll
     for (int k = 0; k < NK; ++k) a[k] = A[k * lda + n - 1];
-    w[n - 1] = row(w[n - 1], a);
+    const double o = row(w[n - 1], a);
+    w[n - 1] = o;
+    if constexpr (X0) x0[n - 1] = 0.0 + omega * o / d[n - 1];
   }
   __shared__ double red[ND][kBlock / 64];
   const int lane = threadIdx.x & 63, wv = threadIdx.x >> 6;
@@ -526,10 +534,11 @@
 
 hipError_t vec_multiaxpy_dots(double *w, const double *A, int64_t lda, int nk, const double *h, double sign, int64_t n,
                               int64_t n1, int64_t off2, int64_t n2, bool dots, double scale, double *out, double *work,
-                              hipStream_t s) {
-  if (nk < 1 || nk > kDotChunk) return hipErrorInvalidValue;
+                              hipStream_t s, double *x0, const double *d, double omega) {
+  if (nk < 1 || nk > kDotChunk || (x0 && (!d || x0 == w))) return hipErrorInvalidValue;
   const int nb = grid_for(n);
   const bool v16 = vec16(A, lda, w, n, n1, n2);
+  const bool x16 = x0 && v16 && dots && ((uintptr_t)x0 % 16) == 0 && ((uintptr_t)d % 16) == 0;
   switch (nk * 2 + (dots ? 1 : 0)) {
 #define MX(M)                                                                                                         \
   case 2 * M:                                                                                                         \
@@ -540,7 +549,10 @@
                          scale, work);                                                                                \
     break;                                                                                                            \
   case 2 * M + 1:                                                                                                     \
-    if (v16)                                                                                                          \
+    if (x16)                                                                                                          \
+      hipLaunchKernelGGL((k_multiaxpy_dot16<M, true, true>), dim3(nb), dim3(kBlock), 0, s, w, A, lda, h, sign, n, scale, \
+                         work, x0, d, omega);                                                                         \
+    else if (v16)                                                                                                     \
       hipLaunchKernelGGL((k_multiaxpy_dot16<M, true>), dim3(nb), dim3(kBlock), 0, s, w, A, lda, h, sign, n, scale, work); \
     else                                                                                                              \
       hipLaunchKernelGGL((k_multiaxpy_dot<M, true>), dim3(nb), dim3(kBlock), 0, s, w, A, lda, h, sign, n, n1, off2, n2, \
@@ -550,6 +562,7 @@
 #undef MX
   }
   hipLaunchKernelGGL(k_reduce_rows, dim3(dots ? nk + 1 : 1), dim3(kBlock), 0, s, work, nb, out);
+  if (x0 && !x16) return mg_jacobi_update(x0, w, nullptr, d, omega, n, 1, s);
   return hipGetLastError();
 }
 
```
